# jcyk/gtos

Measured on AMD Instinct MI355X. Metric: graphs/sec training step (100-node AMR, batch 64), higher is better.
Workload: dtype bf16

## Files before the change

### gtos_amd/_lib.py

```python
import ctypes
import os
import threading

import torch

_HERE = os.path.dirname(os.path.abspath(__file__))
LIB_PATH = os.path.join(_HERE, "csrc", "libgtos_hip.so")
ABI_VERSION = 25

c_p, c_i, c_l, c_f, c_u64 = ctypes.c_void_p, ctypes.c_int, ctypes.c_int64, ctypes.c_float, ctypes.c_uint64

SIGNATURES = {
    "gtos_abi_version": [],
    "gtos_pathtrie_dev_workspace": [c_l, c_l, c_p],
    "gtos_pathtrie_dev_phase_a": [c_i, c_l, c_p, c_p, c_p, c_p, c_p, c_p, c_p, ctypes.c_size_t, c_p],
    "gtos_pathtrie_dev_phase_b": [c_l, c_l, c_i, c_i, c_i, c_i, c_p, c_p, c_p, c_p, c_p, ctypes.c_size_t, c_p],
    "gtos_relbatch_dev_workspace": [c_l, c_p],
    "gtos_relbatch_dev_phase_a": [c_p, c_p, c_p, ctypes.c_size_t, c_p],
    "gtos_relbatch_dev_phase_b": [c_p, c_l, c_p, c_p, ctypes.c_size_t, c_p],
    "gtos_relbatch_dev_all_count": [c_p, c_p, c_p, ctypes.c_size_t, c_p],
    "gtos_relbatch_dev_all_keys": [c_p, c_p, c_p, ctypes.c_size_t, c_p],
    "gtos_relbatch_dev_all_fill": [c_p, c_l, c_p, c_p, ctypes.c_size_t, c_p],
    "gtos_relindex_dev_workspace": [c_l, c_p],
    "gtos_relindex_dev_phase_a": [c_p, c_p, c_p, ctypes.c_size_t, c_p],
    "gtos_relindex_dev_phase_b": [c_p, c_l, c_p, c_p, ctypes.c_size_t, c_p],
    "gtos_gemm": [c_i, c_i, c_i, c_i, c_i, c_i, c_i, c_p, c_l, c_p, c_l, c_p, c_l, c_p, c_i, c_f, c_u64, c_i, c_i, c_p, c_l, c_p],
    "gtos_rel_attn_fwd": [c_i] * 7 + [c_p, c_l, c_p, c_l, c_p, c_l, c_p, c_p, c_p, c_p, c_f, c_f, c_u64, c_p, c_l, c_p, c_p, c_p],
    "gtos_rel_attn_bwd": [c_i] * 7 + [c_p, c_l, c_p, c_l, c_p, c_l, c_p, c_p, c_p, c_p, c_p, c_f, c_f, c_u64,
                                      c_p, c_l, c_p, c_p, c_p, c_l, c_p, c_p, c_l, c_p, c_l, c_p, c_l, c_p, c_l, c_p, c_p, c_p],
    "gtos_rel_attn_bwd_bank": [c_i] * 5 + [c_p, c_l, c_p, c_l, c_p, c_p, c_p, c_p, c_p, c_p, c_p, c_p, c_i, c_p, c_l, c_p, c_p],
    "gtos_ln_residual_fwd": [c_i, c_i, c_i, c_p, c_p, c_f, c_u64, c_p, c_p, c_f, c_p, c_p, c_p, c_p],
    "gtos_ln_residual_bwd": [c_i, c_i, c_i, c_p, c_p, c_p, c_f, c_u64, c_p, c_p, c_p, c_p, c_p, c_p, c_p, c_p],
    "gtos_ln_residual_fwd2": [c_i, c_i, c_i, c_i, c_i, c_p, c_p, c_f, c_u64, c_p, c_p, c_f, c_p, c_p, c_p, c_p, c_p],
    "gtos_ln_residual_bwd2": [c_i, c_i, c_i, c_i, c_i, c_p, c_p, c_p, c_p, c_f, c_u64, c_p, c_p, c_p, c_p, c_p, c_p, c_p, c_p],
    "gtos_relu_dropout_bwd": [c_i, c_l, c_p, c_p, c_f, c_p],
    "gtos_colsum": [c_i, c_i, c_i, c_l, c_p, c_p, c_p],
    "gtos_gru_cell_fwd": [c_i, c_i, c_i, c_p, c_p, c_p, c_p, c_l, c_p, c_p, c_f, c_u64, c_l, c_p],
    "gtos_gru_step_fwd": [c_i, c_i, c_p, c_l, c_i, c_p, c_p, c_p, c_p, c_p, c_p, c_p, c_p, c_p, c_p, c_p, c_p, c_i, c_p, c_l, c_p, c_p, c_p, c_l,
                          c_f, c_u64, c_l, c_p],
    "gtos_gru_step_bwd": [c_i, c_i, c_p, c_i, c_p, c_p, c_p, c_p, c_p, c_l, c_p, c_i, c_l, c_p, c_f, c_u64, c_l, c_p, c_i, c_p, c_p, c_p, c_i, c_p],
    "gtos_gru_step_bwd_fused": [c_i, c_i, c_p, c_i, c_p, c_p, c_p, c_p, c_p, c_l, c_p, c_i, c_l, c_p, c_f, c_u64, c_l, c_p, c_i, c_p, c_p, c_p, c_i,
                                c_p, c_p, c_l, c_i, c_i, c_f, c_u64, c_l, c_p],
    "gtos_gru_weight_grads": [c_i, c_i, c_i, c_i, c_p, c_p, c_l, c_p, c_l, c_p, c_l, c_p, c_l, c_p, c_l, c_p],
    "gtos_gemm_tn_batch": [c_i, c_p, c_p, c_p, c_p, c_p, c_p, c_p, c_p, c_p, c_p, c_p],
    "gtos_embed_packed_paths": [c_i, c_i, c_i, c_l, c_p, c_p, c_p, c_p, c_i, c_i, c_p, c_f, c_u64, c_p, c_i, c_p, c_p],
    "gtos_segment_sum_rows": [c_i, c_p, c_p, c_p, c_p, c_p, c_p, c_p, c_l, c_i, c_p, c_p, c_l, c_p, c_p, c_p],
    "gtos_segment_sum_stream": [c_i, c_i, c_p, c_p, c_p, c_p, c_p, c_p, c_i, c_p, c_l, c_i, c_p, c_l, c_p, c_p],
    "gtos_segment_sum_finish": [c_i, c_p, c_p, c_i, c_p, c_l, c_p],
    "gtos_segment_sum_ranges": [c_i, c_p, c_p, c_l, c_i, c_p, c_l, c_p],
    "gtos_gru_cell_bwd": [c_i, c_i, c_i, c_p, c_p, c_p, c_l, c_p, c_p, c_p, c_f, c_u64, c_l, c_p, c_i, c_p],
    "gtos_relation_gather_mean": [c_i, c_l, c_i, c_i, c_p, c_p, c_i, c_p, c_p],
    "gtos_embed_rows_fwd": [c_i, c_l, c_i, c_i, c_p, c_p, c_p, c_f, c_u64, c_p],
    "gtos_embed_rows_bwd": [c_i, c_l, c_i, c_i, c_i, c_p, c_p, c_p, c_f, c_u64, c_p, c_l, c_p],
    "gtos_copy_nll_fwd": [c_i, c_i, c_i, c_i, c_i, c_p, c_l, c_p, c_p, c_p, c_p, c_l, c_p, c_p, c_p, c_p],
    "gtos_copy_nll_bwd": [c_i, c_i, c_i, c_i, c_i, c_p, c_l, c_p, c_p, c_p, c_p, c_l, c_p, c_p, c_p, c_p, c_p, c_p, c_p],
    "gtos_copy_ll_fwd": [c_i, c_i, c_i, c_i, c_i, c_i, c_p, c_l, c_p, c_p, c_p, c_p, c_p],
    "gtos_copy_nll_ls_prep": [c_i, c_i, c_i, c_p, c_p, c_l, c_p],
    "gtos_copy_nll_ls_fwd": [c_i] * 5 + [c_p, c_l, c_p, c_p, c_p, c_l, c_f, c_p, c_l, c_p, c_p, c_p, c_p],
    "gtos_copy_nll_ls_bwd": [c_i] * 5 + [c_p, c_l, c_p, c_p, c_p, c_l, c_f, c_p, c_l, c_p, c_p, c_p, c_p, c_p, c_p, c_p],
    "gtos_copy_eval_fwd": [c_i, c_i, c_i, c_i, c_i, c_p, c_l, c_p, c_p, c_p, c_p, c_l, c_p, c_p, c_p, c_p],
    "gtos_eval_accumulate": [c_i, c_i, c_p, c_p, c_p, c_l, c_p, c_p, c_p, c_p, c_p],
    "gtos_beam_topk": [c_i, c_i, c_i, c_p, c_l, c_p, c_p, c_p],
    "gtos_beam_advance": [c_i] * 7 + [c_p] * 13,
    "gtos_beam_reorder": [c_i, c_p, c_p, c_l, c_i, c_i, c_i, c_i, c_p, c_p, c_p, c_p, c_i, c_i, c_p, c_p, c_p, c_p, c_i, c_l, c_p, c_p,
                          c_p, c_p],
    "gtos_sample_step": [c_i] * 7 + [c_f, c_i, c_f, c_u64, c_p, c_l] + [c_p] * 11 + [c_i, c_l] + [c_p] * 4,
    "gtos_highway_fwd": [c_i, c_l, c_i, c_p, c_p, c_p, c_p],
    "gtos_highway_bwd": [c_i, c_l, c_i, c_p, c_p, c_p, c_p, c_p, c_p],
    "gtos_max_relu_fwd": [c_i, c_l, c_i, c_i, c_p, c_p, c_p, c_p],
    "gtos_max_relu_bwd": [c_i, c_l, c_i, c_i, c_p, c_p, c_p, c_p, c_p],
    "gtos_token_row_fwd": [c_i, c_l, c_i, c_i, c_i, c_p, c_p, c_p, c_p, c_f, c_u64, c_p],
    "gtos_token_row_bwd": [c_i, c_l, c_i, c_i, c_i, c_p, c_p, c_p, c_p, c_f, c_u64, c_p],
    "gtos_sqnorm": [c_l, c_p, c_p, c_p],
    "gtos_adam_step": [c_l, c_p, c_p, c_p, c_p, c_f, c_f, c_f, c_f, c_f, c_f, c_p, c_f, c_p, c_p],
    "gtos_cast_f32_to_bf16": [c_l, c_p, c_p, c_p],
    "gtos_transpose_batch_bf16": [c_i, c_p, c_p, c_i, c_p, c_p, c_p],
    "gtos_step_control": [c_i, c_p, c_p, c_p, c_i, c_i, c_p, c_p],
    "gtos_set_seed_epoch": [c_p],
    "gtos_adam_step_ctl": [c_l, c_p, c_p, c_p, c_p, c_p, c_f, c_f, c_f, c_f, c_f, c_p, c_f, c_p, c_p],
}

_lib = None
_load_lock = threading.Lock()


class GtosHipError(RuntimeError):
    pass


def load():
    global _lib
    if _lib is not None:
        return _lib
    with _load_lock:
        if _lib is not None:
            return _lib
        if not os.path.exists(LIB_PATH):
            raise GtosHipError("%s is missing: run `python -m gtos_amd.build` (or __graft_entry__.build()); "
                               "there is no CPU fallback for the gtos hot path" % LIB_PATH)
        lib = ctypes.CDLL(LIB_PATH)
        for name, args in SIGNATURES.items():
            fn = getattr(lib, name)
            fn.argtypes = args
            fn.restype = ctypes.c_int
        if lib.gtos_abi_version() != ABI_VERSION:
            raise GtosHipError("libgtos_hip.so ABI %d != binding ABI %d: rebuild" % (lib.gtos_abi_version(), ABI_VERSION))
        _lib = lib
    return _lib


def call(name, *args):
    rc = getattr(load(), name)(*args)
    if rc != 0:
        raise GtosHipError("%s failed with code %d (%s)" % (
            name, rc, "HIP launch error" if rc > 0 else "unsupported argument/shape"))


def ptr(t):
    return None if t is None else t.data_ptr()


_raw_stream = None


def stream():
    global _raw_stream
    if _raw_stream:
        return _raw_stream(torch.cuda.current_device())
    pub = torch.cuda.current_stream().cuda_stream
    if _raw_stream is None:
        try:
            raw = torch._C._cuda_getCurrentRawStream
            ok = raw(torch.cuda.current_device()) == pub
            probe = torch.cuda.Stream()
            with torch.cuda.stream(probe):
                ok = ok and raw(torch.cuda.current_device()) == probe.cuda_stream == torch.cuda.current_stream().cuda_stream
            ok = ok and raw(torch.cuda.current_device()) == pub
            _raw_stream = raw if ok else False
        except Exception:
            _raw_stream = False
    return pub


def dt(t):
    if t.dtype == torch.float32:
        return 0
    if t.dtype == torch.bfloat16:
        return 1
    raise GtosHipError("unsupported dtype %s" % t.dtype)


def require_cuda(*ts):
    for t in ts:
        if t is not None and not t.is_cuda:
            raise GtosHipError("gtos_amd ops run on the GPU only (got a %s tensor); there is no CPU fallback" % t.device)
```

### gtos_amd/csrc/gemm.hip

```cpp
#include "common.h"
#include <stdlib.h>

__attribute__((visibility("hidden"))) const void* gtos_zero_block() {
    static void* z = nullptr;
    if (!z) {
        if (hipMalloc(&z, 256) != hipSuccess) return nullptr;
        if (hipMemset(z, 0, 256) != hipSuccess) return nullptr;
    }
    return z;
}

namespace {

constexpr int BM = 128, BN = 128;
constexpr int ROWB = 128;

template <typename T> struct GemmCfg;
template <> struct GemmCfg<bf16_t> { static constexpr int BK = 64, VEC = 8; };
template <> struct GemmCfg<float>  { static constexpr int BK = 32, VEC = 4; };

template <int NTH> struct TCfg {
    static constexpr int NT = NTH, WAVES_N = NTH / 128, WTN = BN / WAVES_N, NTW = WTN / 16;
    static constexpr int ITERS = 1024 / NTH;
};
// ... 639 lines not shown
    bool hi[2];
    uint32_t aoff[2][2], boff[2][2];
#pragma unroll
    for (int j = 0; j < 2; ++j) {
        const int rb = (wave + 8 * j) * 8 + (lane >> 3);
        const uint32_t ch = (uint32_t)(((lane & 7) ^ ((rb >> 1) & 7)) << 4);
        hi[j] = ch >= 64;
#pragma unroll
        for (int h = 0; h < 2; ++h) {
            aoff[h][j] = (uint32_t)min((rb >> 6) * 128 + h * 64 + (rb & 63), amax) * lda2 + ch;
            boff[h][j] = (uint32_t)min((rb >> 5) * 64 + h * 32 + (rb & 31), bmax) * ldb2 + ch;
        }
    }
    const int fo0 = fr * ROWB + ((fq ^ ((fr >> 1) & 7)) << 4), fo1 = fr * ROWB + (((4 + fq) ^ ((fr >> 1) & 7)) << 4);
    const int fa_base = wr * 64 * ROWB, fb_base = wc * 32 * ROWB;

    f32x4_t acc[8][4];
#pragma unroll
    for (int i = 0; i < 8; ++i)
#pragma unroll
        for (int j = 0; j < 4; ++j) acc[i][j] = f32x4_t{0.f, 0.f, 0.f, 0.f};
    bf16x8_t fa[4][2], fb[2][2];

#define GTOS_QDMA(src, dst)                                                                                                   \
    __builtin_amdgcn_global_load_lds((const __attribute__((address_space(1))) void*)(src),                                    \
                                     (__attribute__((address_space(3))) void*)(dst), 16, 0, 0)
#define GTOS_QISSUE(buf, isA, h, kt_)                                                                                         \
    {                                                                                                                         \
        const int kb_ = min((kt_), nk - 1) * 128;                                                                             \
        const bool tl_ = tail32 && (kt_) >= nk - 1;                                                                           \
        const char* s0_ = ((isA) ? Ab : Bb) + kb_ + ((isA) ? aoff[h][0] : boff[h][0]);                                        \
        const char* s1_ = ((isA) ? Ab : Bb) + kb_ + ((isA) ? aoff[h][1] : boff[h][1]);                                        \
        GTOS_QDMA((tl_ && hi[0]) ? Zl : s0_, (buf) + wave * 1024);                                                            \
        GTOS_QDMA((tl_ && hi[1]) ? Zl : s1_, (buf) + (8 + wave) * 1024);                                                      \
    }
#define GTOS_QREAD_A(buf)                                                                                                     \
    _Pragma("unroll") for (int i = 0; i < 4; ++i) {                                                                           \
        fa[i][0] = *reinterpret_cast<const bf16x8_t*>((buf) + fa_base + i * 16 * ROWB + fo0);                                 \
        fa[i][1] = *reinterpret_cast<const bf16x8_t*>((buf) + fa_base + i * 16 * ROWB + fo1);                                 \
    }
#define GTOS_QREAD_B(buf)                                                                                                     \
    _Pragma("unroll") for (int j = 0; j < 2; ++j) {                                                                           \
        fb[j][0] = *reinterpret_cast<const bf16x8_t*>((buf) + fb_base + j * 16 * ROWB + fo0);                                 \
        fb[j][1] = *reinterpret_cast<const bf16x8_t*>((buf) + fb_base + j * 16 * ROWB + fo1);                                 \
    }
#define GTOS_QPHASE(READS, ISSUE, mh, nh)                                                                                     \
    {                                                                                                                         \
        READS;                                                                                                                \
        __builtin_amdgcn_sched_barrier(0);                                                                                    \
        ISSUE;                                                                                                                \
        GTOS_VMCNT(4);                                             \
        __builtin_amdgcn_s_barrier();                                                                                         \
        __builtin_amdgcn_s_waitcnt(0xc07f);                                           \
        __builtin_amdgcn_sched_barrier(0);                                                                                    \
        _Pragma("unroll") for (int ks = 0; ks < 2; ++ks)                                                                      \
            _Pragma("unroll") for (int i = 0; i < 4; ++i)                                                                     \
                _Pragma("unroll") for (int j = 0; j < 2; ++j)                                                                 \
                    acc[(mh) * 4 + i][(nh) * 2 + j] =                                                                         \
                        __builtin_amdgcn_mfma_f32_16x16x32_bf16(fb[j][ks], fa[i][ks], acc[(mh) * 4 + i][(nh) * 2 + j], 0, 0, 0); \
        __builtin_amdgcn_sched_barrier(0);                                                                                    \
        __builtin_amdgcn_s_barrier();                                                                                         \
    }
#define GTOS_QTILE(A0_, B0_, B1_, A1_, nA0, nB0, nB1, nA1, kt_)                                                               \
    GTOS_QPHASE({ GTOS_QREAD_B(B0_); __builtin_amdgcn_sched_barrier(0); GTOS_QREAD_A(A0_); }, GTOS_QISSUE(nA0, true, 0, (kt_) + 1), 0, 0); \
    GTOS_QPHASE({ GTOS_QREAD_B(B1_); }, GTOS_QISSUE(nB0, false, 0, (kt_) + 1), 0, 1);                                         \
    GTOS_QPHASE({ GTOS_QREAD_A(A1_); }, GTOS_QISSUE(nB1, false, 1, (kt_) + 1), 1, 1);                                         \
    GTOS_QPHASE({ GTOS_QREAD_B(B0_); }, GTOS_QISSUE(nA1, true, 1, (kt_) + 1), 1, 0);

    GTOS_QISSUE(a00, true, 0, 0);
    GTOS_QISSUE(b00, false, 0, 0);
    GTOS_QISSUE(b01, false, 1, 0);
    GTOS_QISSUE(a01, true, 1, 0);
    GTOS_VMCNT(4);
    __builtin_amdgcn_s_barrier();
    if (wave >= 4) __builtin_amdgcn_s_barrier();
    int kt = 0;
    for (; kt + 2 <= nk; kt += 2) {
        GTOS_QTILE(a00, b00, b01, a01, a10, b10, b11, a11, kt);
        GTOS_QTILE(a10, b10, b11, a11, a00, b00, b01, a01, kt + 1);
    }
    if (kt < nk) { GTOS_QTILE(a00, b00, b01, a01, a10, b10, b11, a11, kt); }
    if (wave < 4) __builtin_amdgcn_s_barrier();
    GTOS_VMCNT(0);
    __syncthreads();
#undef GTOS_QTILE
#undef GTOS_QPHASE
#undef GTOS_QREAD_A
#undef GTOS_QREAD_B
#undef GTOS_QISSUE
#undef GTOS_QDMA

    bf16_t* C = static_cast<bf16_t*>(a.C);
    const float keep_scale = a.p_drop > 0.f ? 1.f / (1.f - a.p_drop) : 1.f;
    constexpr int CP = 64 * 2 + 16;
    char* cs = (wave < 4 ? a00 : b00) + (wave & 3) * 32 * CP;
#pragma unroll
    for (int q4 = 0; q4 < 4; ++q4) {
#pragma unroll
        for (int mh = 0; mh < 2; ++mh)
#pragma unroll
            for (int nt = 0; nt < 4; ++nt) {
                const int mt = q4 * 2 + mh;
                const int m = m0 + wm + mt * 16 + fr, n = n0 + wn + nt * 16 + fq * 4;
                float v[4] = {acc[mt][nt][0], acc[mt][nt][1], acc[mt][nt][2], acc[mt][nt][3]};
#pragma unroll
                for (int i = 0; i < 4; ++i) {
                    if (a.bias && n + i < a.N) v[i] += a.bias[n + i];
                    if (a.relu) v[i] = fmaxf(v[i], 0.f);
                    if (a.p_drop > 0.f)
                        v[i] = drop_keep(a.seed, (uint64_t)m * (uint64_t)a.N + (uint64_t)(n + i), a.p_drop) ? v[i] * keep_scale : 0.f;
                }
                *reinterpret_cast<uint2*>(cs + (mh * 16 + fr) * CP + (nt * 16 + fq * 4) * 2) = make_uint2(pack_bf(v[0], v[1]), pack_bf(v[2], v[3]));
            }
        __builtin_amdgcn_fence(__ATOMIC_RELEASE, "wavefront");
        __builtin_amdgcn_s_waitcnt(0xc07f);
#pragma unroll
        for (int pass = 0; pass < 4; ++pass) {
            const int row = pass * 8 + (lane >> 3), col = (lane & 7) * 8;
            const int m = m0 + wm + q4 * 32 + row, n = n0 + wn + col;
            if (m >= a.M || n >= a.N) continue;
            uint4 val = *reinterpret_cast<const uint4*>(cs + row * CP + col * 2);
            bf16_t* cp = C + (int64_t)m * a.ldc + n;
            if (n + 8 <= a.N) {
                if (a.accumulate) {
                    const uint4 old = *reinterpret_cast<const uint4*>(cp);
                    val = make_uint4(pack_bf(lo_bf(val.x) + lo_bf(old.x), hi_bf(val.x) + hi_bf(old.x)),
                                     pack_bf(lo_bf(val.y) + lo_bf(old.y), hi_bf(val.y) + hi_bf(old.y)),
                                     pack_bf(lo_bf(val.z) + lo_bf(old.z), hi_bf(val.z) + hi_bf(old.z)),
                                     pack_bf(lo_bf(val.w) + lo_bf(old.w), hi_bf(val.w) + hi_bf(old.w)));
                }
                *reinterpret_cast<uint4*>(cp) = val;
            } else {
                const bf16_t* e = reinterpret_cast<const bf16_t*>(cs + row * CP + col * 2);
                for (int i = 0; i < 8 && n + i < a.N; ++i) {
                    float o = bf2f(e[i]);
                    if (a.accumulate) o += bf2f(cp[i]);
                    cp[i] = f2bf(o);
                }
            }
        }
        __builtin_amdgcn_s_waitcnt(0xc07f);
    }
}

int launch256p(const GemmArgs& a, hipStream_t s) {
    const long long nMt = (a.M + BM2 - 1) / BM2, nNt = (a.N + BN2 - 1) / BN2;
    const long long nblk = ((nMt + 7) / 8) * 8 * nNt;
    if (nblk > 0x7fffffffLL) return -6;
    hipLaunchKernelGGL(gemm256q_nt_kernel, dim3((unsigned)nblk), dim3(512), 0, s, a);
    GTOS_CHECK_LAUNCH();
    return 0;
}

struct TnGroup {
    const bf16_t* B1; int64_t ldb1; int N1;
    int tiles;
    int tmn[64];
};

struct TnJob { const bf16_t* A; const bf16_t* B; float* C; int lda, ldb, ldc, M, N, K, tile_end, nN; };
constexpr int TN_MAX_JOBS = 48;
struct TnBatch { int njobs, ntiles; TnJob job[TN_MAX_JOBS]; };

template <int MODE, typename G>
__global__ __launch_bounds__(512) void gemm256p_tn_kernel(GemmArgs a, G g) {
    constexpr bool GROUPED = MODE == 1;
    __shared__ __attribute__((aligned(16))) char st0[ST3];
    __shared__ __attribute__((aligned(16))) char st1[ST3];
    __shared__ __attribute__((aligned(16))) char st2[ST3];
    __shared__ __attribute__((aligned(16))) char st3[ST3];
    const int lane = threadIdx.x & 63, wave = __builtin_amdgcn_readfirstlane(threadIdx.x >> 6);
    const int fr = lane & 15, fq = lane >> 4;
    const int wm = (wave >> 2) * 128, wn = (wave & 3) * 64;
    const int nN = (a.N + BN2 - 1) / BN2, nM = (a.M + BM2 - 1) / BM2;
    int tiles = nM * nN;
    if constexpr (GROUPED) tiles = g.tiles;
    if constexpr (MODE == 2) tiles = 1;
    const int xcd = blockIdx.x & 7, sq = blockIdx.x >> 3;
    int bz = (sq / tiles) * 8 + xcd, t_ = sq % tiles;
    if constexpr (MODE == 2) { bz = 0; t_ = blockIdx.x; if (t_ >= g.ntiles) return; }
    if (bz >= a.splitk) return;
    int m0, n0, Nv;
    const bf16_t* Bp;
    int64_t ldb, wld;
    float* wst;
    if constexpr (MODE == 2) {
        int j = 0;
        while (j + 1 < g.njobs && t_ >= g.job[j].tile_end) ++j;
        const TnJob& jb = g.job[j];
        const int tl = t_ - (j ? g.job[j - 1].tile_end : 0);
        m0 = (tl / jb.nN) * BM2; n0 = (tl % jb.nN) * BN2;
        a.A = jb.A; a.lda = jb.lda; a.M = jb.M; a.K = jb.K; a.splitk = 1;
        Bp = jb.B; ldb = jb.ldb; Nv = jb.N;
        wst = jb.C + (int64_t)m0 * jb.ldc + n0; wld = jb.ldc;
    } else if constexpr (GROUPED) {
        const int e = g.tmn[t_], src = (e >> 8) & 255;
        m0 = (e & 255) * BM2; n0 = ((e >> 16) & 255) * BN2;
        Bp = src ? g.B1 : static_cast<const bf16_t*>(a.B); ldb = src ? g.ldb1 : a.ldb; Nv = src ? g.N1 : a.N;
        wst = a.ws + ((int64_t)bz * tiles + t_) * (BM2 * BN2); wld = BN2;
    } else {
        m0 = (t_ / nN) * BM2; n0 = (t_ % nN) * BN2;
        Bp = static_cast<const bf16_t*>(a.B); ldb = a.ldb; Nv = a.N;
        wst = a.ws + ((int64_t)bz * a.M + m0) * a.N + n0; wld = a.N;
    }
    const int ktiles = (a.K + 63) / 64, tps = (ktiles + a.splitk - 1) / a.splitk;
    const int kbeg = bz * tps * 64, kend = min(a.K, kbeg + tps * 64);
    if (kbeg >= kend) return;
    const int nk = (kend - kbeg + 31) / 32;
    const char* Z = static_cast<const char*>(a.zeros);
    const int kr = lane >> 5, pp = lane & 31;
    const int kl0 = 2 * wave + kr, kq_d = kl0 & 3;
    const int lp = ((((pp >> 1) ^ kq_d)) << 1) | (pp & 1);
    const int acol = min(m0 + lp * 8, a.M - 8), bcol = min(n0 + lp * 8, Nv - 8);
    const char* pa = reinterpret_cast<const char*>(static_cast<const bf16_t*>(a.A) + (int64_t)(kbeg + kl0) * a.lda + acol);
    const char* pb = reinterpret_cast<const char*>(Bp + (int64_t)(kbeg + kl0) * ldb + bcol);
    const int64_t a16 = 32 * a.lda, b16 = 32 * ldb;
    int kcur = kbeg + kl0;
    const int kq = fr >> 2;
    const int fbase = (fq * 8 + kq) * 512 + (fr & 3) * 8;

    f32x4_t acc[8][4];
#pragma unroll
    for (int i = 0; i < 8; ++i)
#pragma unroll
        for (int j = 0; j < 4; ++j) acc[i][j] = f32x4_t{0.f, 0.f, 0.f, 0.f};
    bf16x8_t fa[8], fb[4];

#define GTOS_DMA1(src, dst)                                                                                                   \
    __builtin_amdgcn_global_load_lds((const __attribute__((address_space(1))) void*)(src),                                    \
                                     (__attribute__((address_space(3))) void*)(dst), 16, 0, 0)
#define GTOS_DMA4(stage)                                                                                                      \
    {                                                                                                                         \
        const bool ok0 = kcur < kend, ok1 = kcur + 16 < kend;                                                                 \
        GTOS_DMA1(ok0 ? pa : Z, (stage) + wave * 1024);                                                                       \
        GTOS_DMA1(ok1 ? pa + a16 : Z, (stage) + (8 + wave) * 1024);                                                           \
        GTOS_DMA1(ok0 ? pb : Z, (stage) + A3 + wave * 1024);                                                                  \
        GTOS_DMA1(ok1 ? pb + b16 : Z, (stage) + A3 + (8 + wave) * 1024);                                                      \
        kcur += 32; pa += 2 * a16; pb += 2 * b16;                                                                             \
    }
#define GTOS_TRF(tile, c0)                                                                                                    \
    ([&]() -> bf16x8_t {                                                                                                      \
        const char* p0 = (tile) + fbase + ((((c0) >> 4) ^ kq) << 5);                                                          \
        const s16x4_t lo = __builtin_amdgcn_ds_read_tr16_b64_v4i16((__attribute__((address_space(3))) s16x4_t*)(p0));         \
        const s16x4_t hi = __builtin_amdgcn_ds_read_tr16_b64_v4i16((__attribute__((address_space(3))) s16x4_t*)(p0 + 4 * 512)); \
        const s16x8_t v = {lo[0], lo[1], lo[2], lo[3], hi[0], hi[1], hi[2], hi[3]};                                           \
        return __builtin_bit_cast(bf16x8_t, v);                                                                               \
    }())
#define GTOS_STEP(slot_s, slot_d, s_)                                                                                         \
    {                                                                                                                         \
        GTOS_DMA4(slot_d);                                                                                                  \
        _Pragma("unroll") for (int t = 0; t < 4; ++t) fb[t] = GTOS_TRF((slot_s) + A3, wn + t * 16);                           \
        _Pragma("unroll") for (int t = 0; t < 8; ++t) fa[t] = GTOS_TRF((slot_s), wm + t * 16);                                \
        __builtin_amdgcn_s_waitcnt(0x0078);                 \
        __builtin_amdgcn_s_barrier();                                                                                         \
        __builtin_amdgcn_sched_barrier(0);                                                                                    \
        _Pragma("unroll") for (int mt = 0; mt < 8; ++mt)                                                                      \
            _Pragma("unroll") for (int nt = 0; nt < 4; ++nt)                                                                  \
                acc[mt][nt] = __builtin_amdgcn_mfma_f32_16x16x32_bf16(fb[nt], fa[mt], acc[mt][nt], 0, 0, 0);                  \
        __builtin_amdgcn_sched_barrier(0);                                                                                    \
        __builtin_amdgcn_s_barrier();                                                                                         \
    }

    GTOS_DMA4(st0);
    GTOS_DMA4(st1);
    GTOS_DMA4(st2);
    GTOS_VMCNT(8);
    __builtin_amdgcn_s_barrier();
    if (wave >= 4) __builtin_amdgcn_s_barrier();
    int s = 0;
    for (; s + 4 <= nk; s += 4) {
        GTOS_STEP(st0, st3, s);
        GTOS_STEP(st1, st0, s + 1);
        GTOS_STEP(st2, st1, s + 2);
        GTOS_STEP(st3, st2, s + 3);
    }
    if (s < nk) {
        GTOS_STEP(st0, st3, s);
        if (s + 1 < nk) {
            GTOS_STEP(st1, st0, s + 1);
            if (s + 2 < nk) GTOS_STEP(st2, st1, s + 2);
        }
    }
    if (wave < 4) __builtin_amdgcn_s_barrier();
#undef GTOS_STEP
#undef GTOS_TRF
#undef GTOS_DMA4
#undef GTOS_DMA1

#pragma unroll
    for (int mt = 0; mt < 8; ++mt) {
        const int m = m0 + wm + mt * 16 + fr;
        if (m >= a.M) continue;
#pragma unroll
        for (int nt = 0; nt < 4; ++nt) {
            const int n = n0 + wn + nt * 16 + fq * 4;
            if (n >= Nv) continue;
            float4* dst = reinterpret_cast<float4*>(wst + (int64_t)(m - m0) * wld + (n - n0));
            if constexpr (MODE == 2) {
                const float4 o = *dst;
                *dst = make_float4(o.x + acc[mt][nt][0], o.y + acc[mt][nt][1], o.z + acc[mt][nt][2], o.w + acc[mt][nt][3]);
            } else {
                *dst = make_float4(acc[mt][nt][0], acc[mt][nt][1], acc[mt][nt][2], acc[mt][nt][3]);
            }
        }
    }
}

struct ColJob { const bf16_t* A; float* out; int lda, M, K, blk_end, gx; };
struct ColBatch { int njobs, nblocks, rpb; ColJob job[TN_MAX_JOBS]; };
__global__ __launch_bounds__(256) void colsum_batch_kernel(ColBatch g) {
    __shared__ float red[4][64][8];
    int t_ = blockIdx.x, j = 0;
    if (t_ >= g.nblocks) return;
    while (j + 1 < g.njobs && t_ >= g.job[j].blk_end) ++j;
    const ColJob& jb = g.job[j];
    const int tl = t_ - (j ? g.job[j - 1].blk_end : 0);
    const int bx = tl % jb.gx, by = tl / jb.gx;
    const int lane = threadIdx.x & 63, w = threadIdx.x >> 6;
    const int c = (bx * 64 + lane) * 8;
    const int r0 = by * g.rpb, r1 = min(jb.K, r0 + g.rpb);
    float acc[8] = {0, 0, 0, 0, 0, 0, 0, 0};
    if (c < jb.M) {
        for (int r = r0 + w; r < r1; r += 4) {
            float v[8];
            Vec8<bf16_t>::load(jb.A + (int64_t)r * jb.lda + c, v);
#pragma unroll
            for (int e = 0; e < 8; ++e) acc[e] += v[e];
        }
    }
#pragma unroll
    for (int e = 0; e < 8; ++e) red[w][lane][e] = acc[e];
    __syncthreads();
    if (w == 0 && c < jb.M) {
#pragma unroll
        for (int e = 0; e < 8; ++e) atomicAdd(jb.out + c + e, red[0][lane][e] + red[1][lane][e] + red[2][lane][e] + red[3][lane][e]);
    }
}

struct GruDwOut { float* dwih; int64_t ld_ih; float* dwhh; int64_t ld_hh; int hs, in_dim; };
__global__ void gru_dw_reduce_kernel(const float* __restrict__ ws, int splits, TnGroup g, GruDwOut o) {
    const int t_ = blockIdx.x >> 6, q = (blockIdx.x & 63) * 256 + threadIdx.x;
    const int e = g.tmn[t_], src = (e >> 8) & 255;
    const int r = q >> 6, c = (q & 63) * 4;
    const int i = (e & 255) * BM2 + r, j = ((e >> 16) & 255) * BN2 + c;
    if (i >= 4 * o.hs) return;
    const int gate = i / o.hs, ch = i - gate * o.hs;
    float* dst;
    if (src == 0) {
        if (gate == 3 || j >= o.in_dim) return;
        dst = o.dwih + (int64_t)(gate * o.hs + ch) * o.ld_ih + j;
    } else {
        if (gate == 2 || j >= o.hs) return;
        dst = o.dwhh + (int64_t)((gate == 3 ? 2 : gate) * o.hs + ch) * o.ld_hh + j;
    }
    const float* p = ws + (int64_t)t_ * (BM2 * BN2) + r * BN2 + c;
    const int64_t plane = (int64_t)g.tiles * (BM2 * BN2);
    float4 acc = *reinterpret_cast<const float4*>(p);
    for (int s = 1; s < splits; ++s) {
        const float4 v = *reinterpret_cast<const float4*>(p + s * plane);
        acc.x += v.x; acc.y += v.y; acc.z += v.z; acc.w += v.w;
    }
    dst[0] += acc.x; dst[1] += acc.y; dst[2] += acc.z; dst[3] += acc.w;
}

int launch256p_tn(const GemmArgs& a, hipStream_t s) {
    const long long tiles = ((long long)(a.M + BM2 - 1) / BM2) * ((a.N + BN2 - 1) / BN2);
    const long long nblk = tiles * 8 * ((a.splitk + 7) / 8);
    if (nblk > 0x7fffffffLL) return -6;
    hipLaunchKernelGGL((gemm256p_tn_kernel<0, TnGroup>), dim3((unsigned)nblk), dim3(512), 0, s, a, TnGroup{});
    GTOS_CHECK_LAUNCH();
    return 0;
}

int launch256(const GemmArgs& a, hipStream_t s) {
    static bool configured = false;
    if (!configured) {
        if (hipFuncSetAttribute(reinterpret_cast<const void*>(gemm256_nt_kernel), hipFuncAttributeMaxDynamicSharedMemorySize,
                                2 * STAGE2) != hipSuccess) return -7;
        configured = true;
    }
    const long long nMt = (a.M + BM2 - 1) / BM2, nNt = (a.N + BN2 - 1) / BN2;
    const long long nblk = ((nMt + 7) / 8) * 8 * nNt;
    if (nblk > 0x7fffffffLL) return -6;
    hipLaunchKernelGGL(gemm256_nt_kernel, dim3((unsigned)nblk), dim3(512), 2 * STAGE2, s, a);
    GTOS_CHECK_LAUNCH();
    return 0;
}

template <typename T, typename TO>
int launch(const GemmArgs& a, int transA, int transB, hipStream_t s) {
    const long long nMt = (a.M + BM - 1) / BM, nNt = (a.N + BN - 1) / BN;
    const long long nblk = a.splitk > 1 ? nMt * nNt * 8 * ((a.splitk + 7) / 8) : ((nMt + 7) / 8) * 8 * nNt;
    if (nblk > 0x7fffffffLL) return -6;
    dim3 grid((unsigned)nblk);
    const bool fast = a.vecA && a.vecB;
    constexpr bool BF = sizeof(T) == 2;
    if (!transA && transB) {
        if (fast) hipLaunchKernelGGL((gemm_kernel<T, TO, false, true, true, 256, 1>), grid, dim3(256), 0, s, a);
        else      hipLaunchKernelGGL((gemm_kernel<T, TO, false, true, false, 512, 2>), grid, dim3(512), 0, s, a);
    } else if (!transA && !transB) {
        if (fast && BF) hipLaunchKernelGGL((gemm_kernel<T, TO, false, false, true, 256, BF ? 1 : 2>), grid, dim3(256), 0, s, a);
        else if (fast)  hipLaunchKernelGGL((gemm_kernel<T, TO, false, false, true, 512, 2>), grid, dim3(512), 0, s, a);
        else            hipLaunchKernelGGL((gemm_kernel<T, TO, false, false, false, 512, 2>), grid, dim3(512), 0, s, a);
    } else if (transA && !transB) {
        if (fast && BF) hipLaunchKernelGGL((gemm_kernel<T, TO, true, false, true, 256, BF ? 1 : 2>), grid, dim3(256), 0, s, a);
        else if (fast)  hipLaunchKernelGGL((gemm_kernel<T, TO, true, false, true, 512, 2>), grid, dim3(512), 0, s, a);
        else            hipLaunchKernelGGL((gemm_kernel<T, TO, true, false, false, 512, 2>), grid, dim3(512), 0, s, a);
    } else return -2;
    GTOS_CHECK_LAUNCH();
    return 0;
}

}

extern "C" int gtos_gemm(int in_dtype, int out_dtype, int transA, int transB, int M, int N, int K,
                         const void* A, int64_t lda, const void* B, int64_t ldb, void* C, int64_t ldc,
                         const float* bias, int relu, float p_drop, uint64_t seed, int accumulate,
                         int splitk, void* workspace, int64_t workspace_bytes, void* stream) {
    if (M <= 0 || N <= 0) return 0;
    if (K <= 0) return -3;
    const int es = in_dtype == GTOS_BF16 ? 2 : 4, vec = 16 / es;
    const int eo = out_dtype == GTOS_BF16 ? 2 : 4;
    GemmArgs a;
    a.A = A; a.B = B; a.C = C; a.bias = bias; a.M = M; a.N = N; a.K = K; a.lda = lda; a.ldb = ldb; a.ldc = ldc;
    a.vecA = ((uintptr_t)A % 16 == 0) && (lda % vec == 0) && ((transA ? M : K) % vec == 0);
    a.vecB = ((uintptr_t)B % 16 == 0) && (ldb % vec == 0) && ((transB ? K : N) % vec == 0);
    a.vecC = ((uintptr_t)C % 16 == 0) && (ldc % (16 / eo) == 0);
    a.relu = relu; a.accumulate = accumulate; a.p_drop = p_drop; a.seed = seed;
    a.zeros = zero_block();
    if (!a.zeros) return -5;
    if (splitk < 1) splitk = 1;
    const int BKc = in_dtype == GTOS_BF16 ? GemmCfg<bf16_t>::BK : GemmCfg<float>::BK;
    const int ktiles = (K + BKc - 1) / BKc;
    if (splitk > ktiles) splitk = ktiles;
    if (splitk > 1) { const int tps = (ktiles + splitk - 1) / splitk; splitk = (ktiles + tps - 1) / tps; }
    a.splitk = splitk;
    if (splitk > 1 && (out_dtype != GTOS_F32 || bias || relu || p_drop > 0.f || !accumulate)) return -4;
    hipStream_t s = static_cast<hipStream_t>(stream);
    a.ws = nullptr;
    if (splitk > 1 && workspace && N % 4 == 0 && (uintptr_t)workspace % 16 == 0 && (uintptr_t)C % 4 == 0 &&
        (int64_t)splitk * M * N * 4 <= workspace_bytes) {
        a.ws = static_cast<float*>(workspace);
        const int kps = ((ktiles + splitk - 1) / splitk) * BKc;
        const bool tn256 = g_use_pipe_tn && in_dtype == GTOS_BF16 && transA && !transB && a.vecA && a.vecB && M >= 256 && N >= 256 &&
                           M % 8 == 0 && N % 8 == 0 && kps >= 256;
        int rc = tn256 ? launch256p_tn(a, s)
                       : (in_dtype == GTOS_BF16 ? launch<bf16_t, float>(a, transA, transB, s) : launch<float, float>(a, transA, transB, s));
        if (rc) return rc;
        const int64_t total = (int64_t)M * (N / 4);
        const int nb = (int)((total + 255) / 256 < 2048 ? (total + 255) / 256 : 2048);
        hipLaunchKernelGGL(splitk_reduce_kernel, dim3(nb), dim3(256), 0, s, a.ws, splitk, M, N, static_cast<float*>(C), ldc);
        GTOS_CHECK_LAUNCH();
        return 0;
    }
    if (in_dtype == GTOS_BF16 && out_dtype == GTOS_BF16) {
        const long long t256 = ((long long)(M + BM2 - 1) / BM2) * ((N + BN2 - 1) / BN2);
        if (g_use_pipe && !transA && transB && a.vecA && a.vecB && a.vecC && splitk == 1 && N >= 256 && K % 32 == 0 &&
            lda < (1 << 22) && ldb < (1 << 22) &&
            (t256 >= 512 && K >= g_min_kpipe))
            return launch256p(a, s);
        if (g_use256 && !transA && transB && a.vecA && a.vecB && a.vecC && splitk == 1 && t256 >= 1024 && N >= 256 && K >= g_min_k256)
            return launch256(a, s);
        return launch<bf16_t, bf16_t>(a, transA, transB, s);
    }
    if (in_dtype == GTOS_BF16 && out_dtype == GTOS_F32)  return launch<bf16_t, float>(a, transA, transB, s);
    if (in_dtype == GTOS_F32 && out_dtype == GTOS_F32)   return launch<float, float>(a, transA, transB, s);
    return -1;
}


extern "C" int gtos_gru_weight_grads(int rows, int hs, int in_dim, int in_valid, const void* d4, const void* x, int64_t ldx, const void* hprev, int64_t ldh,
                                     float* dwih, int64_t ld_dwih, float* dwhh, int64_t ld_dwhh, void* workspace, int64_t workspace_bytes,
                                     void* stream) {
    if (rows <= 0) return 0;
    if (hs <= 0 || hs % 64 || in_dim < 8 || in_dim % 8 || ldx < in_dim || ldx % 8 || ldh < hs || ldh % 8 || in_valid < 1 || in_valid > in_dim ||
        in_valid % 4) return -22;
    if (!d4 || !x || !hprev || !dwih || !dwhh || !workspace) return -23;
    if ((uintptr_t)d4 % 16 || (uintptr_t)x % 16 || (uintptr_t)hprev % 16 || (uintptr_t)dwih % 4 || (uintptr_t)dwhh % 4 || (uintptr_t)workspace % 16 ||
        ld_dwih < in_valid || ld_dwhh < hs) return -25;
    GemmArgs a{};
    a.A = d4; a.lda = 4 * (int64_t)hs; a.M = 4 * hs; a.B = x; a.ldb = ldx; a.N = in_dim; a.K = rows; a.vecA = a.vecB = 1;
    a.accumulate = 1; a.zeros = zero_block();
    if (!a.zeros) return -5;
    TnGroup g{};
    g.B1 = static_cast<const bf16_t*>(hprev); g.ldb1 = ldh; g.N1 = hs;
    int nt = 0;
    for (int mb = 0; mb * BM2 < 4 * hs; ++mb) {
        const int lo = mb * BM2, hi = (lo + BM2 < 4 * hs ? lo + BM2 : 4 * hs) - 1;
        const int g_lo = lo / hs, g_hi = hi / hs;
        const bool needs_x = g_lo <= 2, needs_h = !(g_lo == 2 && g_hi == 2);
        for (int src = 0; src < 2; ++src) {
            if (!(src ? needs_h : needs_x)) continue;
            const int ncols = src ? hs : in_dim;
            for (int nb = 0; nb * BN2 < ncols; ++nb) {
                if (nt >= 64) return -28;
                g.tmn[nt++] = mb | (src << 8) | (nb << 16);
            }
        }
    }
    g.tiles = nt;
    const int ktiles = (rows + 63) / 64;
    const long long tile_bytes = (long long)BM2 * BN2 * 4;
    long long sk = 8LL * (32 / nt > 0 ? 32 / nt : 1);
    if (sk > ktiles / 4) sk = ktiles / 4;
    if (sk * nt * tile_bytes > workspace_bytes) sk = workspace_bytes / (nt * tile_bytes);
    if (sk < 1) { if (nt * tile_bytes > workspace_bytes) return -4; sk = 1; }
    const int tps = (int)((ktiles + sk - 1) / sk);
    a.splitk = (ktiles + tps - 1) / tps;
    a.ws = static_cast<float*>(workspace);
    hipStream_t s = static_cast<hipStream_t>(stream);
    const long long nblk = (long long)nt * 8 * ((a.splitk + 7) / 8);
    hipLaunchKernelGGL((gemm256p_tn_kernel<1, TnGroup>), dim3((unsigned)nblk), dim3(512), 0, s, a, g);
    GTOS_CHECK_LAUNCH();
    GruDwOut o{dwih, ld_dwih, dwhh, ld_dwhh, hs, in_valid};
    hipLaunchKernelGGL(gru_dw_reduce_kernel, dim3((unsigned)(nt * 64)), dim3(256), 0, s, a.ws, a.splitk, g, o);
    GTOS_CHECK_LAUNCH();
    return 0;
}

extern "C" int gtos_gemm_tn_batch(int n, const void* const* A, const int64_t* lda, const int* M, const void* const* B, const int64_t* ldb,
                                  const int* N, const int* K, float* const* C, const int64_t* ldc, float* const* bias, void* stream) {
    if (n <= 0) return 0;
    if (!A || !lda || !M || !B || !ldb || !N || !K || !C || !ldc) return -23;
    hipStream_t s = static_cast<hipStream_t>(stream);
    const void* zeros = zero_block();
    if (!zeros) return -5;
    for (int j = 0; j < n; ++j) {
        if (M[j] < 8 || M[j] % 8 || N[j] < 8 || N[j] % 8 || K[j] < 1 || lda[j] < M[j] || lda[j] % 8 || ldb[j] < N[j] || ldb[j] % 8 || ldc[j] < N[j] ||
            ldc[j] % 4 || lda[j] >= (1LL << 31) || ldb[j] >= (1LL << 31) || ldc[j] >= (1LL << 31)) return -22;
        if (!A[j] || !B[j] || !C[j] || (uintptr_t)A[j] % 16 || (uintptr_t)B[j] % 16 || (uintptr_t)C[j] % 16) return -25;
        if (bias && bias[j] && (uintptr_t)bias[j] % 4) return -25;
    }
    for (int j0 = 0, nj = 0; j0 < n; j0 += nj) {
        nj = 0;
        while (nj < TN_MAX_JOBS && j0 + nj < n) {
            const int q = j0 + nj;
            const uintptr_t lo = (uintptr_t)C[q], hi = lo + (uintptr_t)(((int64_t)(M[q] - 1) * ldc[q] + N[q]) * 4);
            bool meets = false;
            for (int p = j0; p < q && !meets; ++p) {
                const uintptr_t plo = (uintptr_t)C[p], phi = plo + (uintptr_t)(((int64_t)(M[p] - 1) * ldc[p] + N[p]) * 4);
                meets = lo < phi && plo < hi;
            }
            if (meets) break;
            ++nj;
        }
        TnBatch tb{};
        ColBatch cb{};
        int tiles = 0, blocks = 0, ncol = 0;
        cb.rpb = 512;
        for (int j = 0; j < nj; ++j) {
            const int q = j0 + j;
            TnJob& t = tb.job[j];
            t.A = static_cast<const bf16_t*>(A[q]); t.B = static_cast<const bf16_t*>(B[q]); t.C = C[q];
            t.lda = (int)lda[q]; t.ldb = (int)ldb[q]; t.ldc = (int)ldc[q]; t.M = M[q]; t.N = N[q]; t.K = K[q];
            t.nN = (N[q] + BN2 - 1) / BN2;
            tiles += ((M[q] + BM2 - 1) / BM2) * t.nN;
            t.tile_end = tiles;
            if (bias && bias[q]) {
                ColJob& c = cb.job[ncol++];
                c.A = t.A; c.out = bias[q]; c.lda = t.lda; c.M = t.M; c.K = t.K;
                c.gx = (t.M + 511) / 512;
                blocks += c.gx * ((t.K + cb.rpb - 1) / cb.rpb);
                c.blk_end = blocks;
            }
        }
        tb.njobs = nj; tb.ntiles = tiles;
        GemmArgs a{};
        a.splitk = 1; a.zeros = zeros; a.vecA = a.vecB = 1; a.accumulate = 1;
        hipLaunchKernelGGL((gemm256p_tn_kernel<2, TnBatch>), dim3((unsigned)tiles), dim3(512), 0, s, a, tb);
        GTOS_CHECK_LAUNCH();
        if (ncol) {
            cb.njobs = ncol; cb.nblocks = blocks;
            hipLaunchKernelGGL(colsum_batch_kernel, dim3((unsigned)blocks), dim3(256), 0, s, cb);
            GTOS_CHECK_LAUNCH();
        }
    }
    return 0;
}

GTOS_SEED_EPOCH_SETTER(gemm)
```

### gtos_amd/csrc/gru_step.hip

```cpp
#include <cstdlib>
#include "common.h"

__attribute__((visibility("hidden"))) const void* gtos_zero_block();

#define GTOS_VMCNT(n) __builtin_amdgcn_s_waitcnt(0x0F70 | ((n) & 15) | (((n) >> 4) << 14))
#ifndef GTOS_RACE_DEMO
#define GTOS_VMCNT_LDS(n) __builtin_amdgcn_s_waitcnt(0x0070 | ((n) & 15) | (((n) >> 4) << 14))
#define GTOS_LGKM0() __builtin_amdgcn_s_waitcnt(0xc07f)
#else
#define GTOS_VMCNT_LDS(n) GTOS_VMCNT(n)
#define GTOS_LGKM0()
#endif

namespace {

constexpr int ROWB = 128, BK = 64, TM = 128, TC = 64, WROWS = 3 * TC;
constexpr int A_BYTES = TM * ROWB, B_BYTES = WROWS * ROWB;

__device__ __forceinline__ int swz(int row) { return ((row >> 1) & 7) ^ ((row >> 4) & 3); }
__device__ __forceinline__ int lds_off(int r, int c) { return r * ROWB + ((c ^ swz(r)) << 4); }

struct StepArgs {
    const bf16_t* x; int64_t ldx; int in_dim; const bf16_t* w_ih; const float* b_ih;
    const bf16_t* xg;
    const bf16_t* gf; const int* gf_idx; const bf16_t* gb; const int* gb_idx;
    const bf16_t* h_in; const int* h_idx; const bf16_t* w_hh; const float* b_hh;
    bf16_t* h_out; int n_out; bf16_t* h_fin; bf16_t* gates; bf16_t* y; int64_t ldy;
    int64_t ld_fin; const int* fin_idx;
    float p_drop; uint64_t seed; int64_t drop_base;
    int rows, hs; const void* zeros;
};

__device__ __forceinline__ void dma_rows(const bf16_t* __restrict__ base, const U128* __restrict__ zeros, int64_t ld, int rows_total,
                                         int row0, int k0, int kend, char* tile, int wave, int lane,
                                         const int* __restrict__ gather = nullptr) {
#pragma unroll
    for (int it = 0; it < TM / 32; ++it) {
        const int blk = it * 4 + wave, rl = blk * 8 + (lane >> 3);
        const int c = (lane & 7) ^ swz(rl);
        const int r = row0 + rl, k = k0 + c * 8;
        const bool ok = r < rows_total && k + 8 <= kend;
        const int64_t sr = (gather && ok) ? gather[r] : r;
        const void* src = ok ? static_cast<const void*>(base + sr * ld + k) : static_cast<const void*>(zeros);
        __builtin_amdgcn_global_load_lds((const __attribute__((address_space(1))) void*)src,
                                         (__attribute__((address_space(3))) void*)(tile + blk * 1024), 16, 0, 0);
    }
}

__device__ __forceinline__ void dma_weights(const bf16_t* __restrict__ w, const U128* __restrict__ zeros, int64_t ld, int hs,
                                            int c0, int k0, int kend, char* tile, int wave, int lane) {
#pragma unroll
    for (int it = 0; it < WROWS / 32; ++it) {
        const int blk = it * 4 + wave, rl = blk * 8 + (lane >> 3);
        const int g = rl >> 6, nt = (rl >> 4) & 3, q = (rl >> 2) & 3, e = rl & 3;
        const int wrow = g * hs + c0 + q * 16 + nt * 4 + e;
        const int c = (lane & 7) ^ swz(rl);
        const int k = k0 + c * 8;
        const bool ok = k + 8 <= kend;
        const void* src = ok ? static_cast<const void*>(w + (int64_t)wrow * ld + k) : static_cast<const void*>(zeros);
        __builtin_amdgcn_global_load_lds((const __attribute__((address_space(1))) void*)src,
                                         (__attribute__((address_space(3))) void*)(tile + blk * 1024), 16, 0, 0);
    }
}

struct RowSrc { const char* p[TM / 32]; int c[TM / 32]; };
__device__ __forceinline__ RowSrc row_src(const bf16_t* __restrict__ base, int64_t ld, int rows_total, int row0, int wave, int lane,
                                          const int* __restrict__ gather = nullptr, int zero_row = -1) {
    RowSrc s;
#pragma unroll
    for (int it = 0; it < TM / 32; ++it) {
        const int rl = (it * 4 + wave) * 8 + (lane >> 3);
        const int r = row0 + rl;
        s.c[it] = (lane & 7) ^ swz(rl);
        const bool ok = r < rows_total;
        const int64_t sr = (gather && ok) ? gather[r] : r;
        s.p[it] = (ok && sr != zero_row) ? reinterpret_cast<const char*>(base + sr * ld + s.c[it] * 8) : nullptr;
    }
    return s;
}
__device__ __forceinline__ void dma_rows_at(const RowSrc& s, const U128* __restrict__ zeros, int k0, int kend, char* tile, int wave) {
#pragma unroll
    for (int it = 0; it < TM / 32; ++it) {
        const bool ok = s.p[it] != nullptr && k0 + s.c[it] * 8 + 8 <= kend;
        const void* src = ok ? static_cast<const void*>(s.p[it] + (int64_t)k0 * 2) : static_cast<const void*>(zeros);
        __builtin_amdgcn_global_load_lds((const __attribute__((address_space(1))) void*)src,
                                         (__attribute__((address_space(3))) void*)(tile + (it * 4 + wave) * 1024), 16, 0, 0);
    }
}
__device__ __forceinline__ void dma_rows_at_z(const RowSrc& s, int k0, char* tile, int wave, int lane) {
#pragma unroll
    for (int it = 0; it < TM / 32; ++it) {
        char* blk = tile + (it * 4 + wave) * 1024;
        if (s.p[it] != nullptr)
            __builtin_amdgcn_global_load_lds((const __attribute__((address_space(1))) void*)(s.p[it] + (int64_t)k0 * 2),
                                             (__attribute__((address_space(3))) void*)blk, 16, 0, 0);
        else
            *reinterpret_cast<uint4*>(blk + lane * 16) = make_uint4(0, 0, 0, 0);
    }
}
struct WSrc { uint32_t off[WROWS / 32]; int c[WROWS / 32]; };
__device__ __forceinline__ WSrc w_src(int64_t ld, int hs, int c0, int wave, int lane) {
    WSrc s;
#pragma unroll
    for (int it = 0; it < WROWS / 32; ++it) {
        const int rl = (it * 4 + wave) * 8 + (lane >> 3);
        const int g = rl >> 6, nt = (rl >> 4) & 3, q = (rl >> 2) & 3, e = rl & 3;
        const int wrow = g * hs + c0 + q * 16 + nt * 4 + e;
        s.c[it] = (lane & 7) ^ swz(rl);
        s.off[it] = (uint32_t)(wrow * (int)ld + s.c[it] * 8) * 2u;
    }
    return s;
}
__device__ __forceinline__ void dma_weights_at(const WSrc& s, const bf16_t* __restrict__ w, const U128* __restrict__ zeros, int k0, int kend,
                                               char* tile, int wave) {
    const char* wk = reinterpret_cast<const char*>(w) + (int64_t)k0 * 2;
#pragma unroll
    for (int it = 0; it < WROWS / 32; ++it) {
        const bool ok = k0 + s.c[it] * 8 + 8 <= kend;
        const void* src = ok ? static_cast<const void*>(wk + s.off[it]) : static_cast<const void*>(zeros);
        __builtin_amdgcn_global_load_lds((const __attribute__((address_space(1))) void*)src,
                                         (__attribute__((address_space(3))) void*)(tile + (it * 4 + wave) * 1024), 16, 0, 0);
    }
}

template <int NG, int G2>
__device__ __forceinline__ void mma_tile(const char* As, const char* Bs, int wrow0, int fr, int fq, f32x4_t (&acc)[2][NG * 4]) {
#pragma unroll
    for (int ks = 0; ks < 2; ++ks) {
        bf16x8_t fa[2];
#pragma unroll
        for (int mt = 0; mt < 2; ++mt) fa[mt] = *reinterpret_cast<const bf16x8_t*>(As + lds_off(wrow0 + mt * 16 + fr, ks * 4 + fq));
#pragma unroll
        for (int g = 0; g < 3; ++g) {
            const int ag = g < 2 ? g : G2;
#pragma unroll
            for (int nt = 0; nt < 4; ++nt) {
                const bf16x8_t fb = *reinterpret_cast<const bf16x8_t*>(Bs + lds_off(g * 64 + nt * 16 + fr, ks * 4 + fq));
#pragma unroll
                for (int mt = 0; mt < 2; ++mt)
                    acc[mt][ag * 4 + nt] = __builtin_amdgcn_mfma_f32_16x16x32_bf16(fb, fa[mt], acc[mt][ag * 4 + nt], 0, 0, 0);
            }
        }
    }
}

__device__ __forceinline__ void ld16(const bf16_t* p, float (&v)[16]) {
    const uint4 a = *reinterpret_cast<const uint4*>(p), b = *reinterpret_cast<const uint4*>(p + 8);
    v[0] = lo_bf(a.x); v[1] = hi_bf(a.x); v[2] = lo_bf(a.y); v[3] = hi_bf(a.y);
    v[4] = lo_bf(a.z); v[5] = hi_bf(a.z); v[6] = lo_bf(a.w); v[7] = hi_bf(a.w);
    v[8] = lo_bf(b.x); v[9] = hi_bf(b.x); v[10] = lo_bf(b.y); v[11] = hi_bf(b.y);
    v[12] = lo_bf(b.z); v[13] = hi_bf(b.z); v[14] = lo_bf(b.w); v[15] = hi_bf(b.w);
}
__device__ __forceinline__ void st16(bf16_t* p, const float (&v)[16]) {
    *reinterpret_cast<uint4*>(p) = make_uint4(pack_bf(v[0], v[1]), pack_bf(v[2], v[3]), pack_bf(v[4], v[5]), pack_bf(v[6], v[7]));
    *reinterpret_cast<uint4*>(p + 8) = make_uint4(pack_bf(v[8], v[9]), pack_bf(v[10], v[11]), pack_bf(v[12], v[13]), pack_bf(v[14], v[15]));
}
__device__ __forceinline__ void ldf16(const float* p, float (&v)[16]) {
#pragma unroll
    for (int i = 0; i < 4; ++i) {
        const float4 a = *reinterpret_cast<const float4*>(p + i * 4);
        v[i * 4] = a.x; v[i * 4 + 1] = a.y; v[i * 4 + 2] = a.z; v[i * 4 + 3] = a.w;
    }
}

__device__ __forceinline__ float fast_tanh(float x) {
    const float e = __expf(2.f * x);
    return 1.f - 2.f * __builtin_amdgcn_rcpf(e + 1.f);
}

template <int MODE>
__device__ __forceinline__ void step_cell(const StepArgs& a, f32x4_t (&acc)[2][(MODE == 1 ? 4 : 3) * 4], int m0, int c0, int wave, int fr, int fq) {
    constexpr bool HAS_X = MODE == 1;
    constexpr int GH = HAS_X ? 3 : 2;
    const int cb = c0 + fq * 16, hs = a.hs;
    float bhr[16], bhz[16], bhn[16];
    ldf16(a.b_hh + cb, bhr); ldf16(a.b_hh + hs + cb, bhz); ldf16(a.b_hh + 2 * hs + cb, bhn);
    if constexpr (MODE != 0) {
        float t[16];
        ldf16(a.b_ih + cb, t);
#pragma unroll
        for (int i = 0; i < 16; ++i) bhr[i] += t[i];
        ldf16(a.b_ih + hs + cb, t);
#pragma unroll
        for (int i = 0; i < 16; ++i) bhz[i] += t[i];
    }
    const float ks = a.p_drop > 0.f ? 1.f / (1.f - a.p_drop) : 1.f;
#pragma unroll
    for (int mt = 0; mt < 2; ++mt) {
        const int m = m0 + wave * 32 + mt * 16 + fr;
        if (m >= a.rows) continue;
        float xr[16], xz[16], xn[16], hp[16];
        if constexpr (HAS_X) {
            ldf16(a.b_ih + 2 * hs + cb, xn);
#pragma unroll
            for (int i = 0; i < 16; ++i) { xr[i] = 0.f; xz[i] = 0.f; xn[i] += acc[mt][8 + (i >> 2)][i & 3]; }
        } else if constexpr (MODE == 2) {
            const bf16_t* fp = a.gf + (int64_t)a.gf_idx[m] * 3 * hs + cb;
            const bf16_t* bp = a.gb + (int64_t)a.gb_idx[m] * 3 * hs + cb;
            float t[16];
            ld16(fp, xr); ld16(bp, t);
#pragma unroll
            for (int i = 0; i < 16; ++i) xr[i] += t[i];
            ld16(fp + hs, xz); ld16(bp + hs, t);
#pragma unroll
            for (int i = 0; i < 16; ++i) xz[i] += t[i];
            ld16(fp + 2 * hs, xn); ld16(bp + 2 * hs, t);
#pragma unroll
            for (int i = 0; i < 16; ++i) xn[i] += t[i];
            ldf16(a.b_ih + 2 * hs + cb, t);
#pragma unroll
            for (int i = 0; i < 16; ++i) xn[i] += t[i];
        } else {
            const bf16_t* xp = a.xg + (int64_t)m * 3 * hs + cb;
            ld16(xp, xr); ld16(xp + hs, xz); ld16(xp + 2 * hs, xn);
        }
        ld16(a.h_in + (int64_t)(a.h_idx ? a.h_idx[m] : m) * hs + cb, hp);
        float gr[16], gz[16], gn[16], hn[16], o[16];
#pragma unroll
        for (int i = 0; i < 16; ++i) {
            gr[i] = 1.f / (1.f + __expf(-(xr[i] + acc[mt][(i >> 2)][i & 3] + bhr[i])));
            gz[i] = 1.f / (1.f + __expf(-(xz[i] + acc[mt][4 + (i >> 2)][i & 3] + bhz[i])));
            hn[i] = acc[mt][GH * 4 + (i >> 2)][i & 3] + bhn[i];
            hn[i] = bf2f(f2bf(hn[i]));
            gn[i] = fast_tanh(xn[i] + gr[i] * hn[i]);
            o[i] = (1.f - gz[i]) * gn[i] + gz[i] * hp[i];
        }
        bf16_t* gp = a.gates + (int64_t)m * 4 * hs + cb;
        st16(gp, gr); st16(gp + hs, gz); st16(gp + 2 * hs, gn);
        st16(gp + 3 * hs, hn);
        bf16_t* hdst = m < a.n_out ? a.h_out + (int64_t)m * hs + cb
                                   : a.h_fin + (int64_t)(a.fin_idx ? a.fin_idx[m] : m) * a.ld_fin + cb;
        st16(hdst, o);
        if (a.y) {
            if (a.p_drop > 0.f) {
#pragma unroll
                for (int i = 0; i < 16; ++i)
                    o[i] = drop_keep(a.seed, (uint64_t)(a.drop_base + (int64_t)m * a.ldy + cb + i), a.p_drop) ? o[i] * ks : 0.f;
            }
            st16(a.y + (int64_t)m * a.ldy + cb, o);
        }
    }
}

template <int MODE>
__global__ __launch_bounds__(256, 2) void gru_step_fwd_kernel(StepArgs a) {
    if (a.p_drop > 0.f) a.seed = live_seed(a.seed);
    constexpr bool HAS_X = MODE == 1;
    constexpr int NG = HAS_X ? 4 : 3;
    constexpr int GH = HAS_X ? 3 : 2;
    __shared__ __attribute__((aligned(16))) char lds[A_BYTES + B_BYTES];
    char* As = lds;
    char* Bs = lds + A_BYTES;
    const int lane = threadIdx.x & 63, wave = __builtin_amdgcn_readfirstlane(threadIdx.x >> 6);
    const int fr = lane & 15, fq = lane >> 4;
    const int nC = a.hs / TC;
    const int xcd = blockIdx.x & 7, sq = blockIdx.x >> 3;
    const int m0 = ((sq / nC) * 8 + xcd) * TM, c0 = (sq % nC) * TC;
    if (m0 >= a.rows) return;
    const U128* Z = static_cast<const U128*>(a.zeros);

    f32x4_t acc[2][NG * 4];
#pragma unroll
    for (int i = 0; i < 2; ++i)
#pragma unroll
        for (int j = 0; j < NG * 4; ++j) acc[i][j] = f32x4_t{0.f, 0.f, 0.f, 0.f};

    if constexpr (HAS_X) {
        const RowSrc xs = row_src(a.x, a.ldx, a.rows, m0, wave, lane);
        const WSrc ws = w_src(a.in_dim, a.hs, c0, wave, lane);
        for (int k0 = 0; k0 < a.in_dim; k0 += BK) {
            dma_rows_at(xs, Z, k0, a.in_dim, As, wave);
            dma_weights_at(ws, a.w_ih, Z, k0, a.in_dim, Bs, wave);
            __syncthreads();
            mma_tile<NG, 2>(As, Bs, wave * 32, fr, fq, acc);
            __syncthreads();
        }
    }
    {
        const RowSrc hsrc = row_src(a.h_in, a.hs, a.rows, m0, wave, lane, a.h_idx);
        const WSrc ws = w_src(a.hs, a.hs, c0, wave, lane);
        for (int k0 = 0; k0 < a.hs; k0 += BK) {
            dma_rows_at(hsrc, Z, k0, a.hs, As, wave);
            dma_weights_at(ws, a.w_hh, Z, k0, a.hs, Bs, wave);
            __syncthreads();
            mma_tile<NG, GH>(As, Bs, wave * 32, fr, fq, acc);
            __syncthreads();
        }
    }

    step_cell<MODE>(a, acc, m0, c0, wave, fr, fq);
}


__global__ __launch_bounds__(512, 2) void gru_step_fwd_a2w3_kernel(StepArgs a) {
    constexpr int TMW = 256, AW = TMW * ROWB;
    if (a.p_drop > 0.f) a.seed = live_seed(a.seed);
    __shared__ __attribute__((aligned(16))) char sa0[AW];
    __shared__ __attribute__((aligned(16))) char sa1[AW];
    __shared__ __attribute__((aligned(16))) char sw0[B_BYTES];
    __shared__ __attribute__((aligned(16))) char sw1[B_BYTES];
    __shared__ __attribute__((aligned(16))) char sa2[AW];
    const int lane = threadIdx.x & 63, wave = __builtin_amdgcn_readfirstlane(threadIdx.x >> 6);
    const int fr = lane & 15, fq = lane >> 4;
    const int hs = a.hs, nC = hs / TC;
    const int xcd = blockIdx.x & 7, sq = blockIdx.x >> 3;
    const int m0 = ((sq / nC) * 8 + xcd) * TMW, c0 = (sq % nC) * TC;
    if (m0 >= a.rows) return;
    const int nkx = a.in_dim / BK, nk = nkx + hs / BK;
    uint32_t axo[4], aho[4], bxo[3], bho[3];
#pragma unroll
    for (int i = 0; i < 4; ++i) {
        const int rl = (i * 8 + wave) * 8 + (lane >> 3);
        const int r = min(m0 + rl, a.rows - 1) - m0;
        const uint32_t c = (uint32_t)(((lane & 7) ^ swz(rl)) << 4);
        axo[i] = (uint32_t)r * (uint32_t)(a.ldx * 2) + c;
        aho[i] = (uint32_t)r * (uint32_t)(hs * 2) + c;
    }
#pragma unroll
    for (int i = 0; i < 3; ++i) {
        const int rl = (i * 8 + wave) * 8 + (lane >> 3);
        const int g = rl >> 6, nt = (rl >> 4) & 3, q = (rl >> 2) & 3, e = rl & 3;
        const int wrow = g * hs + c0 + q * 16 + nt * 4 + e;
        const uint32_t c = (uint32_t)(((lane & 7) ^ swz(rl)) << 4);
        bxo[i] = (uint32_t)wrow * (uint32_t)(a.in_dim * 2) + c;
        bho[i] = (uint32_t)wrow * (uint32_t)(hs * 2) + c;
    }
    const char* Xb = reinterpret_cast<const char*>(a.x + (int64_t)m0 * a.ldx);
    const char* Hb = reinterpret_cast<const char*>(a.h_in + (int64_t)m0 * hs);
    const char* Wi = reinterpret_cast<const char*>(a.w_ih);
    const char* Wh = reinterpret_cast<const char*>(a.w_hh);

    f32x4_t acc[2][16];
#pragma unroll
    for (int i = 0; i < 2; ++i)
#pragma unroll
        for (int j = 0; j < 16; ++j) acc[i][j] = f32x4_t{0.f, 0.f, 0.f, 0.f};

#define GTOS_DMA1(src, dst)                                                                                                   \
    __builtin_amdgcn_global_load_lds((const __attribute__((address_space(1))) void*)(src),                                    \
                                     (__attribute__((address_space(3))) void*)(dst), 16, 0, 0)
#define GTOS_A2W3_DMA_A(slot, s_)                                                                                             \
    {                                                                                                                         \
        const int st_ = min((s_), nk - 1);                                                                                    \
        const bool px_ = st_ < nkx;                                                                                           \
        const char* ab_ = px_ ? Xb + st_ * ROWB : Hb + (st_ - nkx) * ROWB;                                                    \
        GTOS_DMA1(ab_ + (px_ ? axo[0] : aho[0]), (slot) + (0 * 8 + wave) * 1024);                                             \
        GTOS_DMA1(ab_ + (px_ ? axo[1] : aho[1]), (slot) + (1 * 8 + wave) * 1024);                                             \
        GTOS_DMA1(ab_ + (px_ ? axo[2] : aho[2]), (slot) + (2 * 8 + wave) * 1024);                                             \
        GTOS_DMA1(ab_ + (px_ ? axo[3] : aho[3]), (slot) + (3 * 8 + wave) * 1024);                                             \
    }
#define GTOS_A2W3_DMA_W(slot, s_)                                                                                             \
    {                                                                                                                         \
        const int st_ = min((s_), nk - 1);                                                                                    \
        const bool px_ = st_ < nkx;                                                                                           \
        const char* bb_ = px_ ? Wi + st_ * ROWB : Wh + (st_ - nkx) * ROWB;                                                    \
        GTOS_DMA1(bb_ + (px_ ? bxo[0] : bho[0]), (slot) + (0 * 8 + wave) * 1024);                                             \
        GTOS_DMA1(bb_ + (px_ ? bxo[1] : bho[1]), (slot) + (1 * 8 + wave) * 1024);                                             \
        GTOS_DMA1(bb_ + (px_ ? bxo[2] : bho[2]), (slot) + (2 * 8 + wave) * 1024);                                             \
    }
#define GTOS_A2W3_STEP(sa_, sw_, sa_n, sw_n, s_)                                                                              \
    {                                                                                                                         \
        GTOS_VMCNT_LDS(4);                                  \
        __builtin_amdgcn_s_barrier();                       \
        GTOS_A2W3_DMA_W(sw_n, (s_) + 1);                                                                                      \
        GTOS_A2W3_DMA_A(sa_n, (s_) + 2);                                                                                      \
        {                                                                                                                     \
            _Pragma("unroll") for (int ks = 0; ks < 2; ++ks) {                                                                \
                bf16x8_t fa[2], fb[12];                                                                                       \
                _Pragma("unroll") for (int mt = 0; mt < 2; ++mt)                                                              \
                    fa[mt] = *reinterpret_cast<const bf16x8_t*>((sa_) + lds_off(wave * 32 + mt * 16 + fr, ks * 4 + fq));      \
                _Pragma("unroll") for (int t = 0; t < 12; ++t)                                                                \
                    fb[t] = *reinterpret_cast<const bf16x8_t*>((sw_) + lds_off(t * 16 + fr, ks * 4 + fq));                    \
                _Pragma("unroll") for (int g = 0; g < 2; ++g)                                                                 \
                    _Pragma("unroll") for (int nt = 0; nt < 4; ++nt)                                                          \
                        _Pragma("unroll") for (int mt = 0; mt < 2; ++mt)                                                      \
                            acc[mt][g * 4 + nt] = __builtin_amdgcn_mfma_f32_16x16x32_bf16(fb[g * 4 + nt], fa[mt], acc[mt][g * 4 + nt], 0, 0, 0); \
                if ((s_) < nkx) {                                                                                             \
                    _Pragma("unroll") for (int nt = 0; nt < 4; ++nt)                                                          \
                        _Pragma("unroll") for (int mt = 0; mt < 2; ++mt)                                                      \
                            acc[mt][8 + nt] = __builtin_amdgcn_mfma_f32_16x16x32_bf16(fb[8 + nt], fa[mt], acc[mt][8 + nt], 0, 0, 0); \
                } else {                                                                                                      \
                    _Pragma("unroll") for (int nt = 0; nt < 4; ++nt)                                                          \
                        _Pragma("unroll") for (int mt = 0; mt < 2; ++mt)                                                      \
                            acc[mt][12 + nt] = __builtin_amdgcn_mfma_f32_16x16x32_bf16(fb[8 + nt], fa[mt], acc[mt][12 + nt], 0, 0, 0); \
                }                                                                                                             \
            }                                                                                                                 \
        }                                                                                                                     \
    }

    if (nk > 0) {
        GTOS_A2W3_DMA_A(sa0, 0);
        GTOS_A2W3_DMA_W(sw0, 0);
        GTOS_A2W3_DMA_A(sa1, 1);
    }
    for (int s = 0; s + 6 <= nk; s += 6) {
        GTOS_A2W3_STEP(sa0, sw0, sa2, sw1, s);
        GTOS_A2W3_STEP(sa1, sw1, sa0, sw0, s + 1);
        GTOS_A2W3_STEP(sa2, sw0, sa1, sw1, s + 2);
        GTOS_A2W3_STEP(sa0, sw1, sa2, sw0, s + 3);
        GTOS_A2W3_STEP(sa1, sw0, sa0, sw1, s + 4);
        GTOS_A2W3_STEP(sa2, sw1, sa1, sw0, s + 5);
    }
    GTOS_VMCNT(0);
#undef GTOS_A2W3_STEP
#undef GTOS_A2W3_DMA_W
#undef GTOS_A2W3_DMA_A
#undef GTOS_DMA1
    step_cell<1>(a, acc, m0, c0, wave, fr, fq);
}


struct Raw16 { uint4 a, b; };
__device__ __forceinline__ void unpack16(const Raw16& r, float (&v)[16]) {
    v[0] = lo_bf(r.a.x); v[1] = hi_bf(r.a.x); v[2] = lo_bf(r.a.y); v[3] = hi_bf(r.a.y);
    v[4] = lo_bf(r.a.z); v[5] = hi_bf(r.a.z); v[6] = lo_bf(r.a.w); v[7] = hi_bf(r.a.w);
    v[8] = lo_bf(r.b.x); v[9] = hi_bf(r.b.x); v[10] = lo_bf(r.b.y); v[11] = hi_bf(r.b.y);
    v[12] = lo_bf(r.b.z); v[13] = hi_bf(r.b.z); v[14] = lo_bf(r.b.w); v[15] = hi_bf(r.b.w);
}
__device__ __forceinline__ Raw16 ldraw16(const bf16_t* p) {
    Raw16 r;
    r.a = *reinterpret_cast<const uint4*>(p);
    r.b = *reinterpret_cast<const uint4*>(p + 8);
    return r;
}

constexpr int P_ROWS = 32;
constexpr int P_TM = 4 * P_ROWS;

template <int KT>
__global__ __launch_bounds__(256, 1) void gru_l1_fwd_persistent_kernel(StepArgs a, int n_workers) {
    extern __shared__ __attribute__((aligned(16))) char plds[];
    constexpr int HS = 64 * KT;
    constexpr int A_TILE = P_ROWS * ROWB;
    const int lane = threadIdx.x & 63, wave = __builtin_amdgcn_readfirstlane(threadIdx.x >> 6);
    const int fr = lane & 15, fq = lane >> 4;
    char* Ws = plds;
    char* Aw = plds + KT * B_BYTES + wave * (KT * A_TILE);
    const int nC = KT;
    const int xcd = blockIdx.x & 7, sub = blockIdx.x >> 3;
    const int ct = sub % nC, worker = (sub / nC) * 8 + xcd, c0 = ct * TC;
    const U128* Z = static_cast<const U128*>(a.zeros);
#pragma unroll
    for (int kt = 0; kt < KT; ++kt) dma_weights(a.w_hh, Z, HS, HS, c0, kt * BK, HS, Ws + kt * B_BYTES, wave, lane);
    __syncthreads();

    const int cb = c0 + fq * 16;
    float bhr[16], bhz[16], bhn[16], bin[16];
    {
        float t[16];
        ldf16(a.b_hh + cb, bhr); ldf16(a.b_ih + cb, t);
#pragma unroll
        for (int i = 0; i < 16; ++i) bhr[i] += t[i];
        ldf16(a.b_hh + HS + cb, bhz); ldf16(a.b_ih + HS + cb, t);
#pragma unroll
        for (int i = 0; i < 16; ++i) bhz[i] += t[i];
        ldf16(a.b_hh + 2 * HS + cb, bhn); ldf16(a.b_ih + 2 * HS + cb, bin);
    }
    const int n_tiles = (a.rows + P_TM - 1) / P_TM;

    auto dma_A = [&](int tile) {
        const int r0 = tile * P_TM + wave * P_ROWS;
#pragma unroll
        for (int kt = 0; kt < KT; ++kt)
#pragma unroll
            for (int it = 0; it < P_ROWS / 8; ++it) {
                const int rl = it * 8 + (lane >> 3);
                const int c = (lane & 7) ^ swz(rl);
                const int r = r0 + rl;
                const void* src = r < a.rows ? static_cast<const void*>(a.h_in + (int64_t)r * HS + kt * BK + c * 8)
                                             : static_cast<const void*>(Z);
                __builtin_amdgcn_global_load_lds((const __attribute__((address_space(1))) void*)src,
                                                 (__attribute__((address_space(3))) void*)(Aw + kt * A_TILE + it * 1024), 16, 0, 0);
            }
    };
    struct Pre { Raw16 f[3], b[3], h; };
    auto gather = [&](int tile, Pre (&P)[2]) {
#pragma unroll
        for (int mt = 0; mt < 2; ++mt) {
            int m = tile * P_TM + wave * P_ROWS + mt * 16 + fr;
            m = m < a.rows ? m : a.rows - 1;
            const bf16_t* fp = a.gf + (int64_t)a.gf_idx[m] * 3 * HS + cb;
            const bf16_t* bp = a.gb + (int64_t)a.gb_idx[m] * 3 * HS + cb;
#pragma unroll
            for (int g = 0; g < 3; ++g) { P[mt].f[g] = ldraw16(fp + g * HS); P[mt].b[g] = ldraw16(bp + g * HS); }
            P[mt].h = ldraw16(a.h_in + (int64_t)m * HS + cb);
        }
    };

    int tile = worker;
    Pre P[2];
    if (tile < n_tiles) { dma_A(tile); gather(tile, P); }
    for (; tile < n_tiles; tile += n_workers) {
        f32x4_t acc[2][12];
#pragma unroll
        for (int i = 0; i < 2; ++i)
#pragma unroll
            for (int j = 0; j < 12; ++j) acc[i][j] = f32x4_t{0.f, 0.f, 0.f, 0.f};
#pragma unroll
        for (int kt = 0; kt < KT; ++kt) {
            const char* As = Aw + kt * A_TILE;
            const char* Bs = Ws + kt * B_BYTES;
#pragma unroll
            for (int ks = 0; ks < 2; ++ks) {
                bf16x8_t fa[2];
#pragma unroll
                for (int mt = 0; mt < 2; ++mt) fa[mt] = *reinterpret_cast<const bf16x8_t*>(As + lds_off(mt * 16 + fr, ks * 4 + fq));
#pragma unroll
                for (int g = 0; g < 3; ++g)
#pragma unroll
                    for (int nt = 0; nt < 4; ++nt) {
                        const bf16x8_t fb = *reinterpret_cast<const bf16x8_t*>(Bs + lds_off(g * 64 + nt * 16 + fr, ks * 4 + fq));
#pragma unroll
                        for (int mt = 0; mt < 2; ++mt)
                            acc[mt][g * 4 + nt] = __builtin_amdgcn_mfma_f32_16x16x32_bf16(fb, fa[mt], acc[mt][g * 4 + nt], 0, 0, 0);
                    }
            }
        }
        __builtin_amdgcn_s_waitcnt(0xc07f);
        const int next = tile + n_workers;
        if (next < n_tiles) dma_A(next);
#pragma unroll
        for (int mt = 0; mt < 2; ++mt) {
            const int m = tile * P_TM + wave * P_ROWS + mt * 16 + fr;
            float xr[16], xz[16], xn[16], hp[16], t[16];
            unpack16(P[mt].f[0], xr); unpack16(P[mt].b[0], t);
#pragma unroll
            for (int i = 0; i < 16; ++i) xr[i] += t[i];
            unpack16(P[mt].f[1], xz); unpack16(P[mt].b[1], t);
#pragma unroll
            for (int i = 0; i < 16; ++i) xz[i] += t[i];
            unpack16(P[mt].f[2], xn); unpack16(P[mt].b[2], t);
#pragma unroll
            for (int i = 0; i < 16; ++i) xn[i] += t[i] + bin[i];
            unpack16(P[mt].h, hp);
            float gr[16], gz[16], gn[16], hn[16], o[16];
#pragma unroll
            for (int i = 0; i < 16; ++i) {
                gr[i] = 1.f / (1.f + __expf(-(xr[i] + acc[mt][(i >> 2)][i & 3] + bhr[i])));
                gz[i] = 1.f / (1.f + __expf(-(xz[i] + acc[mt][4 + (i >> 2)][i & 3] + bhz[i])));
                hn[i] = bf2f(f2bf(acc[mt][8 + (i >> 2)][i & 3] + bhn[i]));
                gn[i] = fast_tanh(xn[i] + gr[i] * hn[i]);
                o[i] = (1.f - gz[i]) * gn[i] + gz[i] * hp[i];
            }
            if (m < a.rows) {
                bf16_t* gp = a.gates + (int64_t)m * 4 * HS + cb;
                st16(gp, gr); st16(gp + HS, gz); st16(gp + 2 * HS, gn);
                st16(gp + 3 * HS, hn);
                bf16_t* hdst = m < a.n_out ? a.h_out + (int64_t)m * HS + cb
                                           : a.h_fin + (int64_t)(a.fin_idx ? a.fin_idx[m] : m) * a.ld_fin + cb;
                st16(hdst, o);
            }
        }
        if (next < n_tiles) gather(next, P);
    }
}


struct StepBwdArgs {
    const bf16_t* d4_prev; int rows_prev; const bf16_t* wh_t;
    const bf16_t* gates; const bf16_t* hprev; const int* hprev_idx; const bf16_t* dy; int64_t ldy;
    void* dh; int dh_bf16; int64_t ld_dh; bf16_t* d4; float* bias_part; int n_partials;
    bf16_t* hp_out;
    const int* sum_idx;
    const void* dh_src;
    int zero_row;
    float p_drop; uint64_t seed; int64_t drop_base;
    int rows, hs; const void* zeros;
    const bf16_t* wi_t; bf16_t* dinp; int64_t ld_dinp; int n_in; int dinp_acc;
    float p_in; uint64_t seed_in; int64_t in_drop_base;
};

#define GTOS_DPP(v, ctrl) __builtin_bit_cast(float, __builtin_amdgcn_update_dpp(0, __builtin_bit_cast(int, (v)), (ctrl), 0xF, 0xF, true))
__device__ __forceinline__ float row16_sum(float v) {
    v += GTOS_DPP(v, 0xB1); v += GTOS_DPP(v, 0x4E); v += GTOS_DPP(v, 0x141); v += GTOS_DPP(v, 0x140);
    return v;
}

__device__ __forceinline__ void dma_wt(const bf16_t* __restrict__ w, int64_t ld, int c0, int k0, char* tile, int wave, int lane) {
#pragma unroll
    for (int it = 0; it < TC / 32; ++it) {
        const int blk = it * 4 + wave, rl = blk * 8 + (lane >> 3);
        const int nt = (rl >> 4) & 3, q = (rl >> 2) & 3, e = rl & 3;
        const int wrow = c0 + q * 16 + nt * 4 + e;
        const int c = (lane & 7) ^ swz(rl);
        const void* src = static_cast<const void*>(w + (int64_t)wrow * ld + k0 + c * 8);
        __builtin_amdgcn_global_load_lds((const __attribute__((address_space(1))) void*)src,
                                         (__attribute__((address_space(3))) void*)(tile + blk * 1024), 16, 0, 0);
    }
}

template <int NB, bool SKIP>
__device__ __forceinline__ void kloop_a2(const bf16_t* __restrict__ A, int64_t lda, int rows_total, int m0, const bf16_t* __restrict__ W,
                                         int64_t ldw, int n0, int nsub, int hs, const U128* __restrict__ Z, char* a0, char* a1, char* ws,
                                         f32x4_t (&acc)[2][NB * 4], int wave, int lane) {
    const int fr = lane & 15, fq = lane >> 4, nst = 3 * hs / BK;
#define GTOS_KA_A(slot, s_)                                                                                                   \
    {                                                                                                                         \
        const int kk_ = min((s_), nst - 1) * BK, ak_ = SKIP ? (kk_ < 2 * hs ? kk_ : kk_ + hs) : kk_;                            \
        dma_rows(A, Z, lda, rows_total, m0, ak_, ak_ + BK, (slot), wave, lane);                                               \
    }
#define GTOS_KA_STEP(cur, nxt, s_)                                                                                            \
    {                                                                                                                         \
        _Pragma("unroll") for (int h = 0; h < NB; ++h)                                                                        \
            if (h < nsub) dma_wt(W, ldw, n0 + h * TC, (s_) * BK, ws + h * TC * ROWB, wave, lane);                             \
        GTOS_VMCNT_LDS(0);                                                                                                    \
        __builtin_amdgcn_s_barrier();                                          \
        GTOS_KA_A(nxt, (s_) + 1);                                                                                             \
        __builtin_amdgcn_sched_barrier(0);                                                                                    \
        _Pragma("unroll") for (int ks = 0; ks < 2; ++ks) {                                                                    \
            bf16x8_t fa[2], fb[4];                                                                                            \
            _Pragma("unroll") for (int mt = 0; mt < 2; ++mt)                                                                  \
                fa[mt] = *reinterpret_cast<const bf16x8_t*>((cur) + lds_off(wave * 32 + mt * 16 + fr, ks * 4 + fq));          \
            _Pragma("unroll") for (int h = 0; h < NB; ++h) {                                                                  \
                if (h < nsub) {                                                                                               \
                    _Pragma("unroll") for (int nt = 0; nt < 4; ++nt)                                                          \
                        fb[nt] = *reinterpret_cast<const bf16x8_t*>(ws + h * TC * ROWB + lds_off(nt * 16 + fr, ks * 4 + fq)); \
                    _Pragma("unroll") for (int mt = 0; mt < 2; ++mt)                                                          \
                        _Pragma("unroll") for (int nt = 0; nt < 4; ++nt)                                                      \
                            acc[mt][h * 4 + nt] = __builtin_amdgcn_mfma_f32_16x16x32_bf16(fb[nt], fa[mt], acc[mt][h * 4 + nt], 0, 0, 0); \
                }                                                                                                             \
            }                                                                                                                 \
        }                                                                                                                     \
        GTOS_LGKM0();                                       \
        __builtin_amdgcn_s_barrier();                               \
    }
    GTOS_KA_A(a0, 0);
    int s = 0;
    for (; s + 2 <= nst; s += 2) {
        GTOS_KA_STEP(a0, a1, s);
        GTOS_KA_STEP(a1, a0, s + 1);
    }
    if (s < nst) GTOS_KA_STEP(a0, a1, s);
    GTOS_VMCNT(0);
    __builtin_amdgcn_s_barrier();
#undef GTOS_KA_STEP
#undef GTOS_KA_A
}

template <int NS>
__device__ __forceinline__ void dinp_tile(const StepBwdArgs& a, int m0, int n0, char* As, char* Bs, char* A1, int wave, int lane) {
    if (m0 >= a.rows_prev) return;
    const int fr = lane & 15, fq = lane >> 4, hs = a.hs;
    const U128* Z = static_cast<const U128*>(a.zeros);
    const int nsub = min(NS, (a.n_in - n0) / TC);
    f32x4_t acc[2][NS * 4];
#pragma unroll
    for (int i = 0; i < 2; ++i)
#pragma unroll
        for (int j = 0; j < NS * 4; ++j) acc[i][j] = f32x4_t{0.f, 0.f, 0.f, 0.f};
    kloop_a2<NS, false>(a.d4_prev, 4 * (int64_t)hs, a.rows_prev, m0, a.wi_t, 3 * (int64_t)hs, n0, nsub, hs, Z, As, A1, Bs, acc, wave, lane);
    const float ks_in = a.p_in > 0.f ? 1.f / (1.f - a.p_in) : 1.f;
    const uint64_t seed_in = a.p_in > 0.f ? live_seed(a.seed_in) : 0;
    Raw16 oldv[2][NS];
    if (a.dinp_acc) {
#pragma unroll
        for (int mt = 0; mt < 2; ++mt) {
            const int m = min(m0 + wave * 32 + mt * 16 + fr, a.rows_prev - 1);
#pragma unroll
            for (int h = 0; h < NS; ++h)
                if (h < nsub) oldv[mt][h] = ldraw16(a.dinp + (int64_t)m * a.ld_dinp + n0 + h * TC + fq * 16);
        }
    }
#pragma unroll
    for (int mt = 0; mt < 2; ++mt) {
        const int m = m0 + wave * 32 + mt * 16 + fr;
        if (m >= a.rows_prev) continue;
#pragma unroll
        for (int h = 0; h < NS; ++h) {
            if (h >= nsub) continue;
            const int nb = n0 + h * TC + fq * 16;
            float v[16];
#pragma unroll
            for (int i = 0; i < 16; ++i) v[i] = acc[mt][h * 4 + (i >> 2)][i & 3];
            if (a.p_in > 0.f) {
#pragma unroll
                for (int i = 0; i < 16; ++i)
                    v[i] = drop_keep(seed_in, (uint64_t)(a.in_drop_base + (int64_t)m * a.n_in + nb + i), a.p_in) ? v[i] * ks_in : 0.f;
            }
            bf16_t* dp = a.dinp + (int64_t)m * a.ld_dinp + nb;
            if (a.dinp_acc) {
                float old[16];
                unpack16(oldv[mt][h], old);
#pragma unroll
                for (int i = 0; i < 16; ++i) v[i] += old[i];
            }
            st16(dp, v);
        }
    }
}

template <int NS = 2>
__global__ __launch_bounds__(256, 3) void gru_step_bwd_kernel(StepBwdArgs a) {
    if (a.p_drop > 0.f) a.seed = live_seed(a.seed);
    __shared__ __attribute__((aligned(16))) char lds[A_BYTES];
    __shared__ __attribute__((aligned(16))) char lds_w[NS * TC * ROWB];
    __shared__ __attribute__((aligned(16))) char lds_a1[A_BYTES];
    __shared__ float btab[4 * TC];
    char* As = lds;
    char* Bs = lds_w;
    const int lane = threadIdx.x & 63, wave = __builtin_amdgcn_readfirstlane(threadIdx.x >> 6);
    const int fr = lane & 15, fq = lane >> 4;
    const int hs = a.hs, nC = hs / TC;
    const int nB = a.dinp ? (a.n_in + NS * TC - 1) / (NS * TC) : 0, per = nC + nB;
    const int xcd = blockIdx.x & 7, sq = blockIdx.x >> 3;
    const int m0 = ((sq / per) * 8 + xcd) * TM, role = sq % per;
    if (role >= nC) { dinp_tile<NS>(a, m0, (role - nC) * NS * TC, As, Bs, lds_a1, wave, lane); return; }
    const int c0 = role * TC;
    if (m0 >= a.rows) return;
    const U128* Z = static_cast<const U128*>(a.zeros);
    if (a.bias_part) { btab[threadIdx.x] = 0.f; }

    f32x4_t acc[2][4];
#pragma unroll
    for (int i = 0; i < 2; ++i)
#pragma unroll
        for (int j = 0; j < 4; ++j) acc[i][j] = f32x4_t{0.f, 0.f, 0.f, 0.f};

    if (a.d4_prev && a.sum_idx) {
        const RowSrc src = row_src(a.d4_prev, 4 * (int64_t)hs, a.rows, m0, wave, lane, a.sum_idx, a.zero_row);
        for (int kk = 0; kk < 3 * hs; kk += BK) {
            const int ak = kk < 2 * hs ? kk : kk + hs;
            dma_rows_at_z(src, ak, As, wave, lane);
            dma_wt(a.wh_t, 3 * (int64_t)hs, c0, kk, Bs, wave, lane);
            __syncthreads();
#pragma unroll
            for (int ks = 0; ks < 2; ++ks) {
                bf16x8_t fa[2], fb[4];
#pragma unroll
                for (int mt = 0; mt < 2; ++mt) fa[mt] = *reinterpret_cast<const bf16x8_t*>(As + lds_off(wave * 32 + mt * 16 + fr, ks * 4 + fq));
#pragma unroll
                for (int nt = 0; nt < 4; ++nt) fb[nt] = *reinterpret_cast<const bf16x8_t*>(Bs + lds_off(nt * 16 + fr, ks * 4 + fq));
#pragma unroll
                for (int mt = 0; mt < 2; ++mt)
#pragma unroll
                    for (int nt = 0; nt < 4; ++nt)
                        acc[mt][nt] = __builtin_amdgcn_mfma_f32_16x16x32_bf16(fb[nt], fa[mt], acc[mt][nt], 0, 0, 0);
            }
            __syncthreads();
        }
    } else if (a.d4_prev && m0 < a.rows_prev) {
        kloop_a2<1, true>(a.d4_prev, 4 * (int64_t)hs, a.rows_prev, m0, a.wh_t, 3 * (int64_t)hs, c0, 1, hs, Z, As, lds_a1, Bs, acc, wave, lane);
    } else if (a.bias_part) {
        __syncthreads();
    }

    const int cb = c0 + fq * 16;
    const float ks = a.p_drop > 0.f ? 1.f / (1.f - a.p_drop) : 1.f;
#pragma unroll
    for (int mt = 0; mt < 2; ++mt) {
        const int m_raw = m0 + wave * 32 + mt * 16 + fr;
        const bool valid = m_raw < a.rows;
        const int m = valid ? m_raw : a.rows - 1;
        float gr[16], gz[16], gn[16], hn[16], hp[16], g[16];
        const bf16_t* gp = a.gates + (int64_t)m * 4 * hs + cb;
        ld16(gp, gr); ld16(gp + hs, gz); ld16(gp + 2 * hs, gn);
        ld16(gp + 3 * hs, hn);
        ld16(a.hprev + (int64_t)(a.hprev_idx ? a.hprev_idx[m] : m) * hs + cb, hp);
        float* dhp = static_cast<float*>(a.dh) + (int64_t)m * a.ld_dh + cb;
        bf16_t* dhb = static_cast<bf16_t*>(a.dh) + (int64_t)m * a.ld_dh + cb;
        if (a.sum_idx) {
            const int64_t sr = a.sum_idx[m];
            if (sr == a.zero_row) {
#pragma unroll
                for (int i = 0; i < 16; ++i) g[i] = 0.f;
            } else if (a.dh_bf16) ld16(static_cast<const bf16_t*>(a.dh_src) + sr * hs + cb, g);
            else ldf16(static_cast<const float*>(a.dh_src) + sr * hs + cb, g);
        } else if (a.dh_bf16) ld16(dhb, g); else ldf16(dhp, g);
#pragma unroll
        for (int i = 0; i < 16; ++i) g[i] += acc[mt][i >> 2][i & 3];
        if (a.dy) {
            float dyv[16];
            ld16(a.dy + (int64_t)m * a.ldy + cb, dyv);
#pragma unroll
            for (int i = 0; i < 16; ++i) {
                float t2 = dyv[i];
                if (a.p_drop > 0.f) t2 = drop_keep(a.seed, (uint64_t)(a.drop_base + (int64_t)m * a.ldy + cb + i), a.p_drop) ? t2 * ks : 0.f;
                g[i] += t2;
            }
        }
        float dr_[16], dz_[16], dn_[16], dhn[16];
#pragma unroll
        for (int i = 0; i < 16; ++i) {
            const float dn = g[i] * (1.f - gz[i]);
            const float dz = g[i] * (hp[i] - gn[i]);
            dn_[i] = dn * (1.f - gn[i] * gn[i]);
            dhn[i] = dn_[i] * gr[i];
            dr_[i] = dn_[i] * hn[i] * gr[i] * (1.f - gr[i]);
            dz_[i] = dz * gz[i] * (1.f - gz[i]);
            g[i] *= gz[i];
            if (!valid) { dn_[i] = 0.f; dhn[i] = 0.f; dr_[i] = 0.f; dz_[i] = 0.f; }
        }
        if (valid) {
            if (a.dh_bf16) {
                st16(dhb, g);
            } else {
#pragma unroll
                for (int i = 0; i < 4; ++i)
                    *reinterpret_cast<float4*>(dhp + i * 4) = make_float4(g[i * 4], g[i * 4 + 1], g[i * 4 + 2], g[i * 4 + 3]);
            }
            bf16_t* dp = a.d4 + (int64_t)m * 4 * hs + cb;
            st16(dp, dr_); st16(dp + hs, dz_); st16(dp + 2 * hs, dn_); st16(dp + 3 * hs, dhn);
            if (a.hp_out) st16(a.hp_out + (int64_t)m * hs + cb, hp);
        }
        if (a.bias_part) {
#pragma unroll
            for (int i = 0; i < 16; ++i) {
                const float t0 = row16_sum(bf2f(f2bf(dr_[i]))), t1 = row16_sum(bf2f(f2bf(dz_[i])));
                const float t2 = row16_sum(bf2f(f2bf(dn_[i]))), t3 = row16_sum(bf2f(f2bf(dhn[i])));
                if (fr == 0) {
                    atomicAdd(&btab[0 * TC + fq * 16 + i], t0); atomicAdd(&btab[1 * TC + fq * 16 + i], t1);
                    atomicAdd(&btab[2 * TC + fq * 16 + i], t2); atomicAdd(&btab[3 * TC + fq * 16 + i], t3);
                }
            }
        }
    }
    if (a.bias_part) {
        __syncthreads();
        const int q = threadIdx.x >> 6, ch = threadIdx.x & 63;
        float* dst = a.bias_part + (int64_t)(blockIdx.x % a.n_partials) * 4 * hs + q * hs + c0 + ch;
        atomicAdd(dst, btab[threadIdx.x]);
    }
}


}

extern "C" int gtos_gru_step_fwd(int rows, int hs, const void* x, int64_t ldx, int in_dim, const void* w_ih, const float* b_ih,
                                 const void* xg, const void* gf, const int* gf_idx, const void* gb, const int* gb_idx,
                                 const void* h_in, const int* h_idx, const void* w_hh, const float* b_hh,
                                 void* h_out, int n_out, void* h_fin, int64_t ld_fin, const int* fin_idx, void* gates, void* y, int64_t ldy,
                                 float p_drop, uint64_t seed, int64_t drop_base, void* stream) {
    if (rows <= 0) return 0;
    if (hs <= 0 || hs % TC) return -22;
    if (!h_in || !w_hh || !b_hh || !gates) return -23;
    if ((n_out > 0 && !h_out) || (n_out < rows && !h_fin)) return -23;
    if (h_fin && (ld_fin < hs || ld_fin % 8)) return -25;
    const int mode = x ? 1 : (gf ? 2 : 0);
    if (mode == 1) {
        if (!w_ih || !b_ih || in_dim <= 0 || in_dim % 8 || ldx % 8 || (uintptr_t)x % 16 || (uintptr_t)w_ih % 16) return -24;
    } else if (mode == 2) {
        if (!gb || !gf_idx || !gb_idx || !b_ih || (uintptr_t)gf % 16 || (uintptr_t)gb % 16) return -24;
    } else if (!xg || (uintptr_t)xg % 16) return -24;
    if ((uintptr_t)h_in % 16 || (uintptr_t)w_hh % 16 || (uintptr_t)gates % 16 || (uintptr_t)h_out % 16 || (uintptr_t)h_fin % 16 ||
        (uintptr_t)b_hh % 16 || (uintptr_t)b_ih % 16) return -25;
    if (y && ((uintptr_t)y % 16 || ldy % 8)) return -25;
    StepArgs a;
    a.x = (const bf16_t*)x; a.ldx = ldx; a.in_dim = in_dim; a.w_ih = (const bf16_t*)w_ih; a.b_ih = b_ih; a.xg = (const bf16_t*)xg;
    a.gf = (const bf16_t*)gf; a.gf_idx = gf_idx; a.gb = (const bf16_t*)gb; a.gb_idx = gb_idx;
    a.h_in = (const bf16_t*)h_in; a.h_idx = h_idx; a.w_hh = (const bf16_t*)w_hh; a.b_hh = b_hh;
    a.h_out = (bf16_t*)h_out; a.n_out = n_out; a.h_fin = (bf16_t*)h_fin; a.gates = (bf16_t*)gates; a.y = (bf16_t*)y; a.ldy = ldy;
    a.ld_fin = ld_fin; a.fin_idx = fin_idx;
    a.p_drop = p_drop; a.seed = seed; a.drop_base = drop_base; a.rows = rows; a.hs = hs;
    a.zeros = gtos_zero_block();
    if (!a.zeros) return -5;
    const long long nM = (rows + TM - 1) / TM, nC = hs / TC;
    const long long nblk = ((nM + 7) / 8) * 8 * nC;
    if (nblk > 0x7fffffffLL) return -6;
    hipStream_t s = static_cast<hipStream_t>(stream);
    if (mode == 2 && hs == 256 && !h_idx && !y && rows >= 16384) {
        constexpr int KT = 4;
        const size_t lds_bytes = (size_t)KT * B_BYTES + 4 * KT * P_ROWS * ROWB;
        static bool configured = false;
        if (!configured) {
            if (hipFuncSetAttribute(reinterpret_cast<const void*>(gru_l1_fwd_persistent_kernel<KT>),
                                    hipFuncAttributeMaxDynamicSharedMemorySize, (int)lds_bytes) != hipSuccess) return -7;
            configured = true;
        }
        const int n_cu = 256, n_workers = n_cu / KT;
        hipLaunchKernelGGL(gru_l1_fwd_persistent_kernel<KT>, dim3(n_cu), dim3(256), lds_bytes, s, a, n_workers);
        GTOS_CHECK_LAUNCH();
        return 0;
    }
    static const bool use_a2w3 = !(getenv("GTOS_GRU_FWD_A2W3") && getenv("GTOS_GRU_FWD_A2W3")[0] == '0');
    if (mode == 1 && use_a2w3 && rows >= 8192 && in_dim % 64 == 0 && (in_dim / 64 + hs / 64) % 6 == 0 && !h_idx && ldx < (1 << 20) &&
        (int64_t)3 * hs * (in_dim > hs ? in_dim : hs) * 2 < (1LL << 31)) {
        const long long nM8 = (rows + 255) / 256, nblk8 = ((nM8 + 7) / 8) * 8 * nC;
        hipLaunchKernelGGL(gru_step_fwd_a2w3_kernel, dim3((unsigned)nblk8), dim3(512), 0, s, a);
    }
    else if (mode == 1) hipLaunchKernelGGL(gru_step_fwd_kernel<1>, dim3((unsigned)nblk), dim3(256), 0, s, a);
    else if (mode == 2) hipLaunchKernelGGL(gru_step_fwd_kernel<2>, dim3((unsigned)nblk), dim3(256), 0, s, a);
    else hipLaunchKernelGGL(gru_step_fwd_kernel<0>, dim3((unsigned)nblk), dim3(256), 0, s, a);
    GTOS_CHECK_LAUNCH();
    return 0;
}

extern "C" int gtos_gru_step_bwd_fused(int rows, int hs, const void* d4_prev, int rows_prev, const void* w_hh_t,
                                       const void* gates, const void* hprev, const int* hprev_idx, const void* dy, int64_t ldy,
                                       void* dh, int dh_dtype, int64_t ld_dh, void* d4, float p_drop, uint64_t seed, int64_t drop_base,
                                       float* bias_partials, int n_partials, void* hprev_out, const int* sum_idx, const void* dh_src,
                                       int zero_row,
                                       const void* w_ih_t, void* dinp, int64_t ld_dinp, int n_in, int dinp_accumulate, float p_in,
                                       uint64_t seed_in, int64_t in_drop_base, void* stream) {
    const bool role_b = dinp != nullptr && d4_prev != nullptr && rows_prev > 0;
    if (rows <= 0 && !role_b) return 0;
    if (hs <= 0 || hs % TC) return -22;
    if (rows > 0) {
        if (!gates || !hprev || !dh || !d4 || (d4_prev && !w_hh_t)) return -23;
        if (sum_idx && (!dh_src || (uintptr_t)dh_src % 16)) return -23;
    }
    if (dinp && (!d4_prev || !w_ih_t || sum_idx)) return -23;
    if (dinp && (n_in <= 0 || n_in % TC || ld_dinp < n_in || ld_dinp % 8 || (uintptr_t)dinp % 16 || (uintptr_t)w_ih_t % 16)) return -27;
    if (bias_partials && n_partials < 1) return -26;
    if ((uintptr_t)d4_prev % 16 || (uintptr_t)w_hh_t % 16 || (uintptr_t)gates % 16 || (uintptr_t)hprev % 16 || (uintptr_t)dh % 16 ||
        (uintptr_t)d4 % 16 || (dy && ((uintptr_t)dy % 16 || ldy % 8)) || (rows > 0 && (ld_dh < hs || ld_dh % 8)) ||
        (uintptr_t)hprev_out % 16) return -25;
    StepBwdArgs a;
    a.d4_prev = (const bf16_t*)d4_prev; a.rows_prev = d4_prev ? rows_prev : 0; a.wh_t = (const bf16_t*)w_hh_t;
    a.gates = (const bf16_t*)gates; a.hprev = (const bf16_t*)hprev; a.hprev_idx = hprev_idx; a.dy = (const bf16_t*)dy; a.ldy = ldy;
    a.dh = dh; a.dh_bf16 = dh_dtype == GTOS_BF16; a.ld_dh = ld_dh; a.d4 = (bf16_t*)d4; a.bias_part = bias_partials; a.n_partials = n_partials;
    a.hp_out = (bf16_t*)hprev_out; a.sum_idx = sum_idx; a.dh_src = dh_src; a.zero_row = sum_idx ? zero_row : -1;
    a.wi_t = (const bf16_t*)w_ih_t; a.dinp = role_b ? (bf16_t*)dinp : nullptr; a.ld_dinp = ld_dinp; a.n_in = n_in; a.dinp_acc = dinp_accumulate;
    a.p_in = p_in; a.seed_in = seed_in; a.in_drop_base = in_drop_base;
    a.p_drop = p_drop; a.seed = seed; a.drop_base = drop_base; a.rows = rows > 0 ? rows : 0; a.hs = hs;
    a.zeros = gtos_zero_block();
    if (!a.zeros) return -5;
    const long long cover = role_b && rows_prev > a.rows ? rows_prev : a.rows;
    const long long nM = (cover + TM - 1) / TM, per = hs / TC + (role_b ? (n_in + 2 * TC - 1) / (2 * TC) : 0);
    const long long nblk = ((nM + 7) / 8) * 8 * per;
    if (nblk > 0x7fffffffLL) return -6;
    hipLaunchKernelGGL(gru_step_bwd_kernel<2>, dim3((unsigned)nblk), dim3(256), 0, static_cast<hipStream_t>(stream), a);
    GTOS_CHECK_LAUNCH();
    return 0;
}

extern "C" int gtos_gru_step_bwd(int rows, int hs, const void* d4_prev, int rows_prev, const void* w_hh_t,
                                 const void* gates, const void* hprev, const int* hprev_idx, const void* dy, int64_t ldy, void* dh, int dh_dtype,
                                 int64_t ld_dh, void* d4, float p_drop, uint64_t seed, int64_t drop_base, float* bias_partials,
                                 int n_partials, void* hprev_out, const int* sum_idx, const void* dh_src, int zero_row, void* stream) {
    return gtos_gru_step_bwd_fused(rows, hs, d4_prev, rows_prev, w_hh_t, gates, hprev, hprev_idx, dy, ldy, dh, dh_dtype, ld_dh, d4,
                                   p_drop, seed, drop_base, bias_partials, n_partials, hprev_out, sum_idx, dh_src, zero_row,
                                   nullptr, nullptr, 0, 0, 0, 0.f, 0, 0, stream);
}

GTOS_SEED_EPOCH_SETTER(gru_step)
```

### gtos_amd/csrc/rowops.hip

```cpp
#include "common.h"

namespace {

constexpr int LN_MAXC = 2;

template <typename TX, typename TR, typename TY>
__global__ __launch_bounds__(256) void ln_fwd_kernel(int rows, int d, const TX* __restrict__ x, const TR* __restrict__ r,
                                                     float p_drop, uint64_t seed, const float* __restrict__ gamma,
                                                     const float* __restrict__ beta, float eps, TY* __restrict__ y, bf16_t* __restrict__ y2,
                                                     float* __restrict__ mean, float* __restrict__ rstd) {
    if (p_drop > 0.f) seed = live_seed(seed);
    const int lane = threadIdx.x & 63;
    const int row = blockIdx.x * 4 + (threadIdx.x >> 6);
    if (row >= rows) return;
    const float ks = p_drop > 0.f ? 1.f / (1.f - p_drop) : 1.f;
    float z[LN_MAXC][8];
    float s = 0.f;
#pragma unroll
    for (int cI = 0; cI < LN_MAXC; ++cI) {
        const int c = (cI * 64 + lane) * 8;
#pragma unroll
        for (int e = 0; e < 8; ++e) z[cI][e] = 0.f;
        if (c < d) {
            Vec8<TX>::load(x + (int64_t)row * d + c, z[cI]);
// ... 957 lines not shown
        const int64_t fit = workspace_bytes / table_bytes;
        if (nb > fit) nb = fit;
        partials = workspace;
    }
    const int64_t rpb = (n + nb - 1) / nb;
    dim3 grid((unsigned)((n + rpb - 1) / rpb)), block(256);
    const size_t sh = use_lds ? (size_t)table_bytes : 0;
#define GTOS_EMB_BWD(T, L) hipLaunchKernelGGL((embed_rows_bwd_kernel<T, L>), grid, block, sh, s, n, V, dim, dim_pad, tok, (const T*)dout, dtable, p_drop, seed, rpb, partials)
    if (dtype == GTOS_BF16) { if (use_lds) GTOS_EMB_BWD(bf16_t, true); else GTOS_EMB_BWD(bf16_t, false); }
    else { if (use_lds) GTOS_EMB_BWD(float, true); else GTOS_EMB_BWD(float, false); }
#undef GTOS_EMB_BWD
    GTOS_CHECK_LAUNCH();
    if (partials) {
        const int total = V * dim_pad;
        const int slices = grid.x >= 64 ? 16 : 1;
        hipLaunchKernelGGL(embed_reduce_kernel, dim3((total + 255) / 256, slices), dim3(256), 0, s, (int)grid.x, V, dim, dim_pad, partials, dtable);
        GTOS_CHECK_LAUNCH();
    }
    return 0;
}

extern "C" int gtos_segment_sum_rows(int n_chunks, const int* rows, const int* chunk_node, const int* chunk_start, const int* chunk_cnt,
                                     const int* chunk_slot, const void* src, const void* src2, int64_t ld_src, int width,
                                     void* dst, void* dst2, int64_t ld_dst, float* heavy, float* heavy2, void* stream) {
    if (n_chunks <= 0) return 0;
    if (width <= 0 || width % 8 || width > 1536 || ld_src % 8 || ld_dst % 8 || (uintptr_t)src % 16 || (uintptr_t)dst % 16 ||
        (uintptr_t)src2 % 16 || (uintptr_t)dst2 % 16) return -24;
    if (!chunk_node || !chunk_start || !chunk_cnt || !src || !dst || (chunk_slot && !heavy)) return -23;
    if (src2 && (!dst2 || (chunk_slot && !heavy2))) return -23;
    hipStream_t s = static_cast<hipStream_t>(stream);
    const int nblk = (n_chunks + 3) / 4;
    const dim3 grid((unsigned)(nblk < 4096 ? nblk : 4096)), block(256);
#define GTOS_SEG(S, Q) hipLaunchKernelGGL((seg_sum_kernel<S, Q>), grid, block, 0, s, n_chunks, rows, chunk_node, chunk_start, chunk_cnt, \
                                          chunk_slot, (const bf16_t*)src, (const bf16_t*)src2, ld_src, width, (bf16_t*)dst, (bf16_t*)dst2, \
                                          ld_dst, heavy, heavy2)
    if (src2) { if (width <= 512) GTOS_SEG(1, 2); else if (width <= 1024) GTOS_SEG(2, 2); else GTOS_SEG(3, 2); }
    else { if (width <= 512) GTOS_SEG(1, 1); else if (width <= 1024) GTOS_SEG(2, 1); else GTOS_SEG(3, 1); }
#undef GTOS_SEG
    GTOS_CHECK_LAUNCH();
    return 0;
}

extern "C" int gtos_segment_sum_stream(int n_chunks, int total_rows, const int* rows, const int* chunk_node, const int* chunk_start,
                                       const int* chunk_cnt, const int* chunk_slot, const int* wave_off, int n_waves, const void* src,
                                       int64_t ld_src, int width, void* dst, int64_t ld_dst, float* heavy, void* stream) {
    if (n_chunks <= 0 || n_waves <= 0) return 0;
    if (width <= 0 || width % 256 || width > 1536 || ld_src % 8 || ld_dst % 8 || (uintptr_t)src % 16 || (uintptr_t)dst % 16) return -24;
    if (!rows || !chunk_node || !chunk_start || !chunk_cnt || !wave_off || !src || !dst || (chunk_slot && !heavy) || total_rows <= 0) return -23;
    SegStreamArgs a;
    a.n_chunks = n_chunks; a.total_rows = total_rows; a.n_waves = n_waves;
    a.rows = rows; a.chunk_node = chunk_node; a.chunk_start = chunk_start; a.chunk_cnt = chunk_cnt; a.chunk_slot = chunk_slot;
    a.wave_off = wave_off; a.src = (const bf16_t*)src; a.ld_src = ld_src; a.dst = (bf16_t*)dst; a.ld_dst = ld_dst; a.heavy = heavy;
    hipStream_t s = static_cast<hipStream_t>(stream);
    const dim3 grid((unsigned)((n_waves + 3) / 4)), block(256);
#define GTOS_SEGS(S, H) hipLaunchKernelGGL((seg_sum_stream_kernel<S, H>), grid, block, 0, s, a.n_chunks, a.total_rows, a.n_waves, a.rows, \
        a.chunk_node, a.chunk_start, a.chunk_cnt, a.chunk_slot, a.wave_off, a.src, a.ld_src, a.dst, a.ld_dst, a.heavy)
    switch (width / 256) {
        case 1: GTOS_SEGS(0, true); break;
        case 2: GTOS_SEGS(1, false); break;
        case 3: GTOS_SEGS(1, true); break;
        case 4: GTOS_SEGS(2, false); break;
        case 5: GTOS_SEGS(2, true); break;
        default: GTOS_SEGS(3, false); break;
    }
#undef GTOS_SEGS
    GTOS_CHECK_LAUNCH();
    return 0;
}

extern "C" int gtos_segment_sum_finish(int n_heavy, const int* heavy_node, const float* heavy, int width, void* dst, int64_t ld_dst,
                                       void* stream) {
    if (n_heavy <= 0) return 0;
    if (width <= 0 || width % 8 || ld_dst % 8 || !heavy_node || !heavy || !dst) return -24;
    const int64_t n = (int64_t)n_heavy * (width / 8);
    hipLaunchKernelGGL(seg_finish_kernel, dim3((unsigned)((n + 255) / 256)), dim3(256), 0, static_cast<hipStream_t>(stream), n_heavy,
                       heavy_node, heavy, width, (bf16_t*)dst, ld_dst);
    GTOS_CHECK_LAUNCH();
    return 0;
}

extern "C" int gtos_segment_sum_ranges(int n_seg, const int* ranges, const void* src, int64_t ld_src, int width, void* dst, int64_t ld_dst,
                                       void* stream) {
    if (n_seg <= 0) return 0;
    if (width <= 0 || width % 8 || width > 1536 || ld_src % 8 || ld_dst % 8 || (uintptr_t)src % 16 || (uintptr_t)dst % 16) return -24;
    if (!ranges || !src || !dst) return -23;
    hipStream_t s = static_cast<hipStream_t>(stream);
    const dim3 grid((unsigned)((n_seg + 3) / 4)), block(256);
#define GTOS_SEG(S) hipLaunchKernelGGL(seg_sum_range_kernel<S>, grid, block, 0, s, n_seg, ranges, (const bf16_t*)src, ld_src, width, \
                                       (bf16_t*)dst, ld_dst)
    if (width <= 512) GTOS_SEG(1); else if (width <= 1024) GTOS_SEG(2); else GTOS_SEG(3);
#undef GTOS_SEG
    GTOS_CHECK_LAUNCH();
    return 0;
}

extern "C" int gtos_sqnorm(int64_t n, const float* g, float* out, void* stream) {
    if (n <= 0) return 0;
    hipStream_t s = static_cast<hipStream_t>(stream);
    hipLaunchKernelGGL(sqnorm_kernel, dim3(grid_for(n, 256 * 8)), dim3(256), 0, s, n, g, out);
    GTOS_CHECK_LAUNCH();
    return 0;
}

extern "C" int gtos_adam_step(int64_t n, float* p, const float* g, float* m, float* v, float lr, float beta1, float beta2,
                              float eps, float weight_decay, float gscale, const float* sqnorm, float max_norm,
                              void* bf16_mirror, void* stream) {
    if (n <= 0) return 0;
    hipStream_t s = static_cast<hipStream_t>(stream);
    hipLaunchKernelGGL(adam_kernel, dim3(grid_for(n, 256 * 4)), dim3(256), 0, s, n, p, g, m, v, lr, beta1, beta2, eps, weight_decay,
                       gscale, sqnorm, max_norm, (bf16_t*)bf16_mirror, (const float*)nullptr);
    GTOS_CHECK_LAUNCH();
    return 0;
}

extern "C" int gtos_adam_step_ctl(int64_t n, float* p, const float* g, float* m, float* v, const float* ctl, float beta1, float beta2,
                                  float eps, float weight_decay, float gscale, const float* sqnorm, float max_norm,
                                  void* bf16_mirror, void* stream) {
    if (n <= 0) return 0;
    if (!ctl) return -23;
    hipStream_t s = static_cast<hipStream_t>(stream);
    hipLaunchKernelGGL(adam_kernel, dim3(grid_for(n, 256 * 4)), dim3(256), 0, s, n, p, g, m, v, 0.f, beta1, beta2, eps, weight_decay,
                       gscale, sqnorm, max_norm, (bf16_t*)bf16_mirror, ctl);
    GTOS_CHECK_LAUNCH();
    return 0;
}

extern "C" int gtos_step_control(int phase, const float* loss, double* state, float* flag, int warmup_steps, int embed_dim,
                                 float* ctl, void* stream) {
    if ((phase != 0 && phase != 1) || !loss || !state || !flag || !ctl || warmup_steps < 1 || embed_dim < 1) return -23;
    hipLaunchKernelGGL(step_control_kernel, dim3(1), dim3(64), 0, static_cast<hipStream_t>(stream), phase, loss, state, flag,
                       (double)warmup_steps, (double)embed_dim, ctl);
    GTOS_CHECK_LAUNCH();
    return 0;
}

extern "C" int gtos_cast_f32_to_bf16(int64_t n, const float* src, void* dst, void* stream) {
    if (n <= 0) return 0;
    hipStream_t s = static_cast<hipStream_t>(stream);
    hipLaunchKernelGGL(cast_bf16_kernel, dim3(grid_for(n, 256 * 4)), dim3(256), 0, s, n, src, (bf16_t*)dst);
    GTOS_CHECK_LAUNCH();
    return 0;
}

extern "C" int gtos_transpose_batch_bf16(int n_mat, const int64_t* desc, const int* tile_start, int total_tiles, const void* src,
                                         void* dst, void* stream) {
    if (n_mat <= 0 || total_tiles <= 0) return 0;
    if (!desc || !tile_start || !src || !dst) return -23;
    hipLaunchKernelGGL(transpose_batch_kernel, dim3((unsigned)total_tiles), dim3(256), 0, static_cast<hipStream_t>(stream), n_mat, desc,
                       tile_start, (const bf16_t*)src, (bf16_t*)dst);
    GTOS_CHECK_LAUNCH();
    return 0;
}

extern "C" int gtos_set_seed_epoch(const void* epoch) {
    int rc = gtosi_gemm_set_seed_epoch(epoch);
    if (!rc) rc = gtosi_rel_attn_set_seed_epoch(epoch);
    if (!rc) rc = gtosi_attn_tile_set_seed_epoch(epoch);
    if (!rc) rc = gtosi_rowops_set_seed_epoch(epoch);
    if (!rc) rc = gtosi_gru_step_set_seed_epoch(epoch);
    if (!rc) rc = gtosi_tokenenc_set_seed_epoch(epoch);
    return rc;
}

extern "C" int gtos_abi_version(void) { return 25; }

GTOS_SEED_EPOCH_SETTER(rowops)
```

### gtos_amd/gru.py

```python
import contextlib
import os

import torch

from . import _lib
from ._lib import call, dt, ptr, stream
from .ops import (gemm, compute_weight, next_seed, weight_t, _grad_target, _splitk, side_stream as _side_stream, side_ok, defer_side_join, _Timed,
                  embed_bwd_workspace, _workspace, WORKSPACE_BYTES, note_memory)


def _cell_fwd(A, hs, xg, hg, h, y, y_off_elems, ldy, hprev, gates, p, seed, drop_base):
    yp = None if y is None else y.data_ptr() + y_off_elems * y.element_size()
    call("gtos_gru_cell_fwd", dt(xg), A, hs, ptr(xg), ptr(hg), ptr(h), yp, ldy, ptr(hprev), ptr(gates),
         float(p), seed, drop_base, stream())


N_BIAS_PARTIALS = 1024

FUSE = "x"
SIDE_STREAM = os.environ.get("GTOS_GRU_SIDE", "1") != "0"
SIDE_MIN_ROWS = 200000


def _step_fwd(A, hs, x, xg, h_in, wi, b_ih, wh, b_hh, h_out, n_out, h_fin, gates, y, y_off_elems, ldy, p, seed, drop_base,
              h_idx=None, gf=None, gf_idx=None, gb=None, gb_idx=None, fin_idx=None, tag=None):
    yp = None if y is None else y.data_ptr() + y_off_elems * y.element_size()
    need_bi = x is not None or gf is not None
    name = tag or "gru_step_fwd_%s" % ("x" if x is not None else ("tables" if gf is not None else "xg"))
    units = A if tag is None else A * 2 * (x.shape[1] + hs + 4 * hs + hs + (hs if y is not None else 0))
    with _Timed(name, detail=True, units=units):
        _step_fwd_call(A, hs, x, xg, h_in, wi, b_ih, wh, b_hh, h_out, n_out, h_fin, gates, yp, ldy, p, seed, drop_base,
                       h_idx, gf, gf_idx, gb, gb_idx, need_bi, fin_idx)


def _step_fwd_call(A, hs, x, xg, h_in, wi, b_ih, wh, b_hh, h_out, n_out, h_fin, gates, yp, ldy, p, seed, drop_base,
                   h_idx, gf, gf_idx, gb, gb_idx, need_bi, fin_idx=None):
    call("gtos_gru_step_fwd", A, hs, ptr(x), 0 if x is None else x.stride(0), 0 if x is None else x.shape[1],
         ptr(wi) if x is not None else None, ptr(b_ih) if need_bi else None, ptr(xg),
         ptr(gf), ptr(gf_idx), ptr(gb), ptr(gb_idx), ptr(h_in), ptr(h_idx), ptr(wh), ptr(b_hh),
         ptr(h_out), n_out, ptr(h_fin), hs if h_fin is None else h_fin.stride(0), ptr(fin_idx), ptr(gates), yp, ldy,
         float(p), seed, drop_base, stream())


def _step_bwd(A, hs, d4_prev, rows_prev, wh_t, gates, hprev, dy_ptr, ldy, dh, d4, p, seed, drop_base, bpart, hprev_idx=None, hp_out=None,
              sum_idx=None, dh_src=None, zero_row=-1):
    with _Timed("gru_step_bwd_%s" % ("trie" if hprev_idx is not None else "rows"), detail=True, units=A):
        call("gtos_gru_step_bwd", A, hs, ptr(d4_prev), rows_prev if d4_prev is not None else 0, ptr(wh_t), ptr(gates), ptr(hprev),
             ptr(hprev_idx), dy_ptr, ldy, ptr(dh), dt(dh), dh.stride(0), ptr(d4), float(p), seed, drop_base,
             ptr(bpart), N_BIAS_PARTIALS if bpart is not None else 0, ptr(hp_out), ptr(sum_idx), ptr(dh_src), int(zero_row), stream())


def _cell_bwd(A, hs, gates, hprev, dy, dy_off_elems, ldy, dh, dxg, dhg, p, seed, drop_base, bpart):
    dyp = None if dy is None else dy.data_ptr() + dy_off_elems * dy.element_size()
    call("gtos_gru_cell_bwd", dt(gates), A, hs, ptr(gates), ptr(hprev), dyp, ldy, ptr(dh), ptr(dxg), ptr(dhg),
         float(p), seed, drop_base, ptr(bpart), 0 if bpart is None else bpart.shape[0], stream())


class BiGRUFinalFn(torch.autograd.Function):

    @staticmethod
    def forward(ctx, x, batch_sizes, hs, num_layers, p_drop, *weights):
        L, R = len(batch_sizes), batch_sizes[0]
        offs = [0]
        for a in batch_sizes:
            offs.append(offs[-1] + a)
        N = offs[-1]
        assert x.shape[0] == N
        dev, dtp = x.device, x.dtype
        inp = x.contiguous()
        saved = []
        finals = None
        for l in range(num_layers):
            last = l == num_layers - 1
            Y = None if last else torch.empty((N, 2 * hs), dtype=dtp, device=dev)
            seed = next_seed() if (p_drop > 0 and not last) else 0
            pl = p_drop if not last else 0.0
            finals = []
            layer_saved = []
            for direction in (0, 1):
                w_ih, w_hh, b_ih, b_hh = weights[l * 8 + direction * 4: l * 8 + direction * 4 + 4]
                wi, wh = compute_weight(w_ih, dtp), compute_weight(w_hh, dtp)
                gates = torch.empty((N, 4 * hs), dtype=dtp, device=dev)
                hprev = torch.empty((N, hs), dtype=dtp, device=dev)
                steps = range(L) if direction == 0 else range(L - 1, -1, -1)
                fuse = FUSE if (dtp == torch.bfloat16 and hs % 64 == 0 and inp.shape[1] % 8 == 0) else "off"
                if fuse != "off":
                    h = torch.empty((R, hs), dtype=dtp, device=dev)
                    xg = None if fuse == "x" else gemm(inp, wi, trans_b=True, bias=b_ih.detach())
                    bi, bh = b_ih.detach(), b_hh.detach()
                    if direction == 0:
                        hprev[:R].zero_()
                    else:
                        for t in range(L):
                            lo = batch_sizes[t + 1] if t + 1 < L else 0
                            if batch_sizes[t] > lo:
                                hprev[offs[t] + lo: offs[t] + batch_sizes[t]].zero_()
                    for t in steps:
                        A, off = batch_sizes[t], offs[t]
                        nxt = t + 1 if direction == 0 else t - 1
                        if 0 <= nxt < L:
                            h_out, n_out = hprev[offs[nxt]:], min(A, batch_sizes[nxt])
                        else:
                            h_out, n_out = h, A
                        _step_fwd(A, hs, inp[off:off + A] if fuse == "x" else None, None if fuse == "x" else xg[off:off + A],
                                  hprev[off:off + A], wi, bi, wh, bh, h_out, n_out, h, gates[off:off + A],
                                  Y, off * 2 * hs + direction * hs, 2 * hs, pl, seed, off * 2 * hs + direction * hs)
                else:
                    xg = gemm(inp, wi, trans_b=True, bias=b_ih.detach())
                    h = torch.zeros((R, hs), dtype=dtp, device=dev)
                    hg = torch.empty((R, 3 * hs), dtype=dtp, device=dev)
                    for t in steps:
                        A, off = batch_sizes[t], offs[t]
                        gemm(h[:A], wh, trans_b=True, bias=b_hh.detach(), out=hg[:A])
                        _cell_fwd(A, hs, xg[off:off + A], hg, h, Y, off * 2 * hs + direction * hs, 2 * hs,
                                  hprev[off:off + A], gates[off:off + A], pl, seed, off * 2 * hs + direction * hs)
                finals.append(h)
                layer_saved.append((weight_t(w_ih, wi), weight_t(w_hh, wh), gates, hprev))
            saved.append((inp, seed, pl, layer_saved))
            inp = Y
        ctx.cfg = (batch_sizes, offs, hs, num_layers, weights, saved)
        return torch.cat(finals, 1)

    @staticmethod
    def backward(ctx, d_out):
        with _Timed("relation_gru_bwd"):
            return BiGRUFinalFn._backward(ctx, d_out)

    @staticmethod
    def _backward(ctx, d_out):
        batch_sizes, offs, hs, num_layers, weights, saved = ctx.cfg
        L, R, N = len(batch_sizes), batch_sizes[0], offs[-1]
        d_out = d_out.contiguous()
        dev = d_out.device
        grads = [None] * len(weights)
        used_side = False
        dY = None
        for l in range(num_layers - 1, -1, -1):
            inp, seed, pl, layer_saved = saved[l]
            dtp = inp.dtype
            d_inp = None
            for direction in (0, 1):
                wi_t, wh_t, gates, hprev = layer_saved[direction]
                base = l * 8 + direction * 4
                w_ih, w_hh, b_ih, b_hh = weights[base:base + 4]
                steps = range(L - 1, -1, -1) if direction == 0 else range(L)
                want_bias = b_ih.requires_grad or b_hh.requires_grad
                fused = FUSE != "off" and dtp == torch.bfloat16 and hs % 64 == 0
                dh_dt = dtp if fused else torch.float32
                if l == num_layers - 1:
                    dh = d_out[:, direction * hs:(direction + 1) * hs].to(dh_dt).contiguous()
                else:
                    dh = torch.zeros((R, hs), dtype=dh_dt, device=dev)
                if fused:
                    d4 = torch.empty((N, 4 * hs), dtype=dtp, device=dev)
                    bpart = torch.zeros((N_BIAS_PARTIALS, 4 * hs), dtype=torch.float32, device=dev) if want_bias else None
                    prev = None
                    for t in steps:
                        A, off = batch_sizes[t], offs[t]
                        dyp = None if dY is None else dY.data_ptr() + (off * 2 * hs + direction * hs) * dY.element_size()
                        _step_bwd(A, hs, None if prev is None else d4[offs[prev]:], 0 if prev is None else batch_sizes[prev], wh_t,
                                  gates[off:off + A], hprev[off:off + A], dyp, 2 * hs, dh, d4[off:off + A], pl, seed,
                                  off * 2 * hs + direction * hs, bpart)
                        prev = t
                    dxg = d4[:, :3 * hs]
                    w_jobs = ((w_hh, d4[:, :2 * hs], hprev, 1, slice(0, 2 * hs)), (w_hh, d4[:, 3 * hs:], hprev, 1, slice(2 * hs, 3 * hs)),
                              (w_ih, dxg, inp, 0, slice(0, 3 * hs)))
                else:
                    dxg = torch.empty((N, 3 * hs), dtype=dtp, device=dev)
                    dhg = torch.empty((N, 3 * hs), dtype=dtp, device=dev)
                    fuse_bias = (256 % (hs // 8) == 0) and want_bias
                    bpart = torch.zeros((N_BIAS_PARTIALS, 4 * hs), dtype=torch.float32, device=dev) if fuse_bias else None
                    for t in steps:
                        A, off = batch_sizes[t], offs[t]
                        _cell_bwd(A, hs, gates[off:off + A], hprev[off:off + A], dY, off * 2 * hs + direction * hs, 2 * hs,
                                  dh, dxg[off:off + A], dhg[off:off + A], pl, seed, off * 2 * hs + direction * hs, bpart)
                        gemm(dhg[off:off + A], wh_t, trans_b=True, out=dh[:A], accumulate=True)
                    w_jobs = ((w_hh, dhg, hprev, 1, slice(0, 3 * hs)), (w_ih, dxg, inp, 0, slice(0, 3 * hs)))
                for (wt, _, _, slot, _) in w_jobs:
                    if wt.requires_grad and _grad_target(wt) is None and grads[base + slot] is None:
                        grads[base + slot] = torch.zeros(wt.shape, dtype=torch.float32, device=dev)
                for (bt, slot) in ((b_hh, 3), (b_ih, 2)):
                    if bt.requires_grad and _grad_target(bt) is None:
                        grads[base + slot] = torch.zeros(bt.shape, dtype=torch.float32, device=dev)
                main = torch.cuda.current_stream(dev)
                side = _side_stream(dev) if (SIDE_STREAM and side_ok(dev) and fused and N >= SIDE_MIN_ROWS) else main
                if side is not main:
                    side.wait_stream(main)
                    for t_ in (d4, bpart, hprev, inp):
                        if t_ is not None:
                            t_.record_stream(side)
                with torch.cuda.stream(side):
                    for (wt, dyv, xin, slot, rows) in w_jobs:
                        if wt.requires_grad:
                            tgt = _grad_target(wt)
                            if tgt is None:
                                tgt = grads[base + slot]
                            nrow = rows.stop - rows.start
                            gemm(dyv, xin, trans_a=True, out=tgt[rows], accumulate=True, splitk=_splitk(nrow, wt.shape[1], N))
                    bsum = bpart.sum(0) if bpart is not None else None
                    for (bt, slot) in ((b_hh, 3), (b_ih, 2)):
                        if bt.requires_grad:
                            tgt = _grad_target(bt)
                            if tgt is None:
                                tgt = grads[base + slot]
                            if bsum is not None:
                                tgt[:2 * hs] += bsum[:2 * hs]
                                tgt[2 * hs:] += bsum[2 * hs:3 * hs] if slot == 2 else bsum[3 * hs:]
                            else:
                                dyv = dhg if slot == 3 else dxg
                                call("gtos_colsum", dt(dyv), N, 3 * hs, 3 * hs, ptr(dyv), ptr(tgt), stream())
                used_side = used_side or side is not main
                if l > 0 or ctx.needs_input_grad[0]:
                    if d_inp is None:
                        d_inp = gemm(dxg, wi_t, trans_b=True)
                    else:
                        gemm(dxg, wi_t, trans_b=True, out=d_inp, accumulate=True)
            dY = d_inp
        if used_side:
            if all(gr is None for gr in grads):
                defer_side_join(dev)
            else:
                torch.cuda.current_stream(dev).wait_stream(_side_stream(dev))
        return (dY if ctx.needs_input_grad[0] else None, None, None, None, None) + tuple(grads)


class PackPlan(object):

    def __init__(self, batch_sizes, order32, order64=None):
        self.batch_sizes = [int(a) for a in batch_sizes if a > 0]
        self.offs = [0]
        for a in self.batch_sizes:
            self.offs.append(self.offs[-1] + a)
        self.L, self.N = len(self.batch_sizes), self.offs[-1]
        self.order32 = order32
        self.order64 = order64 if order64 is not None else order32.to(torch.int64)
        self.offs_dev = torch.tensor(self.offs, dtype=torch.int32).to(order32.device, non_blocking=True)

    @staticmethod
    def of_trie(trie):
        plan = getattr(trie, "_pack_plan", None)
        if plan is None or plan.order32.device != trie.seq_order32.device:
            plan = trie._pack_plan = PackPlan(trie.batch_sizes, trie.seq_order32, trie.seq_order)
        return plan

    @staticmethod
    def of_lengths(lengths, max_len):
        sorted_len, order = torch.sort(lengths, descending=True, stable=True)
        bs = (sorted_len.unsqueeze(0) > torch.arange(max_len, device=lengths.device).unsqueeze(1)).sum(1).tolist()
        return PackPlan(bs, order.to(torch.int32), order)


def _step_bwd_fused(A, hs, d4_prev, rows_prev, wh_t, gates, hprev, dy_ptr, ldy, dh, d4, p, seed, drop_base, bpart,
                    wi_t=None, dinp=None, n_in=0, dinp_acc=False, p_in=0.0, seed_in=0, in_drop_base=0, tag="gru_step_bwd_packed"):
    rp = rows_prev if d4_prev is not None else 0
    both = min(A, rp) if dinp is not None else 0
    nbytes = 2 * (A * (4 * hs + hs + 2 * hs + 4 * hs + (hs if dy_ptr else 0)) + both * 4 * hs
                  + ((rp - both) * 3 * hs if dinp is not None else min(A, rp) * 3 * hs) + (rp * n_in * (2 if dinp_acc else 1) if dinp is not None else 0))
    with _Timed(tag, detail=True, units=nbytes):
        call("gtos_gru_step_bwd_fused", A, hs, ptr(d4_prev), rows_prev if d4_prev is not None else 0, ptr(wh_t), ptr(gates), ptr(hprev), None,
             dy_ptr, ldy, ptr(dh), 0 if dh is None else dt(dh), hs if dh is None else dh.stride(0), ptr(d4), float(p), seed, drop_base,
             ptr(bpart), N_BIAS_PARTIALS if bpart is not None else 0, None, None, None, -1,
             ptr(wi_t), ptr(dinp), 0 if dinp is None else dinp.stride(0), n_in, int(dinp_acc), float(p_in), seed_in, in_drop_base, stream())


D4_INPLACE = os.environ.get("GTOS_GRU_D4_INPLACE", "auto")
D4_INPLACE_MIN_BYTES = 8 << 30


class PackedPathGRUFn(torch.autograd.Function):

    @staticmethod
    def forward(ctx, bank, plan, table, dim_pad, p_embed, hs, p_layer, *weights):
        dev, dtp = table.device, torch.bfloat16
        bs, offs, L, N = plan.batch_sizes, plan.offs, plan.L, plan.N
        R = bank.shape[1]
        if L == 0 or R == 0:
            ctx.cfg = False
            return torch.zeros((R, 2 * hs), dtype=dtp, device=dev)
        V, dim = table.shape
        tab = table.detach()
        want_table = table.requires_grad and ctx.needs_input_grad[2]
        Vp = (V + 7) // 8 * 8
        X = torch.empty((N, dim_pad), dtype=dtp, device=dev)
        onehot = torch.empty((N, Vp), dtype=dtp, device=dev) if (want_table and V <= 256) else None
        tokens = torch.empty((N,), dtype=torch.int64, device=dev) if (want_table and V > 256) else None
        seed_e = next_seed() if p_embed > 0 else 0
        call("gtos_embed_packed_paths", dt(X), L, R, N, ptr(bank), ptr(plan.order32), ptr(plan.offs_dev), ptr(tab), dim, dim_pad, ptr(X),
             float(p_embed), seed_e, ptr(onehot), Vp, ptr(tokens), stream())
        fin = (torch.empty if bs[0] == R else torch.zeros)((R, 2 * hs), dtype=dtp, device=dev)
        park = [torch.empty((bs[0], hs), dtype=dtp, device=dev) for _ in (0, 1)]
        inp, saved = X, []
        for l in range(2):
            last = l == 1
            Y = None if last else torch.empty((N, 2 * hs), dtype=dtp, device=dev)
            seed = next_seed() if (p_layer > 0 and not last) else 0
            pl = p_layer if not last else 0.0
            layer_saved = []
            bufs = [(torch.empty((N, 4 * hs), dtype=dtp, device=dev), torch.empty((N, hs), dtype=dtp, device=dev)) for _ in (0, 1)]
            wts = []
            for direction in (0, 1):
                w_ih, w_hh, b_ih, b_hh = weights[l * 8 + direction * 4: l * 8 + direction * 4 + 4]
                wi, wh = compute_weight(w_ih, dtp), compute_weight(w_hh, dtp)
                if wi.shape[1] != inp.shape[1]:
                    wi = torch.nn.functional.pad(wi.detach(), (0, inp.shape[1] - wi.shape[1]))
                    wi_t = wi.t().contiguous()
                else:
                    wi_t = weight_t(w_ih, wi)
                wts.append((wi, wh, wi_t, weight_t(w_hh, wh), b_ih.detach(), b_hh.detach()))
            for direction in (0, 1):
                wi, wh, wi_t, wh_t, bi, bh = wts[direction]
                gates, hprev = bufs[direction]
                if direction == 0:
                    hprev[:bs[0]].zero_()
                else:
                    for t in range(L):
                        lo = bs[t + 1] if t + 1 < L else 0
                        if bs[t] > lo:
                            hprev[offs[t] + lo: offs[t] + bs[t]].zero_()
                h_fin = fin[:, direction * hs:(direction + 1) * hs] if last else park[direction]
                for t in (range(L) if direction == 0 else range(L - 1, -1, -1)):
                    A, off = bs[t], offs[t]
                    nxt = t + 1 if direction == 0 else t - 1
                    if 0 <= nxt < L:
                        h_out, n_out = hprev[offs[nxt]:], min(A, bs[nxt])
                    else:
                        h_out, n_out = None, 0
                    _step_fwd(A, hs, inp[off:off + A], None, hprev[off:off + A], wi, bi, wh, bh, h_out, n_out, h_fin, gates[off:off + A],
                              Y, off * 2 * hs + direction * hs, 2 * hs, pl, seed, off * 2 * hs + direction * hs,
                              fin_idx=plan.order32 if last else None, tag="gru_step_fwd_packed_l%d" % l)
                layer_saved.append((wi_t, wh_t, gates, hprev))
            saved.append((inp, seed, pl, layer_saved))
            inp = Y
        ctx.cfg = (plan, table, dim_pad, p_embed, seed_e, hs, weights, saved, onehot, tokens)
        return fin

    @staticmethod
    def backward(ctx, d_out):
        with _Timed("relation_gru_bwd"):
            return PackedPathGRUFn._backward(ctx, d_out)

    @staticmethod
    def _backward(ctx, d_out):
        if ctx.cfg is False:
            return (None,) * len(ctx.needs_input_grad)
        if ctx.cfg is None:
            raise RuntimeError("PackedPathGRUFn: backward called a second time -- the saved gates and states are released piece by piece "
                               "during the first (retain_graph is not supported on this path)")
        plan, table, dim_pad, p_embed, seed_e, hs, weights, saved, onehot, tokens = ctx.cfg
        bs, offs, L, N = plan.batch_sizes, plan.offs, plan.L, plan.N
        dev, dtp = d_out.device, torch.bfloat16
        dfin = d_out.to(dtp).index_select(0, plan.order64)
        grads = [None] * len(weights)
        for base in (8, 12, 0, 4):
            for slot in range(4):
                wt_ = weights[base + slot]
                if wt_.requires_grad and _grad_target(wt_) is None:
                    grads[base + slot] = torch.zeros(wt_.shape, dtype=torch.float32, device=dev)
        want_table = onehot is not None or tokens is not None
        main = torch.cuda.current_stream(dev)
        used_side, held = False, None
        dY = None
        dX = None
        saved = [list(e) for e in saved]
        ctx.cfg = None
        for l in (1, 0):
            inp, seed, pl, layer_saved = saved[l]
            saved[l] = None
            layer_saved = list(layer_saved)
            n_in = inp.shape[1]
            want_dinp = l == 1 or want_table
            d_in = torch.empty((N, n_in), dtype=dtp, device=dev) if want_dinp else None
            for direction in (0, 1):
                wi_t, wh_t, gates, hprev = layer_saved[direction]
                layer_saved[direction] = None
                base = l * 8 + direction * 4
                w_ih, w_hh, b_ih, b_hh = weights[base:base + 4]
                want_bias = b_ih.requires_grad or b_hh.requires_grad
                dh = dfin[:, direction * hs:(direction + 1) * hs] if l == 1 else torch.zeros((bs[0], hs), dtype=dtp, device=dev)
                in_place = D4_INPLACE == "1" or (D4_INPLACE != "0" and gates.numel() * gates.element_size() >= D4_INPLACE_MIN_BYTES)
                d4 = gates if in_place else torch.empty((N, 4 * hs), dtype=dtp, device=dev)
                note_memory(dev)
                bpart = torch.zeros((N_BIAS_PARTIALS, 4 * hs), dtype=torch.float32, device=dev) if want_bias else None
                rb = dict(wi_t=wi_t, n_in=n_in, dinp_acc=direction == 1, p_in=p_embed if l == 0 else 0.0,
                          seed_in=seed_e if l == 0 else 0) if want_dinp else None
                tag = "gru_step_bwd_packed_l%d" % l
                prev = None
                for t in (range(L - 1, -1, -1) if direction == 0 else range(L)):
                    A, off = bs[t], offs[t]
                    dyp = None if dY is None else dY.data_ptr() + (off * 2 * hs + direction * hs) * dY.element_size()
                    kw = {} if (rb is None or prev is None) else dict(rb, dinp=d_in[offs[prev]:], in_drop_base=offs[prev] * n_in)
                    _step_bwd_fused(A, hs, None if prev is None else d4[offs[prev]:], 0 if prev is None else bs[prev], wh_t,
                                    gates[off:off + A], hprev[off:off + A], dyp, 2 * hs, dh, d4[off:off + A], pl, seed,
                                    off * 2 * hs + direction * hs, bpart, tag=tag, **kw)
                    prev = t
                if rb is not None:
                    _step_bwd_fused(0, hs, d4[offs[prev]:], bs[prev], wh_t, None, None, None, 2 * hs, None, None, 0.0, 0, 0, None, tag=tag,
                                    **dict(rb, dinp=d_in[offs[prev]:], in_drop_base=offs[prev] * n_in))
                del gates
                side = _side_stream(dev) if (SIDE_STREAM and side_ok(dev) and N >= SIDE_MIN_ROWS) else main
                if held is not None:
                    main.wait_stream(_side_stream(dev))
                    held = None
                if side is not main:
                    side.wait_stream(main)
                    held = (d4, bpart, hprev, inp)
                with torch.cuda.stream(side):
                    tg_ih = _grad_target(w_ih) if w_ih.requires_grad else None
                    tg_hh = _grad_target(w_hh) if w_hh.requires_grad else None
                    tg_ih = grads[base] if (tg_ih is None and w_ih.requires_grad) else tg_ih
                    tg_hh = grads[base + 1] if (tg_hh is None and w_hh.requires_grad) else tg_hh
                    scr_ih = torch.zeros(w_ih.shape, dtype=torch.float32, device=dev) if tg_ih is None else tg_ih
                    scr_hh = torch.zeros(w_hh.shape, dtype=torch.float32, device=dev) if tg_hh is None else tg_hh
                    if (tg_ih is not None or tg_hh is not None) and w_ih.shape[1] % 4 == 0:
                        with _Timed("gru_dw_grouped_l%d" % l, detail=True, units=2 * N * 3 * hs * (w_ih.shape[1] + hs)):
                            ws = _workspace(dev)
                            call("gtos_gru_weight_grads", N, hs, n_in, w_ih.shape[1], ptr(d4), ptr(inp), inp.stride(0), ptr(hprev), hprev.stride(0),
                                 ptr(scr_ih), scr_ih.stride(0), ptr(scr_hh), scr_hh.stride(0), ptr(ws), ws.numel() * 4, stream())
                    elif tg_ih is not None or tg_hh is not None:
                        for (tg, dyv, xin, rows) in ((tg_hh, d4[:, :2 * hs], hprev, slice(0, 2 * hs)), (tg_hh, d4[:, 3 * hs:], hprev, slice(2 * hs, 3 * hs)),
                                                     (tg_ih, d4[:, :3 * hs], inp, slice(0, 3 * hs))):
                            if tg is None:
                                continue
                            sk = _splitk(rows.stop - rows.start, xin.shape[1], N)
                            if tg.shape[1] == xin.shape[1]:
                                gemm(dyv, xin, trans_a=True, out=tg[rows], accumulate=True, splitk=sk)
                            else:
                                tg[rows] += gemm(dyv, xin, trans_a=True, out_dtype=torch.float32, splitk=sk)[:, :tg.shape[1]]
                    if want_bias:
                        _acc_bias_grads(grads, base, b_ih, b_hh, bpart.sum(0), hs)
                used_side = used_side or side is not main
                del d4, hprev, bpart
            del inp
            if l == 1:
                dY = d_in
            else:
                dX, dY = d_in, None
        dtab = None
        if want_table:
            tgt = _grad_target(table)
            if tgt is None:
                tgt = dtab = torch.zeros(table.shape, dtype=torch.float32, device=dev)
            V, dim = table.shape
            if onehot is not None:
                part = gemm(onehot, dX, trans_a=True, out_dtype=torch.float32, splitk=_splitk(onehot.shape[1], dim_pad, N))
                tgt += part[:V, :dim]
            else:
                ws = embed_bwd_workspace(N, V, dim_pad, dev)
                call("gtos_embed_rows_bwd", dt(dX), N, V, dim, dim_pad, ptr(tokens), ptr(dX), ptr(tgt), 0.0, 0, ptr(ws),
                     0 if ws is None else ws.numel() * 4, stream())
        if used_side:
            if dtab is None and all(gr is None for gr in grads):
                defer_side_join(dev, list(t_ for t_ in (held or ()) if t_ is not None))
            else:
                main.wait_stream(_side_stream(dev))
        return (None, None, dtab, None, None, None, None) + tuple(grads)


def packed_path_gru(bank, plan, table, dim_pad, p_embed, hs, p_layer, weights):
    return PackedPathGRUFn.apply(bank, plan, table, dim_pad, float(p_embed), hs, float(p_layer), *weights)


def bigru_final(x_packed, batch_sizes, hs, num_layers, p_drop, weights):
    return BiGRUFinalFn.apply(x_packed, tuple(batch_sizes), hs, num_layers, float(p_drop), *weights)


TRIE = os.environ.get("GTOS_GRU_TRIE", "1") != "0"
TRIE_SIDE = False
TRIE_L0_OVERLAP = True
EMBED_GRAD_GEMM = True
TRIE_SUM_INDEX = True


SEG_STREAM = True


def _seg_rows(side, src, width, dst, src2=None, dst2=None):
    heavy = torch.zeros((2 if src2 is not None else 1, max(1, side.n_heavy), width), dtype=torch.float32, device=src.device)
    if SEG_STREAM and src2 is None and width % 256 == 0:
        with _Timed("segment_sum_rows", detail=True, units=int(side.rows.numel())):
            call("gtos_segment_sum_stream", side.n_chunks, int(side.rows.numel()), ptr(side.rows), ptr(side.chunk_node), ptr(side.chunk_start),
                 ptr(side.chunk_cnt), ptr(side.chunk_slot), ptr(side.wave_off), side.n_waves, ptr(src), src.stride(0), width, ptr(dst),
                 dst.stride(0), ptr(heavy[0]), stream())
            call("gtos_segment_sum_finish", side.n_heavy, ptr(side.heavy_node), ptr(heavy[0]), width, ptr(dst), dst.stride(0), stream())
        return
    with _Timed("segment_sum_rows", detail=True, units=int(side.rows.numel()) * (2 if src2 is not None else 1)):
        call("gtos_segment_sum_rows", side.n_chunks, ptr(side.rows), ptr(side.chunk_node), ptr(side.chunk_start), ptr(side.chunk_cnt),
             ptr(side.chunk_slot), ptr(src), ptr(src2), src.stride(0), width, ptr(dst), ptr(dst2), dst.stride(0),
             ptr(heavy[0]), ptr(heavy[1]) if src2 is not None else None, stream())
        call("gtos_segment_sum_finish", side.n_heavy, ptr(side.heavy_node), ptr(heavy[0]), width, ptr(dst), dst.stride(0), stream())
        if src2 is not None:
            call("gtos_segment_sum_finish", side.n_heavy, ptr(side.heavy_node), ptr(heavy[1]), width, ptr(dst2), dst2.stride(0), stream())


def _seg_ranges(n_seg, ranges, src, width, dst):
    call("gtos_segment_sum_ranges", n_seg, ptr(ranges), ptr(src), src.stride(0), width, ptr(dst), dst.stride(0), stream())


def _acc_weight_grad(grads, slot, wt, dy, x, rows=None, cols=None):
    if not wt.requires_grad:
        return
    tgt = _grad_target(wt)
    if tgt is None:
        if grads[slot] is None:
            grads[slot] = torch.zeros(wt.shape, dtype=torch.float32, device=dy.device)
        tgt = grads[slot]
    if rows is not None:
        tgt = tgt[rows]
    if cols is not None:
        tgt = tgt[:, cols]
    gemm(dy, x, trans_a=True, out=tgt, accumulate=True, splitk=_splitk(dy.shape[1], x.shape[1], dy.shape[0]))


def _acc_bias_grads(grads, base, b_ih, b_hh, bsum, hs):
    for bt, slot in ((b_hh, 3), (b_ih, 2)):
        if not bt.requires_grad:
            continue
        tgt = _grad_target(bt)
        if tgt is None:
            if grads[base + slot] is None:
                grads[base + slot] = torch.zeros(bt.shape, dtype=torch.float32, device=bsum.device)
            tgt = grads[base + slot]
        tgt[:2 * hs] += bsum[:2 * hs]
        tgt[2 * hs:] += bsum[2 * hs:3 * hs] if slot == 2 else bsum[3 * hs:]


class TrieBiGRUFn(torch.autograd.Function):

    @staticmethod
    def forward(ctx, trie, table, dim_pad, p_embed, hs, p_layer, *weights):
        dev, dtp = table.device, torch.bfloat16
        L, R, N = trie.L, trie.R, trie.N
        bs = trie.batch_sizes
        offs = [0]
        for a in bs:
            offs.append(offs[-1] + a)
        sides = (trie.pf, trie.sf)
        dim = table.shape[1]
        tab = table.detach()
        l0 = []
        main = torch.cuda.current_stream(dev)
        aux = _side_stream(dev) if (TRIE_L0_OVERLAP and table.is_cuda and side_ok(dev) and N >= SIDE_MIN_ROWS) else main
        seeds = [(next_seed() if p_embed > 0 else 0, next_seed() if p_layer > 0 else 0) for _ in sides]
        if aux is not main:
            aux.wait_stream(main)
        for d, side in enumerate(sides):
            with torch.cuda.stream(aux if d == 1 else main):
                n = side.n_nodes
                w_ih, w_hh, b_ih, b_hh = weights[d * 4: d * 4 + 4]
                wi, wh = compute_weight(w_ih, dtp), compute_weight(w_hh, dtp)
                seed_e, seed_y = seeds[d]
                X = torch.empty((n, dim_pad), dtype=dtp, device=dev)
                call("gtos_embed_rows_fwd", dt(X), n, dim, dim_pad, ptr(side.tok), ptr(tab), ptr(X), float(p_embed), seed_e, stream())
                H = torch.empty((n + 1, hs), dtype=dtp, device=dev)
                H[n].zero_()
                gates = torch.empty((n, 4 * hs), dtype=dtp, device=dev)
                Y = torch.empty((n, hs), dtype=dtp, device=dev) if p_layer > 0 else None
                bi, bh = b_ih.detach(), b_hh.detach()
                for k in range(L):
                    lo, hi = side.level_off[k], side.level_off[k + 1]
                    if hi > lo:
                        _step_fwd(hi - lo, hs, X[lo:hi], None, H, wi, bi, wh, bh, H[lo:hi], hi - lo, None, gates[lo:hi],
                                  Y, lo * hs, hs, p_layer, seed_y, lo * hs, h_idx=side.par[lo:hi])
                l0.append((X, H, gates, Y, seed_e, seed_y, weight_t(w_ih, wi), weight_t(w_hh, wh)))
        if aux is not main:
            main.wait_stream(aux)
        src = [l0[d][3] if p_layer > 0 else l0[d][1][:sides[d].n_nodes] for d in (0, 1)]
        fin = torch.empty((R, 2 * hs), dtype=dtp, device=dev)
        l1 = []
# ... 212 lines not shown
```

### include/gtos_hip.h

```cpp
#ifndef GTOS_HIP_H
#define GTOS_HIP_H
#include <stdint.h>

#ifdef __cplusplus
extern "C" {
#endif

#define GTOS_F32 0
#define GTOS_BF16 1

int gtos_abi_version(void);

int gtos_gemm(int in_dtype, int out_dtype, int transA, int transB, int M, int N, int K,
              const void* A, int64_t lda, const void* B, int64_t ldb, void* C, int64_t ldc,
              const float* bias, int relu, float p_drop, uint64_t seed, int accumulate, int splitk,
              void* workspace, int64_t workspace_bytes, void* stream);

int gtos_rel_attn_fwd(int dtype, int mode, int T, int S, int B, int H, int d,
                      const void* q, int64_t ldq, const void* k, int64_t ldk, const void* v, int64_t ldv,
                      const void* rel, const int* idx_q, const uint8_t* key_pad, const uint8_t* attn_mask,
                      float scale, float p_drop, uint64_t seed,
                      void* o, int64_t ldo, float* lse, float* w, void* stream);

int gtos_rel_attn_bwd(int dtype, int mode, int T, int S, int B, int H, int d,
                      const void* q, int64_t ldq, const void* k, int64_t ldk, const void* v, int64_t ldv,
                      const void* rel, const int* idx_q, const int* idx_k,
                      const uint8_t* key_pad, const uint8_t* attn_mask,
                      float scale, float p_drop, uint64_t seed,
                      const void* o, int64_t ldo, const float* lse, const float* w,
                      const void* d_o, int64_t lddo, const float* dw,
                      void* dq, int64_t lddq, void* dk, int64_t lddk, void* dv, int64_t lddv,
                      void* d_rel, int64_t ld_drel, float* pd, float* gs, void* stream);

int gtos_rel_attn_bwd_bank(int dtype, int n, int B, int H, int d,
                           const void* q, int64_t ldq, const void* k, int64_t ldk,
                           const void* bank, const float* gs,
                           const int* pair_sorted, const int* chunk_type, const int* chunk_start,
                           const int* chunk_count, const int* chunk_slot, const int* xcd_off, int nchunks,
                           void* d_bank, int64_t ld_dbank, float* heavy, void* stream);

int gtos_pathtrie_dev_workspace(int64_t R, int64_t N, int64_t* bytes_out);
int gtos_pathtrie_dev_phase_a(int L, int64_t R, const int64_t* bank, const int64_t* length, void** common, void** pf, void** sf,
                              int32_t* sizes, void* workspace, size_t workspace_bytes, void* stream);
int gtos_pathtrie_dev_phase_b(int64_t R, int64_t N, int n_pf, int n_sf, int chunk, int rows_per_wave, void** common, void** pf,
                              void** sf, int32_t* sizes, void* workspace, size_t workspace_bytes, void* stream);

int gtos_relbatch_dev_workspace(int64_t total, int64_t* bytes_out);
int gtos_relbatch_dev_phase_a(const int64_t* geom, void** tab, void* workspace, size_t workspace_bytes, void* stream);
int gtos_relbatch_dev_phase_b(const int64_t* geom, int64_t R, void** tab, void* workspace, size_t workspace_bytes, void* stream);
int gtos_relbatch_dev_all_count(const int64_t* geom, void** tab, void* workspace, size_t workspace_bytes, void* stream);
int gtos_relbatch_dev_all_keys(const int64_t* geom, void** tab, void* workspace, size_t workspace_bytes, void* stream);
int gtos_relbatch_dev_all_fill(const int64_t* geom, int64_t R, void** tab, void* workspace, size_t workspace_bytes, void* stream);

int gtos_relindex_dev_workspace(int64_t n, int64_t* bytes_out);
int gtos_relindex_dev_phase_a(const int64_t* geom, void** tab, void* workspace, size_t workspace_bytes, void* stream);
int gtos_relindex_dev_phase_b(const int64_t* geom, int64_t nchunks, void** tab, void* workspace, size_t workspace_bytes, void* stream);

int gtos_ln_residual_fwd(int dtype, int rows, int d, const void* x, const void* r, float p_drop, uint64_t seed,
                         const float* gamma, const float* beta, float eps, void* y, float* mean, float* rstd, void* stream);
int gtos_ln_residual_bwd(int dtype, int rows, int d, const void* dy, const void* x, const void* r, float p_drop,
                         uint64_t seed, const float* gamma, const float* mean, const float* rstd,
                         void* dx, void* dr, float* dgamma, float* dbeta, void* stream);

int gtos_ln_residual_fwd2(int x_dtype, int r_dtype, int y_dtype, int rows, int d, const void* x, const void* r, float p_drop,
                          uint64_t seed, const float* gamma, const float* beta, float eps, void* y, void* y2_bf16,
                          float* mean, float* rstd, void* stream);
int gtos_ln_residual_bwd2(int x_dtype, int r_dtype, int y_dtype, int rows, int d, const void* dy, const void* dy2_bf16,
                          const void* x, const void* r, float p_drop, uint64_t seed, const float* gamma, const float* mean,
                          const float* rstd, void* dx, void* dr, float* dgamma, float* dbeta, void* stream);

int gtos_relu_dropout_bwd(int dtype, int64_t n, void* dh, const void* h, float p_drop, void* stream);

int gtos_colsum(int dtype, int rows, int N, int64_t ld, const void* dy, float* out, void* stream);

int gtos_gru_cell_fwd(int dtype, int rows, int hs, const void* xg, const void* hg, void* h, void* y, int64_t ldy,
                      void* hprev_save, void* gates, float p_drop, uint64_t seed, int64_t drop_base, void* stream);
int gtos_gru_step_fwd(int rows, int hs, const void* x, int64_t ldx, int in_dim, const void* w_ih, const float* b_ih,
                      const void* xg, const void* gf, const int* gf_idx, const void* gb, const int* gb_idx,
                      const void* h_in, const int* h_idx, const void* w_hh, const float* b_hh,
                      void* h_out, int n_out, void* h_fin, int64_t ld_fin, const int* fin_idx, void* gates, void* y, int64_t ldy,
                      float p_drop, uint64_t seed, int64_t drop_base, void* stream);

int gtos_gru_step_bwd(int rows, int hs, const void* d4_prev, int rows_prev, const void* w_hh_t,
                      const void* gates, const void* hprev, const int* hprev_idx, const void* dy, int64_t ldy, void* dh, int dh_dtype,
                      int64_t ld_dh, void* d4, float p_drop, uint64_t seed, int64_t drop_base, float* bias_partials, int n_partials,
                      void* hprev_out, const int* sum_idx, const void* dh_src, int zero_row, void* stream);

int gtos_gru_step_bwd_fused(int rows, int hs, const void* d4_prev, int rows_prev, const void* w_hh_t,
                            const void* gates, const void* hprev, const int* hprev_idx, const void* dy, int64_t ldy, void* dh, int dh_dtype,
                            int64_t ld_dh, void* d4, float p_drop, uint64_t seed, int64_t drop_base, float* bias_partials, int n_partials,
                            void* hprev_out, const int* sum_idx, const void* dh_src, int zero_row,
                            const void* w_ih_t, void* dinp, int64_t ld_dinp, int n_in, int dinp_accumulate, float p_in, uint64_t seed_in,
                            int64_t in_drop_base, void* stream);

int gtos_gru_weight_grads(int rows, int hs, int in_dim, int in_valid, const void* d4, const void* x, int64_t ldx, const void* hprev, int64_t ldh,
                          float* dwih, int64_t ld_dwih, float* dwhh, int64_t ld_dwhh, void* workspace, int64_t workspace_bytes, void* stream);

int gtos_gemm_tn_batch(int n, const void* const* A, const int64_t* lda, const int* M, const void* const* B, const int64_t* ldb, const int* N,
                       const int* K, float* const* C, const int64_t* ldc, float* const* bias, void* stream);

int gtos_segment_sum_rows(int n_chunks, const int* rows, const int* chunk_node, const int* chunk_start, const int* chunk_cnt,
                          const int* chunk_slot, const void* src, const void* src2, int64_t ld_src, int width,
                          void* dst, void* dst2, int64_t ld_dst, float* heavy, float* heavy2, void* stream);
int gtos_segment_sum_stream(int n_chunks, int total_rows, const int* rows, const int* chunk_node, const int* chunk_start,
                            const int* chunk_cnt, const int* chunk_slot, const int* wave_off, int n_waves, const void* src,
                            int64_t ld_src, int width, void* dst, int64_t ld_dst, float* heavy, void* stream);
int gtos_segment_sum_finish(int n_heavy, const int* heavy_node, const float* heavy, int width, void* dst, int64_t ld_dst,
                            void* stream);
int gtos_segment_sum_ranges(int n_seg, const int* ranges, const void* src, int64_t ld_src, int width, void* dst, int64_t ld_dst,
                            void* stream);

int gtos_gru_cell_bwd(int dtype, int rows, int hs, const void* gates, const void* hprev, const void* dy, int64_t ldy,
                      float* dh, void* dxg, void* dhg, float p_drop, uint64_t seed, int64_t drop_base,
                      float* bias_partials, int n_partials, void* stream);

int gtos_relation_gather_mean(int dtype, int64_t P, int K, int d, const void* bank, const int64_t* idx, int zero_row0,
                              void* out, void* stream);

int gtos_embed_rows_fwd(int dtype, int64_t n, int dim, int dim_pad, const int64_t* tok, const float* table, void* out,
                        float p_drop, uint64_t seed, void* stream);
int gtos_embed_rows_bwd(int dtype, int64_t n, int V, int dim, int dim_pad, const int64_t* tok, const void* dout,
                        float* dtable, float p_drop, uint64_t seed, float* workspace, int64_t workspace_bytes, void* stream);

int gtos_embed_packed_paths(int dtype, int L, int R, int64_t n_rows, const int64_t* bank, const int* order, const int* offs,
                            const float* table, int dim, int dim_pad, void* x, float p_drop, uint64_t seed, void* onehot, int vp,
                            int64_t* tokens, void* stream);

int gtos_highway_fwd(int dtype, int64_t N, int D, const void* y, const void* x, void* out, void* stream);
int gtos_highway_bwd(int dtype, int64_t N, int D, const void* y, const void* x, const void* dout, void* dy, void* dx, void* stream);
int gtos_max_relu_fwd(int dtype, int64_t N, int L, int F, const void* y, void* out, uint8_t* arg, void* stream);
int gtos_max_relu_bwd(int dtype, int64_t N, int L, int F, const void* out, const uint8_t* arg, const void* dout, void* dy, void* stream);
int gtos_token_row_fwd(int dtype, int64_t N, int Cc, int Ct, int Cp, const void* feat, const int64_t* tok, const float* table,
                       void* out, float p_drop, uint64_t seed, void* stream);
int gtos_token_row_bwd(int dtype, int64_t N, int Cc, int Ct, int Cp, const void* dout, const int64_t* tok, void* dfeat,
                       float* dtable, float p_drop, uint64_t seed, void* stream);

int gtos_sqnorm(int64_t n, const float* g, float* out, void* stream);
int gtos_adam_step(int64_t n, float* p, const float* g, float* m, float* v, float lr, float beta1, float beta2,
                   float eps, float weight_decay, float gscale, const float* sqnorm, float max_norm,
                   void* bf16_mirror, void* stream);
int gtos_cast_f32_to_bf16(int64_t n, const float* src, void* dst, void* stream);
int gtos_transpose_batch_bf16(int n_mat, const int64_t* desc, const int* tile_start, int total_tiles, const void* src, void* dst,
                              void* stream);

int gtos_step_control(int phase, const float* loss, double* state, float* flag, int warmup_steps, int embed_dim,
                      float* ctl, void* stream);

int gtos_set_seed_epoch(const void* epoch);
int gtos_adam_step_ctl(int64_t n, float* p, const float* g, float* m, float* v, const float* ctl, float beta1, float beta2,
                       float eps, float weight_decay, float gscale, const float* sqnorm, float max_norm,
                       void* bf16_mirror, void* stream);

int gtos_copy_nll_fwd(int dtype, int T, int B, int V, int S, const void* logits, int64_t ld_logits, const void* div,
                      const float* align, const int64_t* cp_seq, const int64_t* target, int64_t pad_idx,
                      float* nll, float* lse, float* p_tgt, void* stream);
int gtos_copy_nll_bwd(int dtype, int T, int B, int V, int S, const void* logits, int64_t ld_logits, const void* div,
                      const float* align, const int64_t* cp_seq, const int64_t* target, int64_t pad_idx,
                      const float* lse, const float* p_tgt, const float* d_nll, void* d_logits, void* d_div,
                      float* d_align, void* stream);
int gtos_copy_ll_fwd(int dtype, int T, int B, int V, int S, int tot_ext, const void* logits, int64_t ld_logits,
                     const void* div, const float* align, const int64_t* cp_seq, float* ll, void* stream);

int gtos_copy_nll_ls_prep(int B, int S, int V, const int64_t* cp_seq, int* ws, int64_t ws_words, void* stream);
int gtos_copy_nll_ls_fwd(int dtype, int T, int B, int V, int S, const void* logits, int64_t ld_logits, const void* div,
                         const float* align, const int64_t* target, int64_t pad_idx, float eps, const int* ws, int64_t ws_words,
                         float* loss, float* lse, float* sums, void* stream);
int gtos_copy_nll_ls_bwd(int dtype, int T, int B, int V, int S, const void* logits, int64_t ld_logits, const void* div,
                         const float* align, const int64_t* target, int64_t pad_idx, float eps, const int* ws, int64_t ws_words,
                         const float* lse, const float* sums, const float* d_loss, void* d_logits, void* d_div, float* d_align,
                         void* stream);

int gtos_copy_eval_fwd(int dtype, int T, int B, int V, int S, const void* logits, int64_t ld_logits, const void* div,
                       const float* align, const int64_t* cp_seq, const int64_t* target, int64_t pad_idx, float* nll,
                       int* pred, float* p_pred, void* stream);
int gtos_eval_accumulate(int T, int B, const float* nll, const int* pred, const int64_t* target, int64_t pad_idx,
                         double* sent_nll, int* sent_tokens, int* sent_correct, double* totals, void* stream);

int gtos_beam_topk(int rows, int tot, int k, const float* ll, int64_t ld, float* val, int* idx, void* stream);
int gtos_beam_advance(int B, int k, int t, int V, int tot, int min_time_step, int max_time_step, const float* topv,
                      const int* topi, const uint8_t* flag_shared, const uint8_t* flag_local, double* slot_score,
                      int* beam_state, int* bp_parent, int* bp_token, int* comp_step, int* comp_parent,
                      double* comp_score, int* active, void* stream);
int gtos_beam_reorder(int n_caches, void* const* src, void* const* dst, int64_t row_bytes, int N, int k, int t,
                      int max_time_step, const int* bp_parent, const int* bp_token, const int* beam_state,
                      const int* active, int V, int tot, const int64_t* tok_shared, const int64_t* tok_local,
                      const int64_t* char_shared, const int64_t* char_local, int C, int64_t dead_tok,
                      const int64_t* dead_char, int64_t* tok_out, int64_t* char_out, void* stream);

int gtos_sample_step(int N, int k, int t, int V, int tot, int min_time_step, int max_time_step, float temperature, int top_k,
                     float top_p, uint64_t seed, const float* ll, int64_t ld, const uint8_t* flag_shared,
                     const uint8_t* flag_local, const uint8_t* owned_local, double* score, int* slot_state, int* tokens,
                     int* active, const int64_t* tok_shared, const int64_t* tok_local, const int64_t* char_shared,
                     const int64_t* char_local, int C, int64_t dead_tok, const int64_t* dead_char, int64_t* tok_out,
                     int64_t* char_out, void* stream);

#ifdef __cplusplus
}
#endif
#endif
```

Measured before the change: 861.5.

## Skip known-zero GRU hidden-state rows in step kernels and weight-grad GEMM

Adds a host-side plan of which packed hidden-state rows are zero (the initial state at each timestep), announced to the kernels through thread-local side channels. The forward and backward step kernels no longer load those rows and drop the recurrent GEMM for all-zero tiles. The grouped weight-gradient GEMM skips K ranges covering zero rows. A new range-zeroing kernel replaces per-timestep zero_() calls and the parked final-state buffers. The cost is more complex bookkeeping and a thread-local handoff that only holds if the announce call directly precedes the launch with a matching pointer.

New measurement: 858.9. No clear change (-0.3%).

```diff
diff --git a/gtos_amd/_lib.py b/gtos_amd/_lib.py
--- a/gtos_amd/_lib.py
+++ b/gtos_amd/_lib.py
@@ -6,7 +6,7 @@
 
 _HERE = os.path.dirname(os.path.abspath(__file__))
 LIB_PATH = os.path.join(_HERE, "csrc", "libgtos_hip.so")
-ABI_VERSION = 25
+ABI_VERSION = 26
 
 c_p, c_i, c_l, c_f, c_u64 = ctypes.c_void_p, ctypes.c_int, ctypes.c_int64, ctypes.c_float, ctypes.c_uint64
 
@@ -38,9 +38,12 @@
     "gtos_gru_cell_fwd": [c_i, c_i, c_i, c_p, c_p, c_p, c_p, c_l, c_p, c_p, c_f, c_u64, c_l, c_p],
     "gtos_gru_step_fwd": [c_i, c_i, c_p, c_l, c_i, c_p, c_p, c_p, c_p, c_p, c_p, c_p, c_p, c_p, c_p, c_p, c_p, c_i, c_p, c_l, c_p, c_p, c_p, c_l,
                           c_f, c_u64, c_l, c_p],
+    "gtos_gru_step_zero_rows": [c_p, c_i],
     "gtos_gru_step_bwd": [c_i, c_i, c_p, c_i, c_p, c_p, c_p, c_p, c_p, c_l, c_p, c_i, c_l, c_p, c_f, c_u64, c_l, c_p, c_i, c_p, c_p, c_p, c_i, c_p],
     "gtos_gru_step_bwd_fused": [c_i, c_i, c_p, c_i, c_p, c_p, c_p, c_p, c_p, c_l, c_p, c_i, c_l, c_p, c_f, c_u64, c_l, c_p, c_i, c_p, c_p, c_p, c_i,
                                 c_p, c_p, c_l, c_i, c_i, c_f, c_u64, c_l, c_p],
+    "gtos_gru_weight_grads_zero_rows": [c_p, c_p, c_i],
+    "gtos_zero_row_ranges": [c_p, c_i, c_i, c_l, c_p, c_i, c_p],
     "gtos_gru_weight_grads": [c_i, c_i, c_i, c_i, c_p, c_p, c_l, c_p, c_l, c_p, c_l, c_p, c_l, c_p, c_l, c_p],
     "gtos_gemm_tn_batch": [c_i, c_p, c_p, c_p, c_p, c_p, c_p, c_p, c_p, c_p, c_p, c_p],
     "gtos_embed_packed_paths": [c_i, c_i, c_i, c_l, c_p, c_p, c_p, c_p, c_i, c_i, c_p, c_f, c_u64, c_p, c_i, c_p, c_p],
diff --git a/gtos_amd/csrc/gemm.hip b/gtos_amd/csrc/gemm.hip
--- a/gtos_amd/csrc/gemm.hip
+++ b/gtos_amd/csrc/gemm.hip
@@ -815,10 +815,13 @@
     return 0;
 }
 
+constexpr int TN_MAX_SKIP = 48;
 struct TnGroup {
     const bf16_t* B1; int64_t ldb1; int N1;
     int tiles;
     int tmn[64];
+    int nskip;
+    int skip[2 * TN_MAX_SKIP];
 };
 
 struct TnJob { const bf16_t* A; const bf16_t* B; float* C; int lda, ldb, ldc, M, N, K, tile_end, nN; };
@@ -843,7 +846,7 @@
     int bz = (sq / tiles) * 8 + xcd, t_ = sq % tiles;
     if constexpr (MODE == 2) { bz = 0; t_ = blockIdx.x; if (t_ >= g.ntiles) return; }
     if (bz >= a.splitk) return;
-    int m0, n0, Nv;
+    int m0, n0, Nv, nsk = 0;
     const bf16_t* Bp;
     int64_t ldb, wld;
     float* wst;
@@ -860,6 +863,7 @@
         const int e = g.tmn[t_], src = (e >> 8) & 255;
         m0 = (e & 255) * BM2; n0 = ((e >> 16) & 255) * BN2;
         Bp = src ? g.B1 : static_cast<const bf16_t*>(a.B); ldb = src ? g.ldb1 : a.ldb; Nv = src ? g.N1 : a.N;
+        nsk = src ? g.nskip : 0;
         wst = a.ws + ((int64_t)bz * tiles + t_) * (BM2 * BN2); wld = BN2;
     } else {
         m0 = (t_ / nN) * BM2; n0 = (t_ % nN) * BN2;
@@ -869,7 +873,12 @@
     const int ktiles = (a.K + 63) / 64, tps = (ktiles + a.splitk - 1) / a.splitk;
     const int kbeg = bz * tps * 64, kend = min(a.K, kbeg + tps * 64);
     if (kbeg >= kend) return;
-    const int nk = (kend - kbeg + 31) / 32;
+    int nk = (kend - kbeg + 31) / 32;
+    int jcur = kbeg >> 5, si = 0;
+    if constexpr (GROUPED) {
+        const int jend = jcur + nk;
+        for (int i = 0; i < nsk; ++i) nk -= max(0, min(g.skip[2 * i + 1], jend) - max(g.skip[2 * i], jcur));
+    }
     const char* Z = static_cast<const char*>(a.zeros);
     const int kr = lane >> 5, pp = lane & 31;
     const int kl0 = 2 * wave + kr, kq_d = kl0 & 3;
@@ -894,6 +903,14 @@
                                      (__attribute__((address_space(3))) void*)(dst), 16, 0, 0)
 #define GTOS_DMA4(stage)                                                                                                      \
     {                                                                                                                         \
+        if constexpr (GROUPED) {                            \
+            while (si < nsk && jcur >= g.skip[2 * si]) {                                                                      \
+                const int d_ = g.skip[2 * si + 1] - jcur;                                                                     \
+                if (d_ > 0) { jcur += d_; kcur += 32 * d_; pa += 2 * a16 * d_; pb += 2 * b16 * d_; }                          \
+                ++si;                                                                                                         \
+            }                                                                                                                 \
+            ++jcur;                                                                                                           \
+        }                                                                                                                     \
         const bool ok0 = kcur < kend, ok1 = kcur + 16 < kend;                                                                 \
         GTOS_DMA1(ok0 ? pa : Z, (stage) + wave * 1024);                                                                       \
         GTOS_DMA1(ok1 ? pa + a16 : Z, (stage) + (8 + wave) * 1024);                                                           \
@@ -1132,9 +1149,25 @@
 }
 
 
+namespace { thread_local struct { const void* hprev; int n; int r[2 * TN_MAX_SKIP]; } t_zero_rows = {nullptr, 0, {0}}; }
+
+extern "C" int gtos_gru_weight_grads_zero_rows(const void* hprev, const int* ranges, int n_ranges) {
+    t_zero_rows.hprev = nullptr; t_zero_rows.n = 0;
+    if (n_ranges <= 0 || !hprev) return 0;
+    if (!ranges || n_ranges > TN_MAX_SKIP) return -22;
+    for (int i = 0; i < n_ranges; ++i)
+        if (ranges[2 * i] < 0 || ranges[2 * i + 1] < ranges[2 * i] || (i && ranges[2 * i] < ranges[2 * i - 1])) return -22;
+    for (int i = 0; i < 2 * n_ranges; ++i) t_zero_rows.r[i] = ranges[i];
+    t_zero_rows.hprev = hprev; t_zero_rows.n = n_ranges;
+    return 0;
+}
+
 extern "C" int gtos_gru_weight_grads(int rows, int hs, int in_dim, int in_valid, const void* d4, const void* x, int64_t ldx, const void* hprev, int64_t ldh,
                                      float* dwih, int64_t ld_dwih, float* dwhh, int64_t ld_dwhh, void* workspace, int64_t workspace_bytes,
                                      void* stream) {
+    const bool announced = t_zero_rows.hprev != nullptr && t_zero_rows.hprev == hprev;
+    const int n_zero = announced ? t_zero_rows.n : 0;
+    t_zero_rows.hprev = nullptr;
     if (rows <= 0) return 0;
     if (hs <= 0 || hs % 64 || in_dim < 8 || in_dim % 8 || ldx < in_dim || ldx % 8 || ldh < hs || ldh % 8 || in_valid < 1 || in_valid > in_dim ||
         in_valid % 4) return -22;
@@ -1162,6 +1195,11 @@
         }
     }
     g.tiles = nt;
+    for (int i = 0; i < n_zero; ++i) {
+        const int lo = t_zero_rows.r[2 * i], hi = t_zero_rows.r[2 * i + 1] < rows ? t_zero_rows.r[2 * i + 1] : rows;
+        const int js = (lo + 31) / 32, je = hi >= rows ? (rows + 31) / 32 : hi / 32;
+        if (je > js) { g.skip[2 * g.nskip] = js; g.skip[2 * g.nskip + 1] = je; ++g.nskip; }
+    }
     const int ktiles = (rows + 63) / 64;
     const long long tile_bytes = (long long)BM2 * BN2 * 4;
     long long sk = 8LL * (32 / nt > 0 ? 32 / nt : 1);
diff --git a/gtos_amd/csrc/gru_step.hip b/gtos_amd/csrc/gru_step.hip
--- a/gtos_amd/csrc/gru_step.hip
+++ b/gtos_amd/csrc/gru_step.hip
@@ -29,6 +29,7 @@
     int64_t ld_fin; const int* fin_idx;
     float p_drop; uint64_t seed; int64_t drop_base;
     int rows, hs; const void* zeros;
+    int n_live;
 };
 
 __device__ __forceinline__ void dma_rows(const bf16_t* __restrict__ base, const U128* __restrict__ zeros, int64_t ld, int rows_total,
@@ -214,7 +215,12 @@
             const bf16_t* xp = a.xg + (int64_t)m * 3 * hs + cb;
             ld16(xp, xr); ld16(xp + hs, xz); ld16(xp + 2 * hs, xn);
         }
-        ld16(a.h_in + (int64_t)(a.h_idx ? a.h_idx[m] : m) * hs + cb, hp);
+        if (m < a.n_live) {
+            ld16(a.h_in + (int64_t)(a.h_idx ? a.h_idx[m] : m) * hs + cb, hp);
+        } else {
+#pragma unroll
+            for (int i = 0; i < 16; ++i) hp[i] = 0.f;
+        }
         float gr[16], gz[16], gn[16], hn[16], o[16];
 #pragma unroll
         for (int i = 0; i < 16; ++i) {
@@ -228,9 +234,8 @@
         bf16_t* gp = a.gates + (int64_t)m * 4 * hs + cb;
         st16(gp, gr); st16(gp + hs, gz); st16(gp + 2 * hs, gn);
         st16(gp + 3 * hs, hn);
-        bf16_t* hdst = m < a.n_out ? a.h_out + (int64_t)m * hs + cb
-                                   : a.h_fin + (int64_t)(a.fin_idx ? a.fin_idx[m] : m) * a.ld_fin + cb;
-        st16(hdst, o);
+        if (m < a.n_out) st16(a.h_out + (int64_t)m * hs + cb, o);
+        else if (a.h_fin) st16(a.h_fin + (int64_t)(a.fin_idx ? a.fin_idx[m] : m) * a.ld_fin + cb, o);
         if (a.y) {
             if (a.p_drop > 0.f) {
 #pragma unroll
@@ -276,8 +281,8 @@
             __syncthreads();
         }
     }
-    {
-        const RowSrc hsrc = row_src(a.h_in, a.hs, a.rows, m0, wave, lane, a.h_idx);
+    if (m0 < a.n_live) {
+        const RowSrc hsrc = row_src(a.h_in, a.hs, min(a.rows, a.n_live), m0, wave, lane, a.h_idx);
         const WSrc ws = w_src(a.hs, a.hs, c0, wave, lane);
         for (int k0 = 0; k0 < a.hs; k0 += BK) {
             dma_rows_at(hsrc, Z, k0, a.hs, As, wave);
@@ -306,8 +311,8 @@
     const int xcd = blockIdx.x & 7, sq = blockIdx.x >> 3;
     const int m0 = ((sq / nC) * 8 + xcd) * TMW, c0 = (sq % nC) * TC;
     if (m0 >= a.rows) return;
-    const int nkx = a.in_dim / BK, nk = nkx + hs / BK;
-    uint32_t axo[4], aho[4], bxo[3], bho[3];
+    const int nkx = a.in_dim / BK, nk = m0 < a.n_live ? nkx + hs / BK : nkx;
+    uint32_t axo[4], aho[4], bxo[3], bho[3], hz = 0;
 #pragma unroll
     for (int i = 0; i < 4; ++i) {
         const int rl = (i * 8 + wave) * 8 + (lane >> 3);
@@ -315,6 +320,7 @@
         const uint32_t c = (uint32_t)(((lane & 7) ^ swz(rl)) << 4);
         axo[i] = (uint32_t)r * (uint32_t)(a.ldx * 2) + c;
         aho[i] = (uint32_t)r * (uint32_t)(hs * 2) + c;
+        hz |= (m0 + r >= a.n_live ? 1u : 0u) << i;
     }
 #pragma unroll
     for (int i = 0; i < 3; ++i) {
@@ -329,6 +335,7 @@
     const char* Hb = reinterpret_cast<const char*>(a.h_in + (int64_t)m0 * hs);
     const char* Wi = reinterpret_cast<const char*>(a.w_ih);
     const char* Wh = reinterpret_cast<const char*>(a.w_hh);
+    const char* Zb = static_cast<const char*>(a.zeros);
 
     f32x4_t acc[2][16];
 #pragma unroll
@@ -344,10 +351,11 @@
         const int st_ = min((s_), nk - 1);                                                                                    \
         const bool px_ = st_ < nkx;                                                                                           \
         const char* ab_ = px_ ? Xb + st_ * ROWB : Hb + (st_ - nkx) * ROWB;                                                    \
-        GTOS_DMA1(ab_ + (px_ ? axo[0] : aho[0]), (slot) + (0 * 8 + wave) * 1024);                                             \
-        GTOS_DMA1(ab_ + (px_ ? axo[1] : aho[1]), (slot) + (1 * 8 + wave) * 1024);                                             \
-        GTOS_DMA1(ab_ + (px_ ? axo[2] : aho[2]), (slot) + (2 * 8 + wave) * 1024);                                             \
-        GTOS_DMA1(ab_ + (px_ ? axo[3] : aho[3]), (slot) + (3 * 8 + wave) * 1024);                                             \
+        const uint32_t z_ = px_ ? 0u : hz;                                                                                    \
+        GTOS_DMA1((z_ & 1u) ? Zb : ab_ + (px_ ? axo[0] : aho[0]), (slot) + (0 * 8 + wave) * 1024);                            \
+        GTOS_DMA1((z_ & 2u) ? Zb : ab_ + (px_ ? axo[1] : aho[1]), (slot) + (1 * 8 + wave) * 1024);                            \
+        GTOS_DMA1((z_ & 4u) ? Zb : ab_ + (px_ ? axo[2] : aho[2]), (slot) + (2 * 8 + wave) * 1024);                            \
+        GTOS_DMA1((z_ & 8u) ? Zb : ab_ + (px_ ? axo[3] : aho[3]), (slot) + (3 * 8 + wave) * 1024);                            \
     }
 #define GTOS_A2W3_DMA_W(slot, s_)                                                                                             \
     {                                                                                                                         \
@@ -393,13 +401,27 @@
         GTOS_A2W3_DMA_W(sw0, 0);
         GTOS_A2W3_DMA_A(sa1, 1);
     }
-    for (int s = 0; s + 6 <= nk; s += 6) {
+    int s = 0;
+    for (; s + 6 <= nk; s += 6) {
         GTOS_A2W3_STEP(sa0, sw0, sa2, sw1, s);
         GTOS_A2W3_STEP(sa1, sw1, sa0, sw0, s + 1);
         GTOS_A2W3_STEP(sa2, sw0, sa1, sw1, s + 2);
         GTOS_A2W3_STEP(sa0, sw1, sa2, sw0, s + 3);
         GTOS_A2W3_STEP(sa1, sw0, sa0, sw1, s + 4);
         GTOS_A2W3_STEP(sa2, sw1, sa1, sw0, s + 5);
+    }
+    if (s < nk) {
+        GTOS_A2W3_STEP(sa0, sw0, sa2, sw1, s);
+        if (s + 1 < nk) {
+            GTOS_A2W3_STEP(sa1, sw1, sa0, sw0, s + 1);
+            if (s + 2 < nk) {
+                GTOS_A2W3_STEP(sa2, sw0, sa1, sw1, s + 2);
+                if (s + 3 < nk) {
+                    GTOS_A2W3_STEP(sa0, sw1, sa2, sw0, s + 3);
+                    if (s + 4 < nk) GTOS_A2W3_STEP(sa1, sw0, sa0, sw1, s + 4);
+                }
+            }
+        }
     }
     GTOS_VMCNT(0);
 #undef GTOS_A2W3_STEP
@@ -566,6 +588,7 @@
     int zero_row;
     float p_drop; uint64_t seed; int64_t drop_base;
     int rows, hs; const void* zeros;
+    int n_live;
     const bf16_t* wi_t; bf16_t* dinp; int64_t ld_dinp; int n_in; int dinp_acc;
     float p_in; uint64_t seed_in; int64_t in_drop_base;
 };
@@ -755,7 +778,12 @@
         const bf16_t* gp = a.gates + (int64_t)m * 4 * hs + cb;
         ld16(gp, gr); ld16(gp + hs, gz); ld16(gp + 2 * hs, gn);
         ld16(gp + 3 * hs, hn);
-        ld16(a.hprev + (int64_t)(a.hprev_idx ? a.hprev_idx[m] : m) * hs + cb, hp);
+        if (m < a.n_live) {
+            ld16(a.hprev + (int64_t)(a.hprev_idx ? a.hprev_idx[m] : m) * hs + cb, hp);
+        } else {
+#pragma unroll
+            for (int i = 0; i < 16; ++i) hp[i] = 0.f;
+        }
         float* dhp = static_cast<float*>(a.dh) + (int64_t)m * a.ld_dh + cb;
         bf16_t* dhb = static_cast<bf16_t*>(a.dh) + (int64_t)m * a.ld_dh + cb;
         if (a.sum_idx) {
@@ -825,15 +853,33 @@
 
 }
 
-extern "C" int gtos_gru_step_fwd(int rows, int hs, const void* x, int64_t ldx, int in_dim, const void* w_ih, const float* b_ih,
-                                 const void* xg, const void* gf, const int* gf_idx, const void* gb, const int* gb_idx,
-                                 const void* h_in, const int* h_idx, const void* w_hh, const float* b_hh,
-                                 void* h_out, int n_out, void* h_fin, int64_t ld_fin, const int* fin_idx, void* gates, void* y, int64_t ldy,
-                                 float p_drop, uint64_t seed, int64_t drop_base, void* stream) {
+namespace {
+thread_local struct { const void* state; int n_live; } t_zero_rows = {nullptr, 0};
+int take_n_live(const void* state, int rows) {
+    const bool mine = t_zero_rows.state != nullptr && t_zero_rows.state == state;
+    const int n = mine ? t_zero_rows.n_live : rows;
+    t_zero_rows.state = nullptr;
+    return n;
+}
+}
+
+extern "C" int gtos_gru_step_zero_rows(const void* state, int n_live) {
+    t_zero_rows.state = nullptr;
+    if (!state || n_live < 0) return -22;
+    t_zero_rows.state = state; t_zero_rows.n_live = n_live;
+    return 0;
+}
+
+static int step_fwd_launch(int rows, int hs, const void* x, int64_t ldx, int in_dim, const void* w_ih, const float* b_ih,
+                           const void* xg, const void* gf, const int* gf_idx, const void* gb, const int* gb_idx,
+                           const void* h_in, const int* h_idx, const void* w_hh, const float* b_hh,
+                           void* h_out, int n_out, void* h_fin, int64_t ld_fin, const int* fin_idx, void* gates, void* y, int64_t ldy,
+                           float p_drop, uint64_t seed, int64_t drop_base, int n_live, void* stream) {
     if (rows <= 0) return 0;
     if (hs <= 0 || hs % TC) return -22;
-    if (!h_in || !w_hh || !b_hh || !gates) return -23;
-    if ((n_out > 0 && !h_out) || (n_out < rows && !h_fin)) return -23;
+    if (n_live < 0 || n_live > rows) return -22;
+    if ((n_live > 0 && !h_in) || !w_hh || !b_hh || !gates) return -23;
+    if (n_out > 0 && !h_out) return -23;
     if (h_fin && (ld_fin < hs || ld_fin % 8)) return -25;
     const int mode = x ? 1 : (gf ? 2 : 0);
     if (mode == 1) {
@@ -850,14 +896,14 @@
     a.h_in = (const bf16_t*)h_in; a.h_idx = h_idx; a.w_hh = (const bf16_t*)w_hh; a.b_hh = b_hh;
     a.h_out = (bf16_t*)h_out; a.n_out = n_out; a.h_fin = (bf16_t*)h_fin; a.gates = (bf16_t*)gates; a.y = (bf16_t*)y; a.ldy = ldy;
     a.ld_fin = ld_fin; a.fin_idx = fin_idx;
-    a.p_drop = p_drop; a.seed = seed; a.drop_base = drop_base; a.rows = rows; a.hs = hs;
+    a.p_drop = p_drop; a.seed = seed; a.drop_base = drop_base; a.rows = rows; a.hs = hs; a.n_live = n_live;
     a.zeros = gtos_zero_block();
     if (!a.zeros) return -5;
     const long long nM = (rows + TM - 1) / TM, nC = hs / TC;
     const long long nblk = ((nM + 7) / 8) * 8 * nC;
     if (nblk > 0x7fffffffLL) return -6;
     hipStream_t s = static_cast<hipStream_t>(stream);
-    if (mode == 2 && hs == 256 && !h_idx && !y && rows >= 16384) {
+    if (mode == 2 && hs == 256 && !h_idx && !y && rows >= 16384 && n_live == rows && (h_fin || n_out >= rows)) {
         constexpr int KT = 4;
         const size_t lds_bytes = (size_t)KT * B_BYTES + 4 * KT * P_ROWS * ROWB;
         static bool configured = false;
@@ -872,7 +918,7 @@
         return 0;
     }
     static const bool use_a2w3 = !(getenv("GTOS_GRU_FWD_A2W3") && getenv("GTOS_GRU_FWD_A2W3")[0] == '0');
-    if (mode == 1 && use_a2w3 && rows >= 8192 && in_dim % 64 == 0 && (in_dim / 64 + hs / 64) % 6 == 0 && !h_idx && ldx < (1 << 20) &&
+    if (mode == 1 && use_a2w3 && rows >= 8192 && in_dim % 64 == 0 && !h_idx && ldx < (1 << 20) &&
         (int64_t)3 * hs * (in_dim > hs ? in_dim : hs) * 2 < (1LL << 31)) {
         const long long nM8 = (rows + 255) / 256, nblk8 = ((nM8 + 7) / 8) * 8 * nC;
         hipLaunchKernelGGL(gru_step_fwd_a2w3_kernel, dim3((unsigned)nblk8), dim3(512), 0, s, a);
@@ -884,18 +930,30 @@
     return 0;
 }
 
-extern "C" int gtos_gru_step_bwd_fused(int rows, int hs, const void* d4_prev, int rows_prev, const void* w_hh_t,
-                                       const void* gates, const void* hprev, const int* hprev_idx, const void* dy, int64_t ldy,
-                                       void* dh, int dh_dtype, int64_t ld_dh, void* d4, float p_drop, uint64_t seed, int64_t drop_base,
-                                       float* bias_partials, int n_partials, void* hprev_out, const int* sum_idx, const void* dh_src,
-                                       int zero_row,
-                                       const void* w_ih_t, void* dinp, int64_t ld_dinp, int n_in, int dinp_accumulate, float p_in,
-                                       uint64_t seed_in, int64_t in_drop_base, void* stream) {
+extern "C" int gtos_gru_step_fwd(int rows, int hs, const void* x, int64_t ldx, int in_dim, const void* w_ih, const float* b_ih,
+                                 const void* xg, const void* gf, const int* gf_idx, const void* gb, const int* gb_idx,
+                                 const void* h_in, const int* h_idx, const void* w_hh, const float* b_hh,
+                                 void* h_out, int n_out, void* h_fin, int64_t ld_fin, const int* fin_idx, void* gates, void* y, int64_t ldy,
+                                 float p_drop, uint64_t seed, int64_t drop_base, void* stream) {
+    const int n_live = take_n_live(h_in, rows);
+    if (rows > 0 && !h_in) return -23;
+    return step_fwd_launch(rows, hs, x, ldx, in_dim, w_ih, b_ih, xg, gf, gf_idx, gb, gb_idx, h_in, h_idx, w_hh, b_hh, h_out, n_out, h_fin,
+                           ld_fin, fin_idx, gates, y, ldy, p_drop, seed, drop_base, n_live, stream);
+}
+
+static int step_bwd_launch(int rows, int hs, const void* d4_prev, int rows_prev, const void* w_hh_t,
+                           const void* gates, const void* hprev, const int* hprev_idx, const void* dy, int64_t ldy,
+                           void* dh, int dh_dtype, int64_t ld_dh, void* d4, float p_drop, uint64_t seed, int64_t drop_base,
+                           float* bias_partials, int n_partials, void* hprev_out, const int* sum_idx, const void* dh_src,
+                           int zero_row,
+                           const void* w_ih_t, void* dinp, int64_t ld_dinp, int n_in, int dinp_accumulate, float p_in,
+                           uint64_t seed_in, int64_t in_drop_base, int n_live, void* stream) {
+    if (rows > 0 && (n_live < 0 || n_live > rows)) return -22;
     const bool role_b = dinp != nullptr && d4_prev != nullptr && rows_prev > 0;
     if (rows <= 0 && !role_b) return 0;
     if (hs <= 0 || hs % TC) return -22;
     if (rows > 0) {
-        if (!gates || !hprev || !dh || !d4 || (d4_prev && !w_hh_t)) return -23;
+        if (!gates || (n_live > 0 && !hprev) || !dh || !d4 || (d4_prev && !w_hh_t)) return -23;
         if (sum_idx && (!dh_src || (uintptr_t)dh_src % 16)) return -23;
     }
     if (dinp && (!d4_prev || !w_ih_t || sum_idx)) return -23;
@@ -911,7 +969,7 @@
     a.hp_out = (bf16_t*)hprev_out; a.sum_idx = sum_idx; a.dh_src = dh_src; a.zero_row = sum_idx ? zero_row : -1;
     a.wi_t = (const bf16_t*)w_ih_t; a.dinp = role_b ? (bf16_t*)dinp : nullptr; a.ld_dinp = ld_dinp; a.n_in = n_in; a.dinp_acc = dinp_accumulate;
     a.p_in = p_in; a.seed_in = seed_in; a.in_drop_base = in_drop_base;
-    a.p_drop = p_drop; a.seed = seed; a.drop_base = drop_base; a.rows = rows > 0 ? rows : 0; a.hs = hs;
+    a.p_drop = p_drop; a.seed = seed; a.drop_base = drop_base; a.rows = rows > 0 ? rows : 0; a.hs = hs; a.n_live = rows > 0 ? n_live : 0;
     a.zeros = gtos_zero_block();
     if (!a.zeros) return -5;
     const long long cover = role_b && rows_prev > a.rows ? rows_prev : a.rows;
@@ -923,6 +981,19 @@
     return 0;
 }
 
+extern "C" int gtos_gru_step_bwd_fused(int rows, int hs, const void* d4_prev, int rows_prev, const void* w_hh_t,
+                                       const void* gates, const void* hprev, const int* hprev_idx, const void* dy, int64_t ldy,
+                                       void* dh, int dh_dtype, int64_t ld_dh, void* d4, float p_drop, uint64_t seed, int64_t drop_base,
+                                       float* bias_partials, int n_partials, void* hprev_out, const int* sum_idx, const void* dh_src,
+                                       int zero_row,
+                                       const void* w_ih_t, void* dinp, int64_t ld_dinp, int n_in, int dinp_accumulate, float p_in,
+                                       uint64_t seed_in, int64_t in_drop_base, void* stream) {
+    const int n_live = take_n_live(hprev, rows > 0 ? rows : 0);
+    return step_bwd_launch(rows, hs, d4_prev, rows_prev, w_hh_t, gates, hprev, hprev_idx, dy, ldy, dh, dh_dtype, ld_dh, d4,
+                           p_drop, seed, drop_base, bias_partials, n_partials, hprev_out, sum_idx, dh_src, zero_row,
+                           w_ih_t, dinp, ld_dinp, n_in, dinp_accumulate, p_in, seed_in, in_drop_base, n_live, stream);
+}
+
 extern "C" int gtos_gru_step_bwd(int rows, int hs, const void* d4_prev, int rows_prev, const void* w_hh_t,
                                  const void* gates, const void* hprev, const int* hprev_idx, const void* dy, int64_t ldy, void* dh, int dh_dtype,
                                  int64_t ld_dh, void* d4, float p_drop, uint64_t seed, int64_t drop_base, float* bias_partials,
diff --git a/gtos_amd/csrc/rowops.hip b/gtos_amd/csrc/rowops.hip
--- a/gtos_amd/csrc/rowops.hip
+++ b/gtos_amd/csrc/rowops.hip
@@ -1133,6 +1133,45 @@
     return 0;
 }
 
+namespace {
+constexpr int ZR_MAX = 96;
+struct ZeroRanges { int n; int lo[ZR_MAX], hi[ZR_MAX], blk_end[ZR_MAX]; };
+__global__ __launch_bounds__(256) void zero_row_ranges_kernel(bf16_t* __restrict__ p, int64_t ld, int width, ZeroRanges z) {
+    int b = blockIdx.x, j = 0;
+    while (j + 1 < z.n && b >= z.blk_end[j]) ++j;
+    b -= j ? z.blk_end[j - 1] : 0;
+    const int r0 = z.lo[j] + b * 64, r1 = min(z.hi[j], r0 + 64), pieces = width / 8;
+    for (int q = threadIdx.x; q < (r1 - r0) * pieces; q += 256) {
+        const int r = r0 + q / pieces, c = (q % pieces) * 8;
+        *reinterpret_cast<uint4*>(p + (int64_t)r * ld + c) = make_uint4(0, 0, 0, 0);
+    }
+}
+}
+
+extern "C" int gtos_zero_row_ranges(void* p, int rows, int width, int64_t ld, const int* ranges, int n_ranges, void* stream) {
+    if (n_ranges <= 0) return 0;
+    if (!p || !ranges) return -23;
+    if (width <= 0 || width % 8 || ld < width || ld % 8 || (uintptr_t)p % 16) return -25;
+    for (int i = 0; i < n_ranges; ++i)
+        if (ranges[2 * i] < 0 || ranges[2 * i + 1] < ranges[2 * i] || ranges[2 * i + 1] > rows) return -22;
+    for (int i0 = 0; i0 < n_ranges; i0 += ZR_MAX) {
+        ZeroRanges z{};
+        long long blocks = 0;
+        for (int i = i0; i < n_ranges && i < i0 + ZR_MAX; ++i) {
+            const int lo = ranges[2 * i], hi = ranges[2 * i + 1];
+            if (hi == lo) continue;
+            blocks += (hi - lo + 63) / 64;
+            if (blocks > 0x7fffffffLL) return -6;
+            z.lo[z.n] = lo; z.hi[z.n] = hi; z.blk_end[z.n] = (int)blocks; ++z.n;
+        }
+        if (!z.n) continue;
+        hipLaunchKernelGGL(zero_row_ranges_kernel, dim3((unsigned)blocks), dim3(256), 0, static_cast<hipStream_t>(stream), (bf16_t*)p, ld,
+                           width, z);
+        GTOS_CHECK_LAUNCH();
+    }
+    return 0;
+}
+
 extern "C" int gtos_set_seed_epoch(const void* epoch) {
     int rc = gtosi_gemm_set_seed_epoch(epoch);
     if (!rc) rc = gtosi_rel_attn_set_seed_epoch(epoch);
@@ -1143,6 +1182,6 @@
     return rc;
 }
 
-extern "C" int gtos_abi_version(void) { return 25; }
+extern "C" int gtos_abi_version(void) { return 26; }
 
 GTOS_SEED_EPOCH_SETTER(rowops)
diff --git a/gtos_amd/gru.py b/gtos_amd/gru.py
--- a/gtos_amd/gru.py
+++ b/gtos_amd/gru.py
@@ -1,4 +1,5 @@
 import contextlib
+import ctypes
 import os
 
 import torch
@@ -267,6 +268,54 @@
 D4_INPLACE_MIN_BYTES = 8 << 30
 
 
+MAX_ZERO_RANGES = 48
+
+
+def zero_skip():
+    return os.environ.get("GTOS_GRU_ZERO_SKIP", "1")[:1] != "0"
+
+
+def _announce_zero_rows(state, n_live, A):
+    if n_live < A:
+        call("gtos_gru_step_zero_rows", ptr(state), int(n_live))
+
+
+def _int_array(values):
+    arr = (ctypes.c_int * max(1, len(values)))(*values)
+    return arr, ctypes.addressof(arr)
+
+
+def zero_edge_rows(table, N):
+    fill = []
+    for lo, hi in table:
+        head = min(hi, (lo + 31) // 32 * 32)
+        if head > lo:
+            fill.append((lo, head))
+        tail = max(head, hi // 32 * 32)
+        if tail < hi < N:
+            fill.append((tail, hi))
+    return fill
+
+
+def zero_state_plan(bs, offs, direction, table_ok=True):
+    L = len(bs)
+    if direction == 0:
+        live = [0] + [bs[t] for t in range(1, L)]
+    else:
+        live = [bs[t + 1] for t in range(L - 1)] + [0]
+    ranges = []
+    for t in range(L):
+        lo, hi = offs[t] + live[t], offs[t] + bs[t]
+        if hi > lo:
+            if ranges and ranges[-1][1] == lo:
+                ranges[-1][1] = hi
+            else:
+                ranges.append([lo, hi])
+    table = [tuple(r) for r in ranges[:MAX_ZERO_RANGES]] if table_ok else []
+    fill = [tuple(r) for r in ranges[len(table):]] + zero_edge_rows(table, offs[L])
+    return live, table, sorted(fill)
+
+
 class PackedPathGRUFn(torch.autograd.Function):
 
     @staticmethod
@@ -288,7 +337,8 @@
         call("gtos_embed_packed_paths", dt(X), L, R, N, ptr(bank), ptr(plan.order32), ptr(plan.offs_dev), ptr(tab), dim, dim_pad, ptr(X),
              float(p_embed), seed_e, ptr(onehot), Vp, ptr(tokens), stream())
         fin = (torch.empty if bs[0] == R else torch.zeros)((R, 2 * hs), dtype=dtp, device=dev)
-        park = [torch.empty((bs[0], hs), dtype=dtp, device=dev) for _ in (0, 1)]
+        skip = zero_skip()
+        park = None if skip else [torch.empty((bs[0], hs), dtype=dtp, device=dev) for _ in (0, 1)]
         inp, saved = X, []
         for l in range(2):
             last = l == 1
@@ -310,14 +360,19 @@
             for direction in (0, 1):
                 wi, wh, wi_t, wh_t, bi, bh = wts[direction]
                 gates, hprev = bufs[direction]
-                if direction == 0:
+                live, ztable = None, None
+                if skip:
+                    live, ztable, zfill = zero_state_plan(bs, offs, direction, table_ok=weights[l * 8 + direction * 4].shape[1] % 4 == 0)
+                    zarr, zptr = _int_array([v for r in zfill for v in r])
+                    call("gtos_zero_row_ranges", ptr(hprev), N, hs, hprev.stride(0), zptr, len(zfill), stream())
+                elif direction == 0:
                     hprev[:bs[0]].zero_()
                 else:
                     for t in range(L):
                         lo = bs[t + 1] if t + 1 < L else 0
                         if bs[t] > lo:
                             hprev[offs[t] + lo: offs[t] + bs[t]].zero_()
-                h_fin = fin[:, direction * hs:(direction + 1) * hs] if last else park[direction]
+                h_fin = fin[:, direction * hs:(direction + 1) * hs] if last else (None if skip else park[direction])
                 for t in (range(L) if direction == 0 else range(L - 1, -1, -1)):
                     A, off = bs[t], offs[t]
                     nxt = t + 1 if direction == 0 else t - 1
@@ -325,10 +380,12 @@
                         h_out, n_out = hprev[offs[nxt]:], min(A, bs[nxt])
                     else:
                         h_out, n_out = None, 0
+                    if skip:
+                        _announce_zero_rows(hprev[off:off + A], live[t], A)
                     _step_fwd(A, hs, inp[off:off + A], None, hprev[off:off + A], wi, bi, wh, bh, h_out, n_out, h_fin, gates[off:off + A],
                               Y, off * 2 * hs + direction * hs, 2 * hs, pl, seed, off * 2 * hs + direction * hs,
                               fin_idx=plan.order32 if last else None, tag="gru_step_fwd_packed_l%d" % l)
-                layer_saved.append((wi_t, wh_t, gates, hprev))
+                layer_saved.append((wi_t, wh_t, gates, hprev, live, ztable))
             saved.append((inp, seed, pl, layer_saved))
             inp = Y
         ctx.cfg = (plan, table, dim_pad, p_embed, seed_e, hs, weights, saved, onehot, tokens)
@@ -371,7 +428,7 @@
             want_dinp = l == 1 or want_table
             d_in = torch.empty((N, n_in), dtype=dtp, device=dev) if want_dinp else None
             for direction in (0, 1):
-                wi_t, wh_t, gates, hprev = layer_saved[direction]
+                wi_t, wh_t, gates, hprev, live, ztable = layer_saved[direction]
                 layer_saved[direction] = None
                 base = l * 8 + direction * 4
                 w_ih, w_hh, b_ih, b_hh = weights[base:base + 4]
@@ -387,6 +444,8 @@
                 prev = None
                 for t in (range(L - 1, -1, -1) if direction == 0 else range(L)):
                     A, off = bs[t], offs[t]
+                    if live is not None:
+                        _announce_zero_rows(hprev[off:off + A], live[t], A)
                     dyp = None if dY is None else dY.data_ptr() + (off * 2 * hs + direction * hs) * dY.element_size()
                     kw = {} if (rb is None or prev is None) else dict(rb, dinp=d_in[offs[prev]:], in_drop_base=offs[prev] * n_in)
                     _step_bwd_fused(A, hs, None if prev is None else d4[offs[prev]:], 0 if prev is None else bs[prev], wh_t,
@@ -414,6 +473,9 @@
                     if (tg_ih is not None or tg_hh is not None) and w_ih.shape[1] % 4 == 0:
                         with _Timed("gru_dw_grouped_l%d" % l, detail=True, units=2 * N * 3 * hs * (w_ih.shape[1] + hs)):
                             ws = _workspace(dev)
+                            if ztable:
+                                zarr, zptr = _int_array([v for r in ztable for v in r])
+                                call("gtos_gru_weight_grads_zero_rows", ptr(hprev), zptr, len(ztable))
                             call("gtos_gru_weight_grads", N, hs, n_in, w_ih.shape[1], ptr(d4), ptr(inp), inp.stride(0), ptr(hprev), hprev.stride(0),
                                  ptr(scr_ih), scr_ih.stride(0), ptr(scr_hh), scr_hh.stride(0), ptr(ws), ws.numel() * 4, stream())
                     elif tg_ih is not None or tg_hh is not None:
diff --git a/include/gtos_hip.h b/include/gtos_hip.h
--- a/include/gtos_hip.h
+++ b/include/gtos_hip.h
@@ -81,6 +81,8 @@
                       void* h_out, int n_out, void* h_fin, int64_t ld_fin, const int* fin_idx, void* gates, void* y, int64_t ldy,
                       float p_drop, uint64_t seed, int64_t drop_base, void* stream);
 
+int gtos_gru_step_zero_rows(const void* state, int n_live);
+
 int gtos_gru_step_bwd(int rows, int hs, const void* d4_prev, int rows_prev, const void* w_hh_t,
                       const void* gates, const void* hprev, const int* hprev_idx, const void* dy, int64_t ldy, void* dh, int dh_dtype,
                       int64_t ld_dh, void* d4, float p_drop, uint64_t seed, int64_t drop_base, float* bias_partials, int n_partials,
@@ -95,6 +97,8 @@
 
 int gtos_gru_weight_grads(int rows, int hs, int in_dim, int in_valid, const void* d4, const void* x, int64_t ldx, const void* hprev, int64_t ldh,
                           float* dwih, int64_t ld_dwih, float* dwhh, int64_t ld_dwhh, void* workspace, int64_t workspace_bytes, void* stream);
+int gtos_gru_weight_grads_zero_rows(const void* hprev, const int* ranges, int n_ranges);
+int gtos_zero_row_ranges(void* p, int rows, int width, int64_t ld, const int* ranges, int n_ranges, void* stream);
 
 int gtos_gemm_tn_batch(int n, const void* const* A, const int64_t* lda, const int* M, const void* const* B, const int64_t* ldb, const int* N,
                        const int* K, float* const* C, const int64_t* ldc, float* const* bias, void* stream);
```
